# careylab/LocoMouse_cpp

Hardware: AMD Instinct MI355X
Metric: frames/sec whole-node + achieved HBM GB/s; 1024×256 gray, 6 templates (higher is better)
Workload: dtype f32

## Files before the change

### include/locomouse_hip.h

```cpp
#ifndef LOCOMOUSE_HIP_H
#define LOCOMOUSE_HIP_H

#include <stddef.h>
#include <stdint.h>

#ifdef __cplusplus
extern "C" {
#endif

#define LM_ABI_VERSION 6
#define LM_N_PAWS 4
#define LM_N_TAIL_POINTS 15
#define LM_N_LISTS 4
#define LM_N_FEATURES 2

typedef enum {
  LM_OK = 0,
  LM_ERR_INVALID_ARGUMENT = 1,
  LM_ERR_RUNTIME = 2,
  LM_ERR_HIP = 3
} lm_status;

typedef struct {
  int32_t x, y, width, height;
// ... 109 lines not shown
  const int64_t* pw_nz_offset;
  const int32_t* pw_ir;
  const double* pw_pr;
  const int32_t* tail;
} lm_batch_result;

typedef struct lm_ctx lm_ctx;

int32_t lm_abi_version(void);

const char* lm_last_error(void);

lm_status lm_ctx_create(int32_t device, const lm_setup* setup, const lm_params* params,
                        const lm_model* model, int32_t max_batch, lm_ctx** out);
void lm_ctx_destroy(lm_ctx* ctx);

lm_status lm_get_geometry(const lm_ctx* ctx, lm_geometry* out);

void* lm_ctx_stream(lm_ctx* ctx);

lm_status lm_detect_batch(lm_ctx* ctx, const uint8_t* frames, int64_t frame_pitch,
                          int32_t n, int32_t first_frame, const uint8_t* prev_frame,
                          const int32_t* bb, lm_batch_result* out);

lm_status lm_detect_batch_device(lm_ctx* ctx, const uint8_t* d_frames, int64_t frame_pitch,
                                 int32_t n, int32_t first_frame, const uint8_t* d_prev_frame,
                                 const int32_t* bb, lm_batch_result* out);

lm_status lm_detect_submit(lm_ctx* ctx, const uint8_t* frames, int64_t frame_pitch, int32_t n, int32_t first_frame,
                           const uint8_t* prev_frame, const int32_t* bb);
lm_status lm_detect_submit_device(lm_ctx* ctx, const uint8_t* d_frames, int64_t frame_pitch, int32_t n,
                                  int32_t first_frame, const uint8_t* d_prev_frame, const int32_t* bb);
lm_status lm_detect_collect(lm_ctx* ctx, lm_batch_result* out);
int32_t lm_ctx_lanes(const lm_ctx* ctx);
int32_t lm_ctx_pending(const lm_ctx* ctx);


lm_status lm_ctx_set_debug(lm_ctx* ctx, int32_t flags);

lm_status lm_debug_scores(lm_ctx* ctx, int32_t f, int32_t det, float* out, int32_t rows, int32_t cols);

lm_status lm_debug_tail_mask(lm_ctx* ctx, int32_t f, uint8_t* out, int32_t rows, int32_t cols);

int32_t lm_debug_kernel_times(lm_ctx* ctx, const char** names, double* ms, int32_t cap);

int32_t lm_debug_kernel_spans(lm_ctx* ctx, const char** names, double* t0, double* t1, int32_t cap);

lm_status lm_debug_corr_work(const lm_ctx* ctx, int32_t* out);

lm_status lm_debug_tail_work(lm_ctx* ctx, int32_t* out);

lm_status lm_debug_screen_fallback(lm_ctx* ctx, int64_t* out);

lm_status lm_debug_tail_tiles(lm_ctx* ctx, int32_t f, int32_t view, uint8_t* out, int32_t rows, int32_t cols);

lm_status lm_debug_point_work(lm_ctx* ctx, int32_t* out);

lm_status lm_debug_point_tiles(lm_ctx* ctx, int32_t f, int32_t det, uint8_t* out, int32_t rows, int32_t cols);

int32_t lm_debug_dark_tile_width(void);
int32_t lm_debug_dark_tile_height(void);

int32_t lm_debug_batch_slots(const lm_ctx* ctx);


#define LM_BB_FIRSTLAST_AS_EXECUTED 0
#define LM_BB_FIRSTLAST_INTEGER 1

typedef struct {
  int32_t median_filter_size;
  int32_t min_pixel_visible;
  int32_t moving_average_window;
  int32_t conn_comp_connectivity;
  int32_t firstlast_semantics;
  int32_t zero_col_pre, zero_col_post, zero_row_pre, zero_row_post;
  int32_t bb_width, bb_height_side;
  int32_t reserved0;
} lm_bb_params;

typedef struct {
  double x, y_bottom, y_side, width, height_bottom, height_side;
} lm_bb_frame;

typedef struct {
  int32_t n_frames;
  int32_t reserved0;
  lm_rect bb_side_mouse, bb_bottom_mouse;
  const uint32_t* x_pos;
  const uint32_t* y_bottom_pos;
  const uint32_t* y_side_pos;
  const lm_bb_frame* frames;
} lm_bb_result;

typedef struct lm_bb_ctx lm_bb_ctx;

lm_status lm_bb_create(int32_t device, const lm_setup* setup, const lm_bb_params* params, int32_t max_batch,
                       lm_bb_ctx** out);
void lm_bb_destroy(lm_bb_ctx* ctx);

lm_status lm_bb_push(lm_bb_ctx* ctx, const uint8_t* frames, int64_t frame_pitch, int32_t n, lm_bb_frame* out);
lm_status lm_bb_push_device(lm_bb_ctx* ctx, const uint8_t* d_frames, int64_t frame_pitch, int32_t n,
                            lm_bb_frame* out);

lm_status lm_bb_finish(lm_bb_ctx* ctx, lm_bb_result* out);

lm_status lm_bb_debug_binary(lm_bb_ctx* ctx, int32_t f, uint8_t* out, int32_t rows, int32_t cols);
// ... 15 lines not shown
```

### locomouse_cpp_amd/abi.py

```python
import ctypes as C

import numpy as np

LM_OK, LM_ERR_INVALID_ARGUMENT, LM_ERR_RUNTIME, LM_ERR_HIP = 0, 1, 2, 3
LM_N_TAIL_POINTS = 15
LM_FILTER_FUSED, LM_FILTER_UNFUSED = 0, 1
LM_DEBUG_SCORES, LM_DEBUG_TIMING = 1, 2
LM_DEBUG_PLAN_PER_WIDTH, LM_DEBUG_PLAN_MERGED = 16, 32
LM_CORR_FP32, LM_CORR_F16 = 0, 1
LM_DEPTH_8U, LM_DEPTH_32F, LM_DEPTH_64F = 0, 5, 6
DETECTORS = ("paw_bottom", "snout_bottom", "tail_bottom", "paw_side", "snout_side", "tail_side")


class lm_rect(C.Structure):
    _fields_ = [("x", C.c_int32), ("y", C.c_int32), ("width", C.c_int32), ("height", C.c_int32)]

    def tuple(self):
        return (self.x, self.y, self.width, self.height)


class lm_location_prior(C.Structure):
    _fields_ = [(n, C.c_double) for n in ("x", "y", "max_distance", "min_x", "max_x", "min_y", "max_y")]


class lm_params(C.Structure):
    _fields_ = [
        ("conn_comp_connectivity", C.c_int32),
        ("max_displacement_bottom", C.c_int32),
        ("max_displacement_side", C.c_int32),
        ("occlusion_grid_spacing_pixels_side", C.c_int32),
        ("occlusion_grid_spacing_pixels_bottom", C.c_int32),
        ("use_provided_bounding_box", C.c_int32),
        ("transform_gray_values", C.c_int32),
        ("use_reference_image_brightness", C.c_int32),
        ("side_bottom_min_overlap", C.c_double),
        ("occlusion_grid_max_width", C.c_double),
        ("tail_sub_bounding_box", C.c_double),
        ("alpha_vel_bottom", C.c_double),
        ("alpha_vel_side", C.c_double),
        ("pairwise_occluded_cost", C.c_double),
        ("location_prior", lm_location_prior * 5),
        ("bounding_box_side", lm_rect),
        ("bounding_box_bottom", lm_rect),
        ("gray_value_transformation", C.c_float * 256),
        ("gray_value_transformation_depth", C.c_int32),
    ]


class lm_detector(C.Structure):
    _fields_ = [("weights", C.POINTER(C.c_double)), ("rows", C.c_int32), ("cols", C.c_int32), ("bias", C.c_double)]


class lm_model(C.Structure):
    _fields_ = [(n, lm_detector) for n in ("paw_bottom", "paw_side", "snout_bottom", "snout_side", "tail_bottom", "tail_side")]


class lm_setup(C.Structure):
    _fields_ = [
        ("method", C.c_int32),
        ("flip", C.c_int32),
        ("video_rows", C.c_int32),
        ("video_cols", C.c_int32),
        ("background", C.POINTER(C.c_uint8)),
        ("calib_rows", C.c_int32),
# ... 333 lines not shown
```

### locomouse_cpp_amd/csrc/lm_corr.h

```cpp
#ifndef LM_CORR_H
#define LM_CORR_H

#include <hip/hip_runtime.h>
#include <stddef.h>
#include <stdint.h>

#include "lm_corr_dir.h"
#include "lm_device.h"

#define LM_CORR_THREADS 192
#define PK_C 5
#define PK_R 4

__host__ __device__ constexpr int pk_stride(int cols) { return cols + ((4 - (cols & 7)) + 8) % 8; }

struct LmDetGroup {
  int32_t n;
  int32_t ids[LM_NDET];
  int32_t tile_end[LM_NDET];
  int32_t ring_floats;
};

#ifdef LM_KW_ONLY
#define LM_KW_LIST(X) X(LM_KW_ONLY)
#elif defined(LM_KW_C3)
#define LM_KW_LIST(X) X(22) X(24) X(26) X(30)
#else
#define LM_KW_LIST(X)                                                                                             \
  X(16) X(17) X(18) X(19) X(20) X(21) X(22) X(23) X(24) X(25) X(26) X(27) X(28) X(29) X(30) X(31) X(32) X(36) \
      X(40) X(44) X(48) X(52) X(56) X(60) X(64)
#endif
#if defined(LM_KW_ONLY) || defined(LM_KW_C3)
#define LM_KW_LIST_RW_ALL LM_KW_LIST
#else
#define LM_KW_LIST_RW_ALL(X) X(16) X(18) X(20) X(22) X(24) X(26) X(28) X(30) X(32) X(36) X(40)
#endif
__host__ __device__ constexpr bool rw_all_width(int kw) {
  return kw % 2 == 0 && kw >= 16 && (kw <= 32 || kw == 36 || kw == 40);
}

#ifndef LM_RW_WAVES
#define LM_RW_WAVES 4
#endif
#define LM_RW_THREADS (64 * LM_RW_WAVES)
#ifndef LM_RW_ALL_WPE
#define LM_RW_ALL_WPE 4
#endif
#define LM_RW_TH 16
#define LM_RW_HTH LM_FH
#ifndef LM_RW_HSLOTS
#define LM_RW_HSLOTS (LM_FH == 4 ? 3 : LM_RW_NQ == 4 ? 7 : 8)
#endif
static_assert(LM_RW_HSLOTS >= (LM_FH == 4 ? 3 : 7), "k_corr_rw ring: rows live during a step");

__host__ __device__ constexpr int rw_stride(int kw) { return (LM_FW + kw - 1 + 3 + 3) / 4 * 4; }
__host__ __device__ constexpr int rw_qpitch(int kw) {
  return (LM_RW_HSLOTS + 1) * rw_stride(kw) +
         ((LM_FW / 5 - ((LM_RW_HSLOTS + 1) * rw_stride(kw)) % 32) + 32) % 32;
}
__host__ __device__ constexpr int rw_ring_floats(int kw) { return LM_RW_NQ * rw_qpitch(kw); }
size_t corr_rw_lds(int kw);

#define LM_F16_WAVES 4
#define LM_F16_TW 128
#define LM_F16_TH 64
#define LM_F16_THREADS (64 * LM_F16_WAVES)
#define LM_F16_MAX_NCH 10

__host__ __device__ constexpr int f16_nch(int kw) { return (kw + 31 + 15) / 16; }
__host__ __device__ constexpr int f16_cols(int nch) { return LM_F16_TW - 32 + 16 * nch; }
__host__ __device__ constexpr int f16_stride(int cols) { return (cols + 7) / 16 * 16 + 8; }
__host__ __device__ constexpr size_t f16_lds_bytes(int nch, int kh) {
  (void)nch;
  return (size_t)(LM_F16_TH + kh - 1) * f16_stride(f16_cols(nch)) * 2;
}
static inline float f16_bfrag_weight(const double* w, int kw, int i, int c, int l, int j) {
  const int r = l & 31, h = l >> 5, jj = 16 * c + 8 * h + j - r;
  return (jj >= 0 && jj < kw) ? (float)w[(size_t)i * kw + jj] : 0.0f;
}

bool corr_ring(int kw);
const void* corr_kernel(int kw, bool unf);
const void* corr_kernel_gen(bool unf);
const void* corr_kernel_rw_all(bool unf);
const void* corr_kernel_f16(int kw);
struct CorrDark {
  uint8_t* flags = nullptr;
  int32_t* cnt = nullptr;
  uint32_t* list = nullptr;
  uint8_t* tail_flags = nullptr;
  int32_t* tail_cnt = nullptr;
  uint32_t* tail_list = nullptr;
  uint8_t* pt_flags = nullptr;
  int32_t* pt_cnt = nullptr;
  uint32_t* pt_list = nullptr;
};
hipError_t launch_corr(const void* fn, bool ring, dim3 grid, int threads, size_t lds, hipStream_t st, const LmConst* K,
                       const LmDetGroup& G, const uint8_t* ext, int64_t ext_slot_bytes, const void* weights, int s0,
                       unsigned long long* keys, int32_t* n_pos, uint8_t* tailbin, int64_t tailbin_slot_bytes,
                       const CorrDark& dark, const LmCorrDirRec* dir);
#define LM_DEVERR_CORR_DIR 64
hipError_t launch_corr_dir(hipStream_t st, const LmConst* K, const LmDetGroup* groups, const char* ring, int ngroups,
                           int nslots, const CorrDark& dark, LmCorrDirRec* out, int32_t* err);
hipError_t launch_corr_dbg(bool unf, dim3 grid, hipStream_t st, const LmConst* K, const uint8_t* ext,
                           int64_t ext_slot_bytes, const float* weights, int s0, float* dbg, const int64_t* dbg_off,
                           int64_t dbg_slot_floats);

#endif
```

### locomouse_cpp_amd/csrc/lm_corr.hip

```cpp

#include <hip/hip_runtime.h>
#include <stdint.h>

#include <algorithm>
#include <cstdio>
#include <map>
#include <type_traits>
#include <vector>

#include "lm_corr.h"

#define DEV __device__ __forceinline__

typedef float lm_f2 __attribute__((ext_vector_type(2)));

template <bool UNF>
DEV lm_f2 corr_tap(lm_f2 acc, lm_f2 w2, lm_f2 p) {
  if constexpr (UNF) {
    const lm_f2 prod = w2 * p;
    return acc + prod;
  } else {
    return __builtin_elementwise_fma(w2, p, acc);
  }
}
// ... 92 lines not shown
#pragma unroll
          for (int k = 0; k < 16; ++k) o[k] = (float)((w[k >> 2] >> (8 * (k & 3))) & 0xFFu);
        } else {
#pragma unroll
          for (int k = 0; k < 16; ++k)
            if (c0 + k >= 0 && c0 + k < cols) o[k] = (float)((w[k >> 2] >> (8 * (k & 3))) & 0xFFu);
        }
      }
    }
  }
}

struct CorrTile {
  int d, oy0, ox0;
};
DEV CorrTile corr_tile(const LmConst& K, const LmDetGroup& G) {
  int gi = 0, tb = 0;
#pragma unroll
  for (int k = 0; k < LM_NDET - 1; ++k)
    if (k + 1 < G.n && (int)blockIdx.x >= G.tile_end[k]) {
      gi = k + 1;
      tb = G.tile_end[k];
    }
  const int d = G.ids[gi];
  const int lt = blockIdx.x - tb;
  const int tx = K.det[d].tiles_x;
  return CorrTile{d, (lt / tx) * K.det[d].tile_h, (lt % tx) * K.det[d].tile_w};
}

DEV const uint8_t* corr_src(const LmConst& K, const LmDet& D, const uint8_t* ext, int64_t ext_slot_bytes, int slot,
                            int oy0, int ox0) {
  return ext + (int64_t)slot * ext_slot_bytes + (D.view ? (int64_t)K.ext_h[0] * K.ext_w[0] : 0) +
         (int64_t)(D.in_y + oy0) * K.ext_w[D.view] + (D.in_x + ox0);
}


struct RwRun {
  const uint32_t* l;
  int nvalid;
  int ftx;
  int slot, oy, ox;
  DEV uint32_t entry(int i) const { return l ? l[min(i, nvalid - 1)] : 0u; }
  DEV void tile(int i, uint32_t e, int& s, int& y, int& x) const {
    if (l) {
      const int lt = (int)(e & 0xFFFFu);
      s = (int)(e >> 16);
      y = (lt / ftx) * LM_FH;
      x = (lt % ftx) * LM_FW;
    } else {
      s = slot;
      y = oy + (i / LM_RW_NQX) * LM_FH;
      x = ox + (i % LM_RW_NQX) * LM_FW;
    }
  }
};

static_assert(LM_TL_NC == 64, "one list counter per lane");

struct CorrList {
  const int32_t* cnt;
  const uint32_t* lst;
  int ftx, ntile;
};
DEV CorrList corr_det_list(const LmConst& K, const LmDet& D, const int32_t* tl_cnt, const uint32_t* tl_list, int tl_per_det,
                           const int32_t* tt_cnt, const uint32_t* tt_list) {
  const bool pt = tl_cnt != nullptr && D.kind == 0;
  if (!pt && !(tt_cnt != nullptr && D.kind != 0))
    return CorrList{nullptr, nullptr, 0, 0};
  const int v = pt ? D.view : D.list;
  const int li = pt && !tl_per_det ? v : D.list;
  const int ftx = pt ? K.fl_tx[v] : K.tt_tx[v], ntile = ftx * (pt ? K.fl_ty[v] : K.tt_ty[v]);
  const uint32_t* lst = pt ? tl_list + (int64_t)li * K.tl_stride : tt_list + (int64_t)li * K.tt_stride;
  return CorrList{(pt ? tl_cnt : tt_cnt) + li * LM_TL_NC, lst, ftx, ntile};
}

DEV int corr_scan_waves(int wv) {
  const int lane = threadIdx.x & 63;
  int P = wv;
#pragma unroll
  for (int o = 1; o < 64; o <<= 1) {
    const int u = __shfl_up(P, o);
    if (lane >= o) P += u;
  }
  return P;
}

DEV RwRun corr_listed_run(const CorrList& Ls, int cn, int wv, int P, int local, int nslots) {
  constexpr int NQ = LM_RW_NQ;
  const int c = __builtin_amdgcn_readfirstlane(__ffsll((long long)__ballot(P > local)) - 1);
  const int w = local - (__builtin_amdgcn_readlane(P, c) - __builtin_amdgcn_readlane(wv, c));
  const int ng = (nslots + LM_INGEST_FB - 1) / LM_INGEST_FB;
  return RwRun{Ls.lst + (int64_t)lm_tl_y0(c, ng) * LM_INGEST_FB * Ls.ntile + NQ * w,
               min(NQ, __builtin_amdgcn_readlane(cn, c) - NQ * w), Ls.ftx, 0, 0, 0};
}

DEV RwRun corr_unlisted_run(const LmDet& D, int nt, int s0, int local) {
  const int tx = D.tiles_x;
  const int lt = local - (local / nt) * nt;
  return RwRun{nullptr, LM_RW_NQ, 0, s0 + local / nt, (lt / tx) * LM_RW_TH, (lt % tx) * LM_TW};
}

DEV bool corr_locate_walk(const LmConst& K, const LmDetGroup& G, int nslots, int s0, int g, const int32_t* tl_cnt,
                          const uint32_t* tl_list, int tl_per_det, const int32_t* tt_cnt, const uint32_t* tt_list, int& d,
                          RwRun& R) {
  const int lane = threadIdx.x & 63;
  int base = 0;
// ... 133 lines not shown
DEV void lds_pair_nw(lm_f2& dst, unsigned base) {
  static_assert(Q + STRIDE <= 255, "ds_read2_b32 offset range");
  asm volatile("ds_read2_b32 %0, %1 offset0:%2 offset1:%3" : "=v"(dst) : "v"(base), "i"(Q), "i"(Q + STRIDE) : "memory");
}

template <bool UNF, int H>
DEV lm_f2 corr_tap_h(lm_f2 acc, lm_f2 w2, lm_f2 p) {
  if constexpr (UNF) {
    lm_f2 prod;
    if constexpr (H == 0)
      asm volatile("v_pk_mul_f32 %0, %1, %2 op_sel_hi:[0,1]" : "=v"(prod) : "s"(w2), "v"(p));
    else
      asm volatile("v_pk_mul_f32 %0, %1, %2 op_sel:[1,0] op_sel_hi:[1,1]" : "=v"(prod) : "s"(w2), "v"(p));
    asm volatile("v_pk_add_f32 %0, %0, %1" : "+v"(acc) : "v"(prod));
    return acc;
  } else if constexpr (H == 0) {
    asm volatile("v_pk_fma_f32 %0, %1, %2, %0 op_sel_hi:[0,1,1]" : "+v"(acc) : "s"(w2), "v"(p));
    return acc;
  } else {
    asm volatile("v_pk_fma_f32 %0, %1, %2, %0 op_sel:[1,0,0] op_sel_hi:[1,1,1]" : "+v"(acc) : "s"(w2), "v"(p));
    return acc;
  }
}

#define LM_RWF(a, w, p, sel) "v_pk_fma_f32 %" #a ", %" #w ", %" #p ", %" #a " " sel "\n"
#define LM_RW_S0 "op_sel_hi:[0,1,1]"
#define LM_RW_S1 "op_sel:[1,0,0] op_sel_hi:[1,1,1]"
DEV void rw_pair_ab(lm_f2 (&a)[PK_C], lm_f2 (&b)[PK_C], lm_f2 wa, lm_f2 wb, const lm_f2* px) {
  static_assert(PK_C == 5, "the asm block is written for 5 columns");
  asm volatile(LM_RWF(0, 10, 12, LM_RW_S0) LM_RWF(1, 10, 13, LM_RW_S0) LM_RWF(2, 10, 14, LM_RW_S0)
                   LM_RWF(3, 10, 15, LM_RW_S0) LM_RWF(4, 10, 16, LM_RW_S0)
               LM_RWF(5, 11, 12, LM_RW_S0) LM_RWF(6, 11, 13, LM_RW_S0) LM_RWF(7, 11, 14, LM_RW_S0)
                   LM_RWF(8, 11, 15, LM_RW_S0) LM_RWF(9, 11, 16, LM_RW_S0)
               LM_RWF(0, 10, 13, LM_RW_S1) LM_RWF(1, 10, 14, LM_RW_S1) LM_RWF(2, 10, 15, LM_RW_S1)
                   LM_RWF(3, 10, 16, LM_RW_S1) LM_RWF(4, 10, 17, LM_RW_S1)
               LM_RWF(5, 11, 13, LM_RW_S1) LM_RWF(6, 11, 14, LM_RW_S1) LM_RWF(7, 11, 15, LM_RW_S1)
                   LM_RWF(8, 11, 16, LM_RW_S1) LM_RWF(9, 11, 17, LM_RW_S1)
               : "+v"(a[0]), "+v"(a[1]), "+v"(a[2]), "+v"(a[3]), "+v"(a[4]), "+v"(b[0]), "+v"(b[1]), "+v"(b[2]),
                 "+v"(b[3]), "+v"(b[4])
               : "s"(wa), "s"(wb), "v"(px[0]), "v"(px[1]), "v"(px[2]), "v"(px[3]), "v"(px[4]), "v"(px[5]));
}
DEV void rw_pair_1(lm_f2 (&a)[PK_C], lm_f2 w, const lm_f2* px) {
  asm volatile(LM_RWF(0, 5, 6, LM_RW_S0) LM_RWF(1, 5, 7, LM_RW_S0) LM_RWF(2, 5, 8, LM_RW_S0)
                   LM_RWF(3, 5, 9, LM_RW_S0) LM_RWF(4, 5, 10, LM_RW_S0)
               LM_RWF(0, 5, 7, LM_RW_S1) LM_RWF(1, 5, 8, LM_RW_S1) LM_RWF(2, 5, 9, LM_RW_S1)
                   LM_RWF(3, 5, 10, LM_RW_S1) LM_RWF(4, 5, 11, LM_RW_S1)
               : "+v"(a[0]), "+v"(a[1]), "+v"(a[2]), "+v"(a[3]), "+v"(a[4])
               : "s"(w), "v"(px[0]), "v"(px[1]), "v"(px[2]), "v"(px[3]), "v"(px[4]), "v"(px[5]));
}
#undef LM_RWF
#undef LM_RW_S0
#undef LM_RW_S1

template <int KW, bool UNF>
struct RwPipe {
  using P = RwPlan<KW>;
  static constexpr int STR = rw_stride(KW);
  lm_f2 px[PK_C + KW - 1];
  lm_f2 acc[2][PK_C];
  lm_f2 wa[P::PMAX], wb[P::PMAX];
  template <int Q0, int Q1>
  DEV void issue(unsigned base) {
    if constexpr (Q0 < Q1) {
      lds_pair_nw<STR, Q0>(px[Q0], base);
      issue<Q0 + 1, Q1>(base);
    }
  }
  template <int C>
  DEV void load_w(lm_f2 (&na)[P::PMAX], lm_f2 (&nb)[P::PMAX], const lm_f2* __restrict__ ra,
                  const lm_f2* __restrict__ rb) {
#pragma unroll
    for (int q = 0; q < P::qe(C) - P::qb(C); ++q) {
      na[q] = ra[P::qb(C) + q];
      nb[q] = rb[P::qb(C) + q];
    }
  }
  template <int J, int C, bool A, bool B>
  DEV void compute_from() {
    if constexpr (J < P::end(C) && !UNF && (J & 1) == 0 && J + 1 < P::end(C) &&
                  (A || B)) {
      constexpr int q = J / 2 - P::qb(C);
      if constexpr (A && B) rw_pair_ab(acc[0], acc[1], wa[q], wb[q], &px[J]);
      else if constexpr (A) rw_pair_1(acc[0], wa[q], &px[J]);
      else rw_pair_1(acc[1], wb[q], &px[J]);
      compute_from<J + 2, C, A, B>();
    } else if constexpr (J < P::end(C)) {
      constexpr int q = J / 2 - P::qb(C), h = J & 1;
      if constexpr (A) {
#pragma unroll
        for (int c = 0; c < PK_C; ++c) acc[0][c] = corr_tap_h<UNF, h>(acc[0][c], wa[q], px[c + J]);
      }
      if constexpr (B) {
#pragma unroll
        for (int c = 0; c < PK_C; ++c) acc[1][c] = corr_tap_h<UNF, h>(acc[1][c], wb[q], px[c + J]);
      }
      compute_from<J + 1, C, A, B>();
    }
  }
  template <int C, bool A, bool B, bool NEXT = true, typename F>
  DEV void chunks(unsigned base, unsigned base_n, const lm_f2* __restrict__ ra, const lm_f2* __restrict__ rb,
                  const lm_f2* __restrict__ ra_n, const lm_f2* __restrict__ rb_n, F&& at_start) {
    __builtin_amdgcn_s_waitcnt(0xC07F);
    __builtin_amdgcn_sched_barrier(0);
    if constexpr (C == 0) at_start();
    lm_f2 na[P::PMAX], nb[P::PMAX];
    if constexpr (C + 1 < P::N) {
      load_w<C + 1>(na, nb, ra, rb);
      issue<P::pbeg(C + 1), P::pend(C + 1)>(base);
    } else if constexpr (NEXT) {
      load_w<0>(na, nb, ra_n, rb_n);
      issue<P::pbeg(0), P::pend(0)>(base_n);
    }
    __builtin_amdgcn_sched_barrier(0);
    compute_from<P::beg(C), C, A, B>();
    __builtin_amdgcn_sched_barrier(0);
    if constexpr (C + 1 < P::N || NEXT) {
#pragma unroll
      for (int q = 0; q < P::PMAX; ++q) {
        wa[q] = na[q];
        wb[q] = nb[q];
      }
    }
    if constexpr (C + 1 < P::N) chunks<C + 1, A, B, NEXT>(base, base_n, ra, rb, ra_n, rb_n, at_start);
  }
};

struct RwArgs {
  const LmConst* K;
  LmDetGroup G;
  const uint8_t* ext;
  int64_t ext_slot_bytes;
  const float* weights;
  int32_t s0, nslots;
  unsigned long long* keys;
  int32_t* n_pos;
  uint8_t* tailbin;
  int64_t tailbin_slot_bytes;
  const int32_t* tl_cnt;
  const uint32_t* tl_list;
  int32_t tl_per_det;
  const int32_t* tt_cnt;
  const uint32_t* tt_list;
};

template <int KW, bool UNF>
DEV __attribute__((always_inline)) void rw_tile(const RwArgs& A, int dix, const RwRun& R, float* ring) {
  constexpr int NQ = LM_RW_NQ;
  constexpr int QX = LM_FW / PK_C;
  static_assert(LM_FH == PK_R && QX * NQ == 64, "one row of 8 lanes per 40 x 4 sub-tile");
  constexpr int STR = rw_stride(KW);
  constexpr int QP = rw_qpitch(KW);
  constexpr int NL = (3 + LM_FW + KW - 1 + 3) / 4;
  constexpr int NLD = (NQ * NL + 63) / 64;
  static_assert(NLD <= 4, "window rows wider than four loads per lane");
  constexpr int HS = LM_RW_HSLOTS;
  const LmConst& K = *A.K;
  const LmDet& D = K.det[dix];
  const int lane = threadIdx.x & 63;
  const int q = lane / QX, lx = lane % QX;
  const int kh = D.kh, kwp = D.kwp;
  __builtin_assume(kh >= 2);
  const int nrows = LM_RW_HTH + kh - 1;
  const int ew = K.ext_w[D.view];
  const int ew4 = ew >> 2;
  const uint8_t* __restrict__ vext = A.ext + (D.view ? (int64_t)K.ext_h[0] * K.ext_w[0] : 0);
  const int mis = D.in_x & 3;
  int slot, oy0, ox0;
  R.tile(q, R.entry(q), slot, oy0, ox0);
  const bool valid = q < R.nvalid;
  int smin = slot;
#pragma unroll
  for (int o = 1; o < 64; o <<= 1) smin = min(smin, __shfl_xor(smin, o));
  smin = __builtin_amdgcn_readfirstlane(smin);
  const __amdgpu_buffer_rsrc_t wrsrc = __builtin_amdgcn_make_buffer_rsrc(
      const_cast<uint8_t*>(vext + (int64_t)smin * A.ext_slot_bytes), 0, (int)0xFFFFFFFF, 0x00020000);
  unsigned la[NLD];
  int lo[NLD];
  bool lk[NLD];
#pragma unroll
  for (int k = 0; k < NLD; ++k) {
    const int e = lane + 64 * k, qk = e / NL, dk = e - qk * NL;
    lk[k] = qk < R.nvalid;
    int sk, yk, xk;
    const int ik = min(qk, NQ - 1);
    R.tile(ik, R.entry(ik), sk, yk, xk);
    la[k] = (unsigned)((int64_t)(sk - smin) * A.ext_slot_bytes + (int64_t)(D.in_y + yk) * ew + (D.in_x + xk - mis)) +
            4u * (unsigned)dk;
    lo[k] = (int)(unsigned)(uintptr_t)(__attribute__((address_space(3))) float*)(ring + qk * QP + 4 * dk);
  }

  unsigned mbits = 0;
  if (D.kind == 0 && valid) {
    const uint8_t* __restrict__ m =
        vext + (int64_t)slot * A.ext_slot_bytes + (int64_t)(D.m_y + oy0) * ew + (D.m_x + ox0 + lx * PK_C);
    const int mo = (int)((uintptr_t)m & 3);
    const unsigned* __restrict__ m4 = reinterpret_cast<const unsigned*>(m - mo);
    unsigned mw[PK_R][2];
#pragma unroll
    for (int r = 0; r < PK_R; ++r) {
      mw[r][0] = m4[(int64_t)r * ew4];
      mw[r][1] = m4[(int64_t)r * ew4 + 1];
    }
#pragma unroll
    for (int r = 0; r < PK_R; ++r) {
      const unsigned long long row = ((unsigned long long)mw[r][1] << 32 | mw[r][0]) >> (8 * mo);
#pragma unroll
      for (int c = 0; c < PK_C; ++c) mbits |= (((unsigned)(row >> (8 * c)) & 0xFFu) > 25u ? 1u : 0u) << (r * PK_C + c);
    }
  }

  struct Row {
    unsigned v[NLD];
  };
  auto load_row = [&](int r) -> Row {
    Row w;
    const int ro = __builtin_amdgcn_readfirstlane(min(r, nrows - 1) * ew);
#pragma unroll
    for (int k = 0; k < NLD; ++k) w.v[k] = __builtin_amdgcn_raw_buffer_load_b32(wrsrc, (int)la[k], ro, 0);
    return w;
  };
  auto store_row = [&](int r, Row w) {
    if (r >= nrows) return;
    const int s = r % HS;
    const int so = __builtin_amdgcn_readfirstlane(s * STR * (int)sizeof(float));
#pragma unroll
    for (int k = 0; k < NLD; ++k)
      if (lk[k]) {
        const unsigned v = w.v[k];
        typedef float f4v __attribute__((ext_vector_type(4)));
        const f4v f = {(float)(v & 0xFFu), (float)((v >> 8) & 0xFFu), (float)((v >> 16) & 0xFFu), (float)(v >> 24)};
        typedef __attribute__((address_space(3))) f4v lds_f4;
        *reinterpret_cast<lds_f4*>((uintptr_t)(unsigned)(lo[k] + so)) = f;
        if (s == 0) *reinterpret_cast<lds_f4*>((uintptr_t)(unsigned)(lo[k] + HS * STR * (int)sizeof(float))) = f;
      }
  };
  {
    Row v0[HS];
#pragma unroll
    for (int r = 0; r < HS; ++r) v0[r] = load_row(r);
#pragma unroll
    for (int r = 0; r < HS; ++r) store_row(r, v0[r]);
  }

  const lm_f2* __restrict__ W = reinterpret_cast<const lm_f2*>(A.weights + D.w_off);
  const int kwp2 = kwp >> 1;
  const unsigned ring_base = (unsigned)(uintptr_t)(const __attribute__((address_space(3))) float*)ring +
                             (unsigned)(q * QP * (int)sizeof(float));
  const unsigned lane_off = (unsigned)((lx * PK_C + mis) * (int)sizeof(float));
  const unsigned ring_lane = ring_base + lane_off;
  auto row_base = [&](int t) -> unsigned {
    return ring_lane + (unsigned)__builtin_amdgcn_readfirstlane((t % HS) * STR * (int)sizeof(float));
  };
  RwPipe<KW, UNF> S;
#pragma unroll
  for (int p = 0; p < 2; ++p)
#pragma unroll
    for (int c = 0; c < PK_C; ++c) S.acc[p][c] = (lm_f2){D.delta, D.delta};
  auto wrow = [&](int i) { return W + min(max(i, 0), kh - 1) * kwp2; };
  S.template load_w<0>(S.wa, S.wb, wrow(0), wrow(-2));
  S.template issue<RwPlan<KW>::pbeg(0), RwPlan<KW>::pend(0)>(row_base(0));
  using T1 = std::true_type;
  using F0 = std::false_type;
  auto stepx = [&](int t, auto B0, auto B1, Row& st, Row& ld, auto N) {
    S.template chunks<0, decltype(B0)::value, decltype(B1)::value, decltype(N)::value>(
        row_base(t), row_base(t + 1), wrow(t), wrow(t - 2), wrow(t + 1), wrow(t - 1),
        [&]() { if constexpr (decltype(N)::value) ld = load_row(t + HS + 1); });
    if constexpr (decltype(N)::value) store_row(t + HS, st);
  };
  Row r0 = load_row(HS), r1;
  {
    stepx(0, T1{}, F0{}, r0, r1, T1{});
    stepx(1, T1{}, F0{}, r1, r0, T1{});
    int t = 2;
    for (; t + 1 < kh; t += 2) {
      stepx(t, T1{}, T1{}, r0, r1, T1{});
      stepx(t + 1, T1{}, T1{}, r1, r0, T1{});
    }
    if (t < kh) {
      stepx(t, T1{}, T1{}, r0, r1, T1{});
      stepx(kh, F0{}, T1{}, r1, r0, T1{});
      stepx(kh + 1, F0{}, T1{}, r0, r1, F0{});
    } else {
      stepx(kh, F0{}, T1{}, r0, r1, T1{});
      stepx(kh + 1, F0{}, T1{}, r1, r0, F0{});
    }
  }
  __builtin_amdgcn_s_waitcnt(0xC07F);

  unsigned bits = 0;
  if (valid) {
#pragma unroll
    for (int p = 0; p < PK_R / 2; ++p)
#pragma unroll
      for (int c = 0; c < PK_C; ++c) {
        const int x = ox0 + lx * PK_C + c;
        const int y0 = oy0 + 2 * p;
        if (x < D.ow && y0 < D.oh && S.acc[p][c].x > 0.0f) bits |= 1u << ((2 * p) * PK_C + c);
        if (x < D.ow && y0 + 1 < D.oh && S.acc[p][c].y > 0.0f) bits |= 1u << ((2 * p + 1) * PK_C + c);
      }
  }
  if (D.kind != 0) {
    constexpr int WPS = QX / LM_FH;
    static_assert(WPS * LM_FH == QX && (LM_FW == 40 ? WPS == 2 : WPS == 4), "a sub-tile's bitmap words, one per lane");
    unsigned* s_tb = reinterpret_cast<unsigned*>(ring);
    const int w0 = ox0 >> 5;
    s_tb[lane] = 0u;
    __builtin_amdgcn_wave_barrier();
#pragma unroll
    for (int r = 0; r < PK_R; ++r)
#pragma unroll
      for (int c = 0; c < PK_C; ++c)
        if (bits & (1u << (r * PK_C + c))) {
          const int x = ox0 + lx * PK_C + c;
          atomicOr(&s_tb[q * QX + r * WPS + (x >> 5) - w0], 1u << (x & 31));
        }
    __builtin_amdgcn_wave_barrier();
    const unsigned v = s_tb[lane];
    unsigned* __restrict__ tb = reinterpret_cast<unsigned*>(A.tailbin + (int64_t)slot * A.tailbin_slot_bytes) +
                                (D.list ? (int64_t)K.tail_hb * K.tail_nw : 0);
    const int y = oy0 + lx / WPS, gw = w0 + lx % WPS;
    if (v && y < D.oh && gw < K.tail_nw) atomicOr(&tb[(int64_t)y * K.tail_nw + gw], v);
    return;
  }
  bits &= mbits;
  const int cnt = __popc(bits);
  int incl = cnt;
#pragma unroll
  for (int o = 1; o < QX; o <<= 1) {
    const int u = __shfl_up(incl, o, QX);
    if (lx >= o) incl += u;
  }
  const int tot = __shfl(incl, QX - 1, QX);
  const int before = incl - cnt, lastl = (lane & ~(QX - 1)) + QX - 1;
  if (__ballot(tot != 0) == 0) return;
  int base_k = 0;
  if (lane == lastl && tot) base_k = atomicAdd(&A.n_pos[slot * LM_NLIST + D.list], tot);
  base_k = __shfl(base_k, lastl);
  unsigned long long* __restrict__ kl = A.keys + (int64_t)slot * K.keys_per_slot + K.list_off[D.list] + base_k + before;
  int pos = 0;
#pragma unroll
  for (int p = 0; p < PK_R / 2; ++p)
#pragma unroll
    for (int c = 0; c < PK_C; ++c)
#pragma unroll
      for (int hh = 0; hh < 2; ++hh) {
        const int r = 2 * p + hh, k = r * PK_C + c;
        if (bits & (1u << k)) {
          const int y = oy0 + r, x = ox0 + lx * PK_C + c;
          const float sc = hh ? S.acc[p][c].y : S.acc[p][c].x;
          kl[pos++] = ((unsigned long long)(~__float_as_uint(sc)) << 32) | (unsigned)(y * D.ow + x);
        }
      }
}

#ifndef LM_RW_XCD
#define LM_RW_XCD 16
#endif
DEV int xcd_block(int b, int nb) {
#if LM_RW_XCD
  constexpr int C = LM_RW_XCD;
  const int full = nb / (8 * C) * (8 * C);
  if (b >= full) return b;
  const int k = b >> 3, x = b & 7;
  return (k / C) * (8 * C) + x * C + (k % C);
#else
  (void)nb;
  return b;
#endif
}

#ifndef LM_RW_WPE
#define LM_RW_WPE (LM_FW == 40 ? 4 : 5)
#endif
template <int KW, bool UNF>
__global__ __launch_bounds__(LM_RW_THREADS) __attribute__((amdgpu_waves_per_eu(KW <= 32 ? LM_RW_WPE : 1, 8))) void k_corr_rw(
    const LmConst* __restrict__ Kp, const LmDetGroup G, const uint8_t* __restrict__ ext, int64_t ext_slot_bytes,
    const float* __restrict__ weights, int s0, int nslots, unsigned long long* __restrict__ keys,
    int32_t* __restrict__ n_pos, uint8_t* __restrict__ tailbin, int64_t tailbin_slot_bytes,
    const int32_t* __restrict__ tl_cnt, const uint32_t* __restrict__ tl_list, int tl_per_det,
    const int32_t* __restrict__ tt_cnt, const uint32_t* __restrict__ tt_list, const LmCorrDirRec* __restrict__ dir) {
  extern __shared__ uint4 lds_rw[];
  const int wave = __builtin_amdgcn_readfirstlane(threadIdx.x >> 6);
  float* ring = reinterpret_cast<float*>(lds_rw) + wave * rw_ring_floats(KW);
  const RwArgs a{Kp,    G,       ext,    ext_slot_bytes, weights, s0, nslots, keys, n_pos, tailbin, tailbin_slot_bytes,
                 tl_cnt, tl_list, tl_per_det, tt_cnt, tt_list};
  int d;
  RwRun R;
  if (!corr_locate_rw(*a.K, G, a.nslots, a.s0, xcd_block(blockIdx.x, gridDim.x) * LM_RW_WAVES + wave, a.tl_cnt,
                      a.tl_list, a.tl_per_det, a.tt_cnt, a.tt_list, dir, d, R))
    return;
  rw_tile<KW, UNF>(a, d, R, ring);
}

template <bool UNF>
__global__ __launch_bounds__(LM_RW_THREADS) __attribute__((amdgpu_waves_per_eu(LM_RW_ALL_WPE, 8))) void k_corr_rw_all(
    const LmConst* __restrict__ Kp, const LmDetGroup G, const uint8_t* __restrict__ ext, int64_t ext_slot_bytes,
    const float* __restrict__ weights, int s0, int nslots, unsigned long long* __restrict__ keys,
    int32_t* __restrict__ n_pos, uint8_t* __restrict__ tailbin, int64_t tailbin_slot_bytes,
    const int32_t* __restrict__ tl_cnt, const uint32_t* __restrict__ tl_list, int tl_per_det,
    const int32_t* __restrict__ tt_cnt, const uint32_t* __restrict__ tt_list, const LmCorrDirRec* __restrict__ dir) {
  extern __shared__ uint4 lds_rw[];
  const int wave = __builtin_amdgcn_readfirstlane(threadIdx.x >> 6);
  float* ring = reinterpret_cast<float*>(lds_rw) + wave * G.ring_floats;
  const RwArgs a{Kp,    G,       ext,    ext_slot_bytes, weights, s0, nslots, keys, n_pos, tailbin, tailbin_slot_bytes,
                 tl_cnt, tl_list, tl_per_det, tt_cnt, tt_list};
  int d;
  RwRun R;
  if (!corr_locate_rw(*a.K, G, a.nslots, a.s0, xcd_block(blockIdx.x, gridDim.x) * LM_RW_WAVES + wave, a.tl_cnt,
                      a.tl_list, a.tl_per_det, a.tt_cnt, a.tt_list, dir, d, R))
    return;
  switch (a.K->det[d].kw_ring) {
#define LM_KW_CASE(n)           \
  case n:                       \
    rw_tile<n, UNF>(a, d, R, ring); \
    break;
    LM_KW_LIST_RW_ALL(LM_KW_CASE)
#undef LM_KW_CASE
    default:
      break;
  }
}

template <bool UNF>
__global__ __launch_bounds__(LM_CORR_THREADS) void k_corr_gen(const LmConst* __restrict__ Kp, const LmDetGroup G,
                                                              const uint8_t* __restrict__ ext, int64_t ext_slot_bytes,
                                                              const float* __restrict__ weights, int s0,
                                                              unsigned long long* __restrict__ keys,
                                                              int32_t* __restrict__ n_pos, uint8_t* __restrict__ tailbin,
                                                              int64_t tailbin_slot_bytes,
                                                              const uint8_t* __restrict__ dark,
                                                              const uint8_t* __restrict__ tail_flags,
                                                              const uint8_t* __restrict__ pt_flags) {
  const LmConst& K = *Kp;
  extern __shared__ float lds[];
  __shared__ int s_cnt, s_base;
  const int slot = s0 + blockIdx.y;
  const CorrTile T = corr_tile(K, G);
  const LmDet D = K.det[T.d];
  const int oy0 = T.oy0, ox0 = T.ox0;
  if (corr_tile_dark(K, D, pt_flags ? pt_flags + (int64_t)(D.list & 1) * K.pt_plane : dark, tail_flags, slot, oy0, ox0))
    return;
  const int kh = D.kh, kwp = D.kwp, ch = D.chunk_rows;
  const int cols = LM_TW + kwp - 1, stride = pk_stride(cols);
  const int ew = K.ext_w[D.view];
  const uint8_t* __restrict__ src = corr_src(K, D, ext, ext_slot_bytes, slot, oy0, ox0);
  const float* __restrict__ W = weights + D.w_off;
  if (threadIdx.x == 0) s_cnt = 0;
  const int ly = threadIdx.x >> 4, lx = threadIdx.x & 15;
  lm_f2 acc[PK_R / 2][PK_C];
#pragma unroll
  for (int p = 0; p < PK_R / 2; ++p)
#pragma unroll
    for (int c = 0; c < PK_C; ++c) acc[p][c] = (lm_f2){D.delta, D.delta};
  for (int i0 = 0; i0 < kh; i0 += ch) {
    const int cn = min(ch, kh - i0);
    __syncthreads();
    tile_fill_f32(lds, stride, src + (int64_t)i0 * ew, ew, LM_TH + cn - 1, cols);
    __syncthreads();
    for (int t = 0; t < cn + PK_R - 2; ++t) {
      const float* p0 = lds + (ly * PK_R + t) * stride + lx * PK_C;
      for (int jc = 0; jc < kwp; jc += LM_JC) {
        lm_f2 px[PK_C + LM_JC - 1];
#pragma unroll
        for (int q = 0; q < PK_C + LM_JC - 1; ++q) px[q] = (lm_f2){p0[jc + q], p0[jc + q + stride]};
#pragma unroll
        for (int p = 0; p < PK_R / 2; ++p) {
          const int i = t - 2 * p;
// ... 226 lines not shown
  const int ew = K.ext_w[D.view];
  const uint8_t* __restrict__ base =
      ext + (int64_t)slot * ext_slot_bytes + (D.view ? (int64_t)K.ext_h[0] * K.ext_w[0] : 0);
  const float* __restrict__ W = weights + D.w_off;
  for (int64_t e = (int64_t)blockIdx.x * blockDim.x + threadIdx.x; e < n; e += (int64_t)gridDim.x * blockDim.x) {
    const int y = (int)(e / D.ow), x = (int)(e % D.ow);
    const uint8_t* src = base + (int64_t)(D.in_y + y) * ew + (D.in_x + x);
    float a = D.delta;
    for (int i = 0; i < D.kh; ++i)
      for (int j = 0; j < D.kw; ++j) a = corr_tap1<UNF>(a, W[i * D.kwp + j], (float)src[(int64_t)i * ew + j]);
    dbg[(int64_t)slot * dbg_slot_floats + dbg_off[d] + e] = a;
  }
}

const void* corr_kernel_f16(int kw) {
  switch (f16_nch(kw)) {
    case 2: return (const void*)&k_corr_f16<2>;
    case 3: return (const void*)&k_corr_f16<3>;
    case 4: return (const void*)&k_corr_f16<4>;
    case 5: return (const void*)&k_corr_f16<5>;
    case 6: return (const void*)&k_corr_f16<6>;
    case 7: return (const void*)&k_corr_f16<7>;
    case 8: return (const void*)&k_corr_f16<8>;
    case 9: return (const void*)&k_corr_f16<9>;
    case 10: return (const void*)&k_corr_f16<10>;
    default: return nullptr;
  }
}

bool corr_ring(int kw) {
  switch (kw) {
#define LM_KW_CASE(n) case n:
    LM_KW_LIST(LM_KW_CASE)
#undef LM_KW_CASE
    return true;
    default:
      return false;
  }
}

const void* corr_kernel(int kw, bool unf) {
  switch (kw) {
#define LM_KW_CASE(n) \
  case n:             \
    return unf ? (const void*)&k_corr_rw<n, true> : (const void*)&k_corr_rw<n, false>;
    LM_KW_LIST(LM_KW_CASE)
#undef LM_KW_CASE
    default:
      return unf ? (const void*)&k_corr_gen<true> : (const void*)&k_corr_gen<false>;
  }
}

size_t corr_rw_lds(int kw) { return (size_t)LM_RW_WAVES * rw_ring_floats(kw) * sizeof(float); }

const void* corr_kernel_gen(bool unf) { return unf ? (const void*)&k_corr_gen<true> : (const void*)&k_corr_gen<false>; }

const void* corr_kernel_rw_all(bool unf) {
  return unf ? (const void*)&k_corr_rw_all<true> : (const void*)&k_corr_rw_all<false>;
}

hipError_t launch_corr(const void* fn, bool ring, dim3 grid, int threads, size_t lds, hipStream_t st, const LmConst* K,
                       const LmDetGroup& G, const uint8_t* ext, int64_t ext_slot_bytes, const void* weights, int s0,
                       unsigned long long* keys, int32_t* n_pos, uint8_t* tailbin, int64_t tailbin_slot_bytes,
                       const CorrDark& dk, const LmCorrDirRec* dir) {
  if (ring) {
    int nslots = (int)grid.y;
    const unsigned waves = (unsigned)(G.tile_end[G.n - 1] * nslots);
    int per_det = dk.pt_cnt != nullptr ? 1 : 0;
    const int32_t* tl_cnt = per_det ? dk.pt_cnt : dk.cnt;
    const uint32_t* tl_list = per_det ? dk.pt_list : dk.list;
    void* args[] = {(void*)&K,       (void*)&G,    (void*)&ext,     (void*)&ext_slot_bytes,
                    (void*)&weights, (void*)&s0,   (void*)&nslots,  (void*)&keys,
                    (void*)&n_pos,   (void*)&tailbin, (void*)&tailbin_slot_bytes, (void*)&tl_cnt,
                    (void*)&tl_list, (void*)&per_det, (void*)&dk.tail_cnt, (void*)&dk.tail_list, (void*)&dir};
    return hipLaunchKernel(fn, dim3((waves + LM_RW_WAVES - 1) / LM_RW_WAVES), dim3(LM_RW_THREADS), args, lds, st);
  }
  void* args[] = {(void*)&K,     (void*)&G,       (void*)&ext,     (void*)&ext_slot_bytes,           (void*)&weights,
                  (void*)&s0,    (void*)&keys,    (void*)&n_pos,   (void*)&tailbin, (void*)&tailbin_slot_bytes,
                  (void*)&dk.flags, (void*)&dk.tail_flags, (void*)&dk.pt_flags};
  return hipLaunchKernel(fn, grid, dim3(threads), args, lds, st);
}

hipError_t launch_corr_dir(hipStream_t st, const LmConst* K, const LmDetGroup* groups, const char* ring, int ngroups,
                           int nslots, const CorrDark& dk, LmCorrDirRec* out, int32_t* err) {
  if (ngroups < 1 || ngroups > LM_NDET) return hipErrorInvalidValue;
  LmCorrDirGroups A{};
  A.n = ngroups;
  for (int b = 0; b < ngroups; ++b) {
    A.ring[b] = ring[b] ? 1 : 0;
    A.g[b] = groups[b];
  }
  const int per_det = dk.pt_cnt != nullptr ? 1 : 0;
  k_corr_dir<<<ngroups, 64, 0, st>>>(K, A, nslots, per_det ? dk.pt_cnt : dk.cnt, per_det ? dk.pt_list : dk.list, per_det,
                                     dk.tail_cnt, dk.tail_list, out, err);
  return hipGetLastError();
}

hipError_t launch_corr_dbg(bool unf, dim3 grid, hipStream_t st, const LmConst* K, const uint8_t* ext,
                           int64_t ext_slot_bytes, const float* weights, int s0, float* dbg, const int64_t* dbg_off,
                           int64_t dbg_slot_floats) {
  if (unf)
    k_corr_dbg<true><<<grid, 256, 0, st>>>(K, ext, ext_slot_bytes, weights, s0, dbg, dbg_off, dbg_slot_floats);
  else
    k_corr_dbg<false><<<grid, 256, 0, st>>>(K, ext, ext_slot_bytes, weights, s0, dbg, dbg_off, dbg_slot_floats);
  return hipGetLastError();
}
// ... 2 lines not shown
```

### locomouse_cpp_amd/csrc/lm_device.h

```cpp
#ifndef LM_DEVICE_H
#define LM_DEVICE_H

#include <stdint.h>

#if defined(__HIPCC__)
#define LM_HD __host__ __device__
#else
#define LM_HD
#endif

#define LM_C 5
#define LM_R 3
#define LM_TW (16 * LM_C)
#define LM_TH (16 * LM_R)
#define LM_JC 4
#ifndef LM_FW
#define LM_FW 40
#endif
#ifndef LM_FH
#define LM_FH 4
#endif
static_assert((LM_FW == 40 || LM_FW == 80) && (LM_FH == 4 || LM_FH == 8), "dark-tile grid");
#define LM_RW_NQX (LM_TW / LM_FW)
#define LM_RW_NQY (16 / LM_FH)
// ... 11 lines not shown
#define LM_NLIST 4
#define LM_NFEAT 2

enum { DET_PAW_B = 0, DET_SNOUT_B = 1, DET_TAIL_B = 2, DET_PAW_S = 3, DET_SNOUT_S = 4, DET_TAIL_S = 5 };
enum { LIST_PAW_B = 0, LIST_SNOUT_B = 1, LIST_PAW_S = 2, LIST_SNOUT_S = 3 };

struct LmDet {
  int32_t view;
  int32_t kind;
  int32_t list;
  int32_t kh, kw, kwp;
  int32_t kw_ring;
  int32_t w_off;
  float delta;
  int32_t oh, ow;
  int32_t in_y, in_x;
  int32_t m_y, m_x;
  int32_t tiles_x, tiles_y, tile_base;
  int32_t tile_w, tile_h;
  int32_t box_w, box_h;
  int32_t chunk_rows;
  int32_t w16_off;
  float wscale, inv_wscale;
};

struct LmConst {
  LmDet det[LM_NDET];
  int32_t n_tiles;
  int32_t ext_h[2], ext_w[2];
  int32_t ext_oy[2], ext_ox[2];
  int32_t crop_h[2], crop_w[2];
  int32_t unpad_y[2], unpad_x[2];
  int32_t video_rows, video_cols;
  int32_t n_rows, n_cols;
  int32_t pad_pre_rows, pad_pre_cols, ipad_rows, ipad_cols;
  int32_t flip;
  int32_t tail_w, tail_hb, tail_hs;
  int32_t tail_cap, tail_ntc;
  int32_t tail_nw, tail_bm_words;
  int32_t connectivity;
  int32_t fl_tx[2], fl_ty[2], fl_off[2], fl_slot;
  int32_t tl_stride;
  int32_t tt_tx[2], tt_ty[2], tt_off[2], tt_slot;
  int32_t tt_stride;
  int64_t pt_plane;
  int32_t tb_skip[LM_NDET], tb_off[LM_NDET], tb_rng[LM_NDET], tb_lds[2];
  double tb_bias[LM_NDET];
  int32_t tbw_br[2], tbw_nband[2], tbw_blo[2], tbw_nbk[2], tbw_rows[2], tbw_v[2], tbw_al[2], tbw_work[2], tbw_lds[2];
  int32_t tbw_use[LM_NDET], tbw_pn[LM_NDET], tbw_win[LM_NDET], tbw_wsz[LM_NDET], tbw_ent[LM_NDET];
  uint32_t tbw_inv[LM_NDET];
  int32_t tbr_on[LM_NDET], tbr_ng[LM_NDET], tbr_off[LM_NDET];
  int32_t tbs_on[LM_NDET], tbs_off[LM_NDET];
  float tbs_bf[LM_NDET], tbs_e[LM_NDET];
  int32_t fl_my[2], fl_mx[2], fl_oh[2], fl_ow[2];
  int32_t ing_b0[2], ing_nb[2], ing_threads;
  int32_t list_cap[LM_NLIST];
  int64_t list_off[LM_NLIST];
  int64_t keys_per_slot;
  double side_bottom_min_overlap;
  double alpha_vel_bottom, pairwise_occluded_cost;
  int32_t max_displacement_bottom, ong_spacing_bottom;
  int32_t ong_nx, ong_ny;
  double ong_br_x, ong_br_y;
  int32_t bb_bottom_w, bb_bottom_h;
  int32_t spre_b_w, spre_b_h, spre_t_w, spre_t_h;
  int32_t match_b[LM_NFEAT][4];
  int32_t match_s[LM_NFEAT][4];
  int32_t size_b[LM_NFEAT][2];
  int32_t size_s[LM_NFEAT][2];
  double prior[5][7];
  int32_t gray_lut_on;
  uint8_t gray_lut[256];
};

LM_HD inline uint32_t lm_rcp(int d) { return (uint32_t)(0x80000000u / (uint32_t)d + 1u); }
LM_HD inline int lm_div(int x, uint32_t rcp) { return (int)(((uint64_t)(uint32_t)x * rcp) >> 31); }

LM_HD inline int lm_tbw_band(const LmDet& D, int ty, int br, int j, int* t0, int* nty) {
  *t0 = j * br;
  const int t1 = ty < *t0 + br ? ty : *t0 + br;
  *nty = t1 > *t0 ? t1 - *t0 : 0;
  if (*nty == 0) return 0;
  return (D.oh < LM_FH * t1 ? D.oh : LM_FH * t1) - LM_FH * *t0;
}

struct LmSlot {
  int32_t crop_x[2], crop_y[2];
  int32_t frame;
  int32_t active;
};

struct LmSlotOut {
  int32_t n_pos[LM_NLIST];
  int32_t cand_off[LM_NLIST];
  int32_t cand_cnt[LM_NLIST];
  int32_t p22d_off[LM_NFEAT], p22d_cnt[LM_NFEAT];
  int32_t side_off[LM_NFEAT], side_cnt[LM_NFEAT];
  int32_t unary_off[LM_NFEAT], unary_cnt[LM_NFEAT];
  int32_t pw_rows[LM_NFEAT], pw_cols[LM_NFEAT], pw_nnz[LM_NFEAT];
  int32_t pw_jc_off[LM_NFEAT], pw_nz_off[LM_NFEAT];
  int32_t tail[45];
  int32_t ties[LM_NLIST];
  int32_t bottom_kept[LM_NFEAT];
  int32_t pad_[1];
};

// ... 70 lines not shown
```

### locomouse_cpp_amd/csrc/lm_kernels.hip

```cpp
#include <hip/hip_runtime.h>
#include <stdint.h>

#include <type_traits>
#include <utility>

#include "lm_device.h"
#include "lm_introsort.h"

#include "lm_dev_common.h"
#include "lm_tail_bound.h"
#include "lm_tile_plan.h"



__global__ __launch_bounds__(LM_MM_THREADS) void k_minmax(const uint8_t* const* __restrict__ frame_ptr,
                                                          const uint8_t* __restrict__ bkg, int npix, int s0,
                                                          unsigned* __restrict__ mm) {
  const int slot = s0 + blockIdx.y;
  const lm_gu8* __restrict__ F = as_global(frame_ptr[slot]);
  const int nvec = npix >> 4;
  const int per = (nvec + LM_MM_SPLIT - 1) / LM_MM_SPLIT;
  const int v0 = blockIdx.x * per, v1 = min(nvec, v0 + per);
  const lm_gu4* F4 = reinterpret_cast<const lm_gu4*>(F);
  const uint4* B4 = reinterpret_cast<const uint4*>(bkg);
  unsigned mn = 255, mx = 0;
  auto fold = [&](unsigned fw, unsigned bw) {
#pragma unroll
    for (int k = 0; k < 4; ++k) {
      const unsigned fv = (fw >> (8 * k)) & 255u, bv = (bw >> (8 * k)) & 255u;
      const unsigned d = fv > bv ? fv - bv : 0u;
      mn = min(mn, d);
      mx = max(mx, d);
    }
  };
  int i = v0 + threadIdx.x;
  for (; i + 3 * LM_MM_THREADS < v1; i += 4 * LM_MM_THREADS) {
    lm_u32x4 f[4];
    uint4 b[4];
#pragma unroll
    for (int u = 0; u < 4; ++u) {
      f[u] = F4[i + u * LM_MM_THREADS];
      b[u] = B4[i + u * LM_MM_THREADS];
    }
#pragma unroll
    for (int u = 0; u < 4; ++u) {
      fold(f[u].x, b[u].x);
      fold(f[u].y, b[u].y);
      fold(f[u].z, b[u].z);
      fold(f[u].w, b[u].w);
    }
  }
  for (; i < v1; i += LM_MM_THREADS) {
    const lm_u32x4 f = F4[i];
    const uint4 b = B4[i];
    fold(f.x, b.x);
    fold(f.y, b.y);
    fold(f.z, b.z);
    fold(f.w, b.w);
  }
  if (blockIdx.x == LM_MM_SPLIT - 1)
    for (int q = (nvec << 4) + threadIdx.x; q < npix; q += LM_MM_THREADS) {
      const unsigned fv = F[q], bv = bkg[q];
// ... 545 lines not shown
    for (int i = tid; i < ntile; i += T) {
      bool keep = br ? br[i] != 0 : true;
      mbr += br && keep ? 1 : 0;
      if (keep && use[k])
        keep = !lm_tb_tile_skip(rmax, rmin, ftx, D.oh, D.kh, i / ftx, i % ftx, P, P + D.kh, K.tb_bias[d]);
      if (keep && use[k] && K.tbr_on[d] != 0)
        keep = !lm_tbr_tile_skip(bmax, bmin, nbw, D.in_y, D.in_x, D.oh, D.ow, D.kh, D.kw, i / ftx, i % ftx,
                                 tbc + K.tbr_off[d], K.tb_bias[d], LM_TB_RH, false);
      fl[i] = keep ? 1 : 0;
      mine += keep ? 1 : 0;
    }
    if (mine) atomicAdd(&s_n[k], mine);
    if (mbr) atomicAdd(&s_b[k], mbr);
  }
  __syncthreads();
  const int G = ((int)gridDim.x + LM_INGEST_FB - 1) / LM_INGEST_FB;
  const int c = ((int)blockIdx.x / LM_INGEST_FB) * LM_TL_NC / G;
  if (tid < 3 && (K.det[3 * v + tid].kind != 0 ? tt_cnt != nullptr : pt_cnt != nullptr)) {
    const LmDet& D = K.det[3 * v + tid];
    int32_t* __restrict__ cnt = D.kind != 0 ? tt_cnt + v * LM_TL_NC : pt_cnt + D.list * LM_TL_NC;
    s_base[tid] = s_n[tid] ? atomicAdd(&cnt[c], s_n[tid]) : 0;
    if (D.kind == 0 && s_b[tid]) atomicAdd(&pt_cnt[(LM_NLIST + D.list) * LM_TL_NC + c], s_b[tid]);
  }
  __syncthreads();
#pragma unroll
  for (int k = 0; k < 3; ++k) {
    if (!on[k]) continue;
    const LmDet& D = K.det[3 * v + k];
    const bool tail = D.kind != 0;
    const int ntile = tail ? K.tt_tx[v] * K.tt_ty[v] : K.fl_tx[v] * K.fl_ty[v];
    const uint8_t* __restrict__ fl = tail ? tail_flags + (int64_t)slot * K.tt_slot + K.tt_off[v]
                                          : pt_flags + (D.list & 1) * K.pt_plane + (int64_t)slot * K.fl_slot + K.fl_off[v];
    uint32_t* __restrict__ out =
        (tail ? tt_list + (int64_t)v * K.tt_stride : pt_list + (int64_t)D.list * K.tl_stride) +
        (int64_t)lm_tl_y0(c, G) * LM_INGEST_FB * ntile + s_base[k];
    for (int i = tid; i < ntile; i += T)
      if (fl[i]) out[atomicAdd(&s_k[k], 1)] = ((uint32_t)slot << 16) | (uint32_t)i;
  }
}

DEV uint32_t range_merge(uint32_t a, uint32_t b) { return lm_tb_range_merge(a, b); }
DEV int wave_append(bool p, int* ctr) {
  const unsigned long long m = __ballot(p);
  if (m == 0ull) return 0;
  const int rank = (int)__builtin_amdgcn_mbcnt_hi((unsigned)(m >> 32), __builtin_amdgcn_mbcnt_lo((unsigned)m, 0u));
  int base = 0;
  if (p && rank == 0) base = atomicAdd(ctr, (int)__popcll(m));
  return __shfl(base, __ffsll((long long)m) - 1) + rank;
}
#ifndef LM_TBW_WPE
#define LM_TBW_WPE 8
#endif
#define TBW_SEL(a) (k == 0 ? a[0] : k == 1 ? a[1] : a[2])
template <bool ROWS>
__global__ __launch_bounds__(LM_TB_THREADS) __attribute__((amdgpu_waves_per_eu(LM_TBW_WPE, 8))) void k_tile_bound(
    const LmConst* __restrict__ Kp, const uint32_t* __restrict__ rng, int64_t rng_slot, int s0, int nslot,
    const double* __restrict__ tbc, const uint8_t* __restrict__ bright, uint8_t* __restrict__ tail_flags,
    int32_t* __restrict__ tt_cnt, uint32_t* __restrict__ tt_list, uint8_t* __restrict__ pt_flags,
    int32_t* __restrict__ pt_cnt, uint32_t* __restrict__ pt_list, unsigned long long* __restrict__ tbs_fallback) {
  const LmConst& K = *Kp;
  extern __shared__ __attribute__((aligned(16))) uint8_t tbw_lds[];
  __shared__ int s_n[3], s_b[3], s_m[3], s_base[3], s_nw;
  const int v = (int)blockIdx.y < K.tbw_nband[0] ? 0 : 1;
  const int band = (int)blockIdx.y - (v ? K.tbw_nband[0] : 0);
  const int slot = s0 + (int)blockIdx.x;
  const int T = (int)blockDim.x, tid = (int)threadIdx.x;
  if (tid < 3) {
    s_n[tid] = 0;
    s_b[tid] = 0;
    s_m[tid] = 0;
  }
  if (tid == 0) s_nw = 0;
  bool on[3], use[3], refine[3], tail[3];
  int t0[3], nt[3], ohb[3], ftx[3], tbase[3];
  uint8_t* fl[3];
  int y_lo = K.ext_h[v], y_hi = 0;
#pragma unroll
  for (int k = 0; k < 3; ++k) {
    const int d = 3 * v + k;
    const LmDet& D = K.det[d];
    tail[k] = D.kind != 0;
    on[k] = tail[k] ? tt_cnt != nullptr : pt_cnt != nullptr;
    use[k] = on[k] && K.tbw_use[d] != 0;
    ftx[k] = tail[k] ? K.tt_tx[v] : K.fl_tx[v];
    int nty;
    ohb[k] = lm_tbw_band(D, tail[k] ? K.tt_ty[v] : K.fl_ty[v], K.tbw_br[v], band, &t0[k], &nty);
    nt[k] = on[k] ? nty * ftx[k] : 0;
    tbase[k] = t0[k] * ftx[k];
    fl[k] = tail[k] ? tail_flags + (int64_t)slot * K.tt_slot + K.tt_off[v]
                    : pt_flags + (D.list & 1) * K.pt_plane + (int64_t)slot * K.fl_slot + K.fl_off[v];
    use[k] = use[k] && nt[k] > 0;
    refine[k] = use[k] && K.tbr_on[d] != 0;
    if (use[k]) {
      y_lo = min(y_lo, D.in_y + LM_FH * t0[k]);
      y_hi = max(y_hi, D.in_y + LM_FH * t0[k] + ohb[k] + D.kh - 1);
    }
  }
  y_hi = min(y_hi, K.ext_h[v]);
  const int nrow = max(0, min(y_hi - y_lo, K.tbw_rows[v]));
  const int nbk = K.tbw_nbk[v], nw = nbk / 2;
  uint32_t* B = reinterpret_cast<uint32_t*>(tbw_lds);
  uint32_t* V = reinterpret_cast<uint32_t*>(tbw_lds + K.tbw_v[v]);
  uint32_t* work = reinterpret_cast<uint32_t*>(tbw_lds + K.tbw_work[v]);
  __syncthreads();
  constexpr int LD = LM_TBW_LD;
  const int ne = nrow * nw, ewq = K.ext_w[v] / LM_INGEST_VEC;
  const uint32_t rc = lm_rcp(max(nw, 1));
  const uint32_t* __restrict__ src = rng + (int64_t)slot * rng_slot +
                                     (v ? (int64_t)K.ext_h[0] * K.ext_w[0] / LM_INGEST_VEC : 0) +
                                     (int64_t)min(y_lo, y_hi) * ewq + K.tbw_blo[v] / 2;
  uint32_t w[LD];
  auto rng_load = [&](int e0) {
#pragma unroll
    for (int u = 0; u < LD; ++u) {
      const int e = e0 + u * T + tid;
// ... 238 lines not shown
        }) ? -1 : 1;
      };
      auto level_b = [&](int rs, int nn) {
        return lm_tbr_sum_negative(kh, ng, C, bias, [&](int i, int g, unsigned& M, unsigned& m) {
          const uint16_t* row = B16 + (row0 + rs + i) * nbk;
          M = 0u;
          m = 255u;
          for (int r = 0; r < nn; ++r, row += nbk) {
            unsigned a, b;
            lm_tbr_pair_range(nullptr, row, ba0 + g, bendl, a, b);
            M = max(M, a);
            m = min(m, b);
          }
        });
      };
      using std::integral_constant;
      using std::false_type;
      using std::true_type;
      bool proven;
      if constexpr (!ROWS) {
        proven = nr == LM_TB_H && level_v(integral_constant<int, 0>{}, false_type{}) < 0;
      } else {
        proven = false;
        if (nr != LM_TB_H) {
        } else if (nc != 1) proven = level_v(integral_constant<int, 0>{}, false_type{}) < 0;
        else {
          int dec = 0;
          if (K.tbs_on[d] != 0) {
            if (ng == 4) dec = level_v(integral_constant<int, 4>{}, true_type{});
            else if (ng == 3) dec = level_v(integral_constant<int, 3>{}, true_type{});
            else if (ng == 2) dec = level_v(integral_constant<int, 2>{}, true_type{});
            else dec = level_v(integral_constant<int, 1>{}, true_type{});
            const unsigned long long und = __ballot(dec == 0);
            if (und != 0ull && (tid & (WV - 1)) == __ffsll((long long)und) - 1)
              atomicAdd(tbs_fallback, (unsigned long long)__popcll(und));
          }
          if (dec == 0) {
            if (ng == 4) dec = level_v(integral_constant<int, 4>{}, false_type{});
            else if (ng == 3) dec = level_v(integral_constant<int, 3>{}, false_type{});
            else if (ng == 2) dec = level_v(integral_constant<int, 2>{}, false_type{});
            else dec = level_v(integral_constant<int, 1>{}, false_type{});
          }
          proven = dec < 0;
        }
      }
      if (!proven && !(LM_TB_RH == LM_TB_H && nr == LM_TB_H)) {
        if (LM_TB_RH == LM_TB_H) {
          proven = level_b(0, nr);
        } else {
          proven = true;
          for (int r = 0; r < nr && proven; ++r) proven = level_b(r, 1);
        }
      }
      if (!proven) mark[mb + t] = 1u;
    }
    __syncthreads();
    constexpr int CR = LM_TBW_CR;
    for (int g0 = 0; g0 < nref; g0 += CR * T) {
      uint32_t en[CR];
      int kk[CR];
#pragma unroll
      for (int u = 0; u < CR; ++u) {
        const int i = g0 + u * T + tid;
        const bool act = i < nref;
        const int k = i < nr3[0] ? 0 : i < nr3[0] + nr3[1] ? 1 : 2;
        const int t = i - (k == 0 ? 0 : k == 1 ? nr3[0] : nr3[0] + nr3[1]);
        en[u] = act ? reinterpret_cast<const uint32_t*>(tbw_lds + TBW_SEL(ent3))[t] : 0u;
        const bool kp = act && mark[i] != 0u;
        kk[u] = kp ? k : -1;
        if (act) TBW_SEL(fl)[en[u] & 0xFFFFu] = kp ? 1 : 0;
      }
      __syncthreads();
#pragma unroll
      for (int u = 0; u < CR; ++u)
#pragma unroll
        for (int k = 0; k < 3; ++k) {
          const bool mine = kk[u] == k;
          const int pos = wave_append(mine, &s_m[k]);
          if (mine) reinterpret_cast<uint32_t*>(tbw_lds + ent3[k])[pos] = en[u];
        }
    }
    __syncthreads();
    if (tid < 3) {
      const int k = tid;
      if (TBW_SEL(nr3) > 0) s_n[k] = s_m[k];
    }
  }
  __syncthreads();
  const int G = (nslot + LM_INGEST_FB - 1) / LM_INGEST_FB;
  const int c = ((int)blockIdx.x / LM_INGEST_FB) * LM_TL_NC / G;
  if (tid < 3 && (K.det[3 * v + tid].kind != 0 ? tt_cnt != nullptr : pt_cnt != nullptr)) {
    const LmDet& D = K.det[3 * v + tid];
    int32_t* __restrict__ cnt = D.kind != 0 ? tt_cnt + v * LM_TL_NC : pt_cnt + D.list * LM_TL_NC;
    s_base[tid] = s_n[tid] ? atomicAdd(&cnt[c], s_n[tid]) : 0;
    if (D.kind == 0 && s_b[tid]) atomicAdd(&pt_cnt[(LM_NLIST + D.list) * LM_TL_NC + c], s_b[tid]);
  }
  __syncthreads();
#pragma unroll
  for (int k = 0; k < 3; ++k) {
    if (!on[k] || s_n[k] == 0) continue;
    const LmDet& D = K.det[3 * v + k];
    const int ntile = tail[k] ? K.tt_tx[v] * K.tt_ty[v] : K.fl_tx[v] * K.fl_ty[v];
    const uint32_t* ent = reinterpret_cast<const uint32_t*>(tbw_lds + K.tbw_ent[3 * v + k]);
    uint32_t* __restrict__ out =
        (tail[k] ? tt_list + (int64_t)v * K.tt_stride : pt_list + (int64_t)D.list * K.tl_stride) +
        (int64_t)lm_tl_y0(c, G) * LM_INGEST_FB * ntile + s_base[k];
    for (int p = tid; p < s_n[k]; p += T) out[p] = ent[p];
  }
}
#undef TBW_SEL

#include "lm_corr.h"

#include "lm_cc.h"

DEV float key_score(unsigned long long k) { return __uint_as_float(~(unsigned)(k >> 32)); }
DEV unsigned key_lo(unsigned long long k) { return (unsigned)(k & 0xFFFFFFFFu); }
#ifndef LM_TAIL_THREADS
#define LM_TAIL_THREADS 256
#endif
#define LM_TAIL_SEGS 15

struct TailLayout {
  int rowoff, colc, colm, mask, bm, par, area, key, rs, re, mb, ms, bytes;
};
__host__ __device__ inline TailLayout tail_layout(int TW, int HB, int HS, int cap, int ntc) {
  const int Hm = HB > HS ? HB : HS, nb64 = (TW + 63) / 64;
  const int ntrb = (HB + 31) / 32, ntrs = (HS + 31) / 32;
  TailLayout L;
  int o = 0;
  L.rowoff = o;
  o += 4 * (Hm + 1);
  L.colc = o;
  o += 4 * (TW + 2);
  o = (o + 15) & ~15;
  L.colm = o;
  o += 8 * nb64;
  L.mask = o;
  o += 8 * HB * nb64;
  L.bm = o;
  L.par = o;
  L.area = o + 4 * cap;
  L.key = o + 8 * cap;
  const int bmb = 8 * Hm * (nb64 + 1), ufb = 12 * cap;
  o += bmb > ufb ? bmb : ufb;
  L.rs = o;
  o += 2 * cap;
  L.re = o;
  o += 2 * cap;
  o = (o + 15) & ~15;
  L.mb = o;
  o += 4 * LM_TAIL_SEGS * ntrb * ntc * 3;
  L.ms = o;
  o += 4 * LM_TAIL_SEGS * ntrs * 2;
  L.bytes = o;
  return L;
}

DEV void tail_segment(int rx, int rem, int reg, int* seg, int* sx) {
  if (rx < rem * (reg + 1)) {
// ... 1475 lines not shown
    int* g = reinterpret_cast<int*>(gscratch + (int64_t)blockIdx.x * gscratch_slot);
    int* g_off = g;
    int* g_mb = g_off + max(Ni + Nong, Nb) + 1;
    int* g_mt = g_mb + big;
    float* g_bps = reinterpret_cast<float*>(g_mt + big);
    float* g_tpb = g_bps + big;
    if ((int64_t)(reinterpret_cast<int*>(g_tpb + big) - g) > 2 * gscratch_slot) {
      if (threadIdx.x == 0) atomicOr(err, 8);
      return;
    }
    post_run<true>(K, slots, frame_ptr, bkg, cal, luts, H, slot, feat, frame, Nb, Ns, Ni, cb, ct, cp, g_off, g_mb, g_mt,
                   g_bps, g_tpb, big, s_base, s_any1, s_any0, arena_p22d, arena_side_y, arena_side_s, arena_unary,
                   arena_jc, arena_ir, arena_pr, ctl, err, (2 * bx + feat) % ctl->nparts, prof);
  }
}

template <bool GLOB>
__global__ __launch_bounds__(LM_POST_THREADS) void k_post(LM_POST_ARGS, int npairs) {
  if constexpr (!GLOB)
    post_block<false>(blockIdx.x, blockIdx.y, LM_POST_PASS);
  else
    for_overflow_pairs(
        npairs,
        [&](int p) {
          const int slot = 1 + (p >> 1), feat = p & 1;
          const LmSlotOut* H = hdr + slot;
          const int Nb = H->cand_cnt[feat], Ns = H->cand_cnt[2 + feat];
          const int Ni = slots[slot].frame > 0 ? hdr[slot - 1].cand_cnt[feat] : 0;
          return !(Nb <= LM_POST_MAXC && Ns <= LM_POST_MAXC && Ni <= LM_POST_MAXC &&
                   Ni + Kp->ong_nx * Kp->ong_ny + 1 <= LM_POST_MAXOFF);
        },
        [&](int p) { post_block<true>(p >> 1, p & 1, LM_POST_PASS); });
}

DEV void carry_block(const LmConst& K, unsigned long long* __restrict__ keys, const LmSlotOut* __restrict__ prev_hdr,
                     int prev_slot, LmSlotOut* __restrict__ hdr) {
  for (int l = 0; l < LM_NFEAT; ++l) {
    const int cnt = prev_hdr[prev_slot].cand_cnt[l];
    const LmCand* src = LM_CAND_STAGE(K, keys, prev_slot, l);
    LmCand* dst = LM_CAND_STAGE(K, keys, 0, l);
    for (int k = threadIdx.x; k < cnt; k += blockDim.x) dst[k] = src[k];
    if (threadIdx.x == 0) hdr[0].cand_cnt[l] = cnt;
  }
}

static_assert(4 * LM_TL_NC == 256 && 2 * LM_NLIST * LM_TL_NC == 512, "k_prep zeroes the tile-list counters with its 256 threads");
__global__ __launch_bounds__(256) void k_prep(const LmSlot* __restrict__ h_slots, const uint8_t* const* __restrict__ h_fptr,
                                              const LmArenaCtl* __restrict__ h_ctl, int ns, LmSlot* __restrict__ slots,
                                              const uint8_t** __restrict__ fptr, LmArenaCtl* __restrict__ ctl,
                                              int32_t* __restrict__ npos, int32_t* __restrict__ err,
                                              const LmConst* __restrict__ Kp, unsigned long long* __restrict__ keys,
                                              const LmSlotOut* __restrict__ prev_hdr, int prev_slot,
                                              LmSlotOut* __restrict__ hdr, int32_t* __restrict__ dark_cnt,
                                              int32_t* __restrict__ tail_cnt, int32_t* __restrict__ pt_cnt) {
  if (blockIdx.x == 1) {
    carry_block(*Kp, keys, prev_hdr, prev_slot, hdr);
    return;
  }
  if (dark_cnt) dark_cnt[threadIdx.x] = 0;
  if (tail_cnt && threadIdx.x < 2 * LM_TL_NC) tail_cnt[threadIdx.x] = 0;
  if (pt_cnt) {
    pt_cnt[threadIdx.x] = 0;
    pt_cnt[256 + threadIdx.x] = 0;
  }
  for (int i = threadIdx.x; i < ns; i += blockDim.x) {
    slots[i] = h_slots[i];
    fptr[i] = h_fptr[i];
  }
  for (int i = threadIdx.x; i < ns * LM_NLIST; i += blockDim.x) npos[i] = 0;
  if (threadIdx.x < 16) err[threadIdx.x] = 0;
  if (threadIdx.x < AR_COUNT) {
    ctl->used[threadIdx.x] = h_ctl->used[threadIdx.x];
    ctl->cap[threadIdx.x] = h_ctl->cap[threadIdx.x];
  }
  if (threadIdx.x == 0) {
    ctl->overflow = h_ctl->overflow;
    ctl->nparts = h_ctl->nparts;
    ctl->pack_dst = h_ctl->pack_dst;
    ctl->pack_cap = h_ctl->pack_cap;
  }
  for (int i = threadIdx.x; i < LM_SUBARENA * 32; i += blockDim.x) (&ctl->sub[0][0])[i] = 0;
}

__global__ __launch_bounds__(256) void k_out(const LmPackHdr* __restrict__ ph, LmPackHdr* __restrict__ h_ph,
                                             const uint8_t* __restrict__ pack, uint8_t* __restrict__ h_pack, int64_t h_cap,
                                             const LmArenaCtl* __restrict__ ctl,
                                             const uint8_t* __restrict__ halo_arg, const uint8_t* const* __restrict__ fptr,
                                             int fidx, uint8_t* __restrict__ halo_dst, int64_t halo_bytes) {
  if (!h_pack && ctl) {
    h_pack = ctl->pack_dst;
    h_cap = ctl->pack_cap;
  }
  const uint8_t* __restrict__ halo_src = halo_arg ? halo_arg : (fptr ? fptr[fidx] : nullptr);
  const int64_t tid = (int64_t)blockIdx.x * blockDim.x + threadIdx.x, nth = (int64_t)gridDim.x * blockDim.x;
  if (tid == 0) *h_ph = *ph;
  const int64_t bytes = ph->bytes;
  if (ph->overflow || ph->err || bytes > h_cap) return;
  for (int64_t i = tid; i < bytes / 16; i += nth)
    reinterpret_cast<uint4*>(h_pack)[i] = reinterpret_cast<const uint4*>(pack)[i];
  if (halo_src) {
    for (int64_t i = tid; i < halo_bytes / 16; i += nth)
      reinterpret_cast<uint4*>(halo_dst)[i] = reinterpret_cast<const uint4*>(halo_src)[i];
    for (int64_t i = halo_bytes / 16 * 16 + tid; i < halo_bytes; i += nth) halo_dst[i] = halo_src[i];
  }
}

__global__ __launch_bounds__(1024) void k_pack_scan(const LmSlotOut* __restrict__ hdr, int n,
                                                    const LmArenaCtl* __restrict__ ctl, const int32_t* __restrict__ err,
                                                    LmPackHdr* __restrict__ ph, uint8_t* __restrict__ pack, int64_t pack_cap,
                                                    int64_t* __restrict__ side_base) {
  constexpr int NA = 6;
  __shared__ int64_t s_w[1024 / 64 + 1][NA];
  const int64_t zero[PK_COUNT] = {0, 0, 0, 0, 0, 0};
  const LmPackLayout L0 = lm_pack_layout(n, zero);
  const LmSlotOut* H = hdr + 1;
  int64_t* outs[NA] = {reinterpret_cast<int64_t*>(pack + L0.cand_off), reinterpret_cast<int64_t*>(pack + L0.p22d_off),
// ... 156 lines not shown
```

### locomouse_cpp_amd/csrc/lm_runtime.hip

```cpp
#include <hip/hip_runtime.h>

#include <algorithm>
#include <array>
#include <cmath>
#include <cstdio>
#include <cstring>
#include <map>
#include <numeric>
#include <atomic>
#include <deque>
#include <memory>
#include <mutex>
#include <stdexcept>
#include <string>
#include <thread>
#include <vector>

#include "locomouse_hip.h"
#include "lm_host.h"
#include "lm_batch_plan.h"
#include "lm_kernels.hip"

namespace {

// ... 23 lines not shown
  void alloc(const int* c, int nslots) {
    for (int k = 0; k < AR_COUNT; ++k) cap[k] = c[k];
    p22d.alloc(cap[AR_P22D]);
    side_y.alloc(cap[AR_SIDE]);
    side_s.alloc(cap[AR_SIDE]);
    unary.alloc(cap[AR_UNARY]);
    jc.alloc(cap[AR_PWJC]);
    ir.alloc(cap[AR_PWNZ]);
    pr.alloc(cap[AR_PWNZ]);
    if (!hdr.p) hdr.alloc(nslots);
    if (!ctl.p) ctl.alloc(1);
    if (!ph.p) ph.alloc(1);
    if (!side_base.p) side_base.alloc(2 * (size_t)nslots + 1);
    const int64_t tot[PK_COUNT] = {cap[AR_CAND], cap[AR_P22D], cap[AR_SIDE], cap[AR_UNARY], cap[AR_PWJC], cap[AR_PWNZ]};
    alloc_pack(lm_pack_layout(nslots, tot).bytes);
  }
  void alloc_pack(int64_t bytes) {
    if (bytes <= pack_cap) return;
    pack.alloc((size_t)bytes);
    pack_cap = bytes;
  }
};

struct Lane {
  int index = 0;
  int device = 0;
  hipStream_t stream = nullptr;
  DevBuf<uint8_t> frames, halo, luts, ext, tailbin;
  DevBuf<unsigned long long> tailmask;
  DevBuf<int32_t> npos, err;
  DevBuf<unsigned> mm;
  DevBuf<unsigned> tscratch;
  DevBuf<uint8_t> tail_ws;
  DevBuf<float> dbg;
  DevBuf<int64_t> dbg_offd;
  DevBuf<const uint8_t*> frame_ptr;
  DevBuf<LmSlot> slots;
  DevBuf<unsigned long long> keys, gscratch;
  DevBuf<int2> smap;
  DevBuf<uint4> sbkg;
  DevBuf<int32_t> skey;
  int skey_h[4] = {-1, -1, -1, -1};
  DevBuf<uint8_t> dark_flags;
  DevBuf<uint32_t> dark_list;
  DevBuf<int32_t> dark_cnt;
  DevBuf<uint8_t> tail_flags;
  DevBuf<uint32_t> tail_list;
  DevBuf<int32_t> tail_cnt;
  DevBuf<uint8_t> pt_flags;
  DevBuf<uint32_t> pt_list;
  DevBuf<int32_t> pt_cnt;
  DevBuf<uint32_t> rng;
  DevBuf<LmCorrDirRec> corr_dir;
  HostBuf<int32_t> h_cnt;
  bool h_cnt_valid = false;
  DevBuf<long long> kprof;
  DevBuf<long long> kprof_ing;
  Arena arena[2];
  int parity = 0;
  HostBuf<LmSlot> h_slots;
  HostBuf<const uint8_t*> h_frame_ptr;
  HostBuf<LmArenaCtl> h_ctl;
  HostBuf<int32_t> h_err;
  HostBuf<LmPackHdr> h_ph;
  DevBuf<LmPackHdr> zero_ph;
  bool have_state = false;
  int last_frame = -1, last_n = 0, last_parity = 0;
  struct Pending {
    bool on = false;
    int n = 0, first = 0, s_lut0 = 1, s_proc0 = 1, plan = 0, cur = 0, prv = 0, last_n = 0;
    int pack = -1;
    bool carry = false;
  } pend;
  int64_t seq = -1;
  int64_t done_seq = -1;
  int batch_n = 0, batch_s0 = 1;
  hipEvent_t ev_snap = nullptr, ev_consumed = nullptr;
  hipEvent_t ev_done = nullptr;
  std::vector<std::pair<const char*, int>> t_ev;
  std::vector<const char*> t_names;
  std::vector<double> t_ms, t_t0, t_t1;
  int32_t t_work[4] = {-1, -1, -1, -1};
  std::vector<hipEvent_t> ev_pool;
  struct GraphEntry {
    hipGraphExec_t exec[3];
  };
  std::map<std::array<int, 7>, GraphEntry> graphs;
  bool use_graphs = true;
  void drop_graphs() {
    for (auto& g : graphs)
      for (hipGraphExec_t x : g.second.exec)
        if (x) (void)hipGraphExecDestroy(x);
    graphs.clear();
  }
  ~Lane() {
    drop_graphs();
    if (stream) {
      (void)hipSetDevice(device);
      (void)hipStreamSynchronize(stream);
      for (hipEvent_t e : ev_pool) (void)hipEventDestroy(e);
      if (ev_snap) (void)hipEventDestroy(ev_snap);
      if (ev_consumed) (void)hipEventDestroy(ev_consumed);
      if (ev_done) (void)hipEventDestroy(ev_done);
      (void)hipStreamDestroy(stream);
    }
  }
};

}

struct lm_ctx {
  int device = 0;
  int max_batch = 0, nslots = 0;
  int debug = 0;
  lm_setup setup{};
  lm_params params{};
  lm_geometry geo{};
  LmConst K{};
  int npix = 0;
  int64_t fstride = 0;
  int bb_x = 0, bb_yb = 0, bb_ys = 0;
  int64_t ext_slot_bytes = 0, tailbin_slot_bytes = 0, dbg_slot_floats = 0;
  int64_t dbg_off[LM_NDET] = {0};
  int64_t gscratch_slot = 0;
  bool unfused = false;
  struct CorrPlan {
    std::vector<std::pair<const void*, LmDetGroup>> groups;
    std::vector<size_t> lds;
    std::vector<int> threads;
    std::vector<char> ring;
  } corr_plan[2];
  DevBuf<uint8_t> bkg, adj;
  DevBuf<int32_t> cal;
  DevBuf<float> weights;
  DevBuf<_Float16> weights16;
  DevBuf<LmConst> dK;
  size_t tail_lds = 0;
  bool tail_big = false;
  int64_t tail_ws_slot = 0;
  bool kprof_on = false;
  bool dark_on = true;
  bool tailskip_on = true;
  bool pointskip_on = true;
  bool tb_ref = false;
  bool tb_refine = true;
  bool tb_screen = true;
  bool corr_dir_on = true;
  size_t tb_lds = 0;
  size_t tbw_lds = 0;
  bool tbw_row_loop = false;
  DevBuf<double> tb_const;
  DevBuf<unsigned long long> tbs_fallback;
  std::vector<std::unique_ptr<Lane>> lanes;
  DevBuf<uint8_t> handoff;
  std::vector<std::unique_ptr<HostBuf<uint8_t>>> packs;
  std::vector<char> pack_busy;
  int take_pack(size_t cap) {
    size_t i = 0;
    while (i < packs.size() && pack_busy[i]) ++i;
    if (i == packs.size()) {
      packs.emplace_back(new HostBuf<uint8_t>());
      pack_busy.push_back(0);
    }
    if (packs[i]->n < cap) packs[i]->alloc(cap);
    pack_busy[i] = 1;
    return (int)i;
  }
  void drop_pack(int i) {
    if (i >= 0 && i < (int)pack_busy.size()) pack_busy[i] = 0;
  }
  struct BatchRec {
    int64_t seq = 0;
    int lane = -1;
    int ran_lane = -1;
    int first = 0, n = 0;
    int slots = 0;
    lm_status status = LM_OK;
    std::string err;
    int pack = -1;
    LmPackHdr ph{};
    std::vector<const char*> t_names;
    std::vector<double> t_ms, t_t0, t_t1;
    int32_t work[4] = {-1, -1, -1, -1};
  };
  std::deque<BatchRec> queue;
  BatchRec delivered;
  int last_lane = -1;
  int64_t nsub = 0;
  bool have_state = false;
  int last_frame = -1;
  int last_bb[3] = {0, 0, 0};
};

namespace {


struct ModelDets {
  const lm_detector* p[LM_NDET];
  const lm_detector* operator[](int d) const { return p[d]; }
};
// ... 33 lines not shown
    for (int i = 0; i < 256; ++i) {
      const float v = P->gray_value_transformation[i];
      if (!(v >= 0.f && v <= 255.f && v == std::floor(v)))
        throw std::invalid_argument("gray_value_transformation: a CV_8U table holds integers 0..255.");
    }
  }
  if (P->occlusion_grid_spacing_pixels_bottom <= 0) throw std::invalid_argument("occlusion_grid_spacing_pixels_bottom must be > 0.");
  if (!su->background || !su->ind_warp_mapping) throw std::invalid_argument("background / calibration missing.");
  if (su->video_rows <= 0 || su->video_cols <= 0 || su->calib_rows <= 0 || su->calib_cols <= 0)
    throw std::invalid_argument("empty video or calibration.");
  if (su->method < 0 || su->method > 2) throw std::invalid_argument("method must be 0, 1 or 2.");
  const int64_t nv = (int64_t)su->video_rows * su->video_cols;
  const int64_t nc = (int64_t)su->calib_rows * su->calib_cols;
  int32_t mn = INT32_MAX, mx = INT32_MIN;
  for (int64_t i = 0; i < nc; ++i) {
    mn = std::min(mn, su->ind_warp_mapping[i]);
    mx = std::max(mx, su->ind_warp_mapping[i]);
  }
  if (mn < 0 || mx >= nv) throw std::runtime_error("Calibration mapping indices out of range.");
  const int NR = su->calib_rows, NC = su->calib_cols;
  const lm_rect ub = P->bounding_box_bottom, us = P->bounding_box_side;
  if (ub.x < 0 || ub.y < 0 || ub.x + ub.width >= NC || ub.y + ub.height >= NR)
    throw std::runtime_error("Provided bounding box for the bottom view exceeds the image dimensions.");
  if (us.x < 0 || us.y < 0 || us.x + us.width >= NC || us.y + us.height >= NR)
    throw std::runtime_error("Provided bounding box for the side view exceeds the image dimensions.");
  if (ub.width <= 0 || ub.height <= 0 || us.width <= 0 || us.height <= 0)
    throw std::runtime_error("Empty mouse bounding box: cropBoundingBox / filter2D would work on an empty image.");
  const ModelDets dets = model_dets(M);
  const char* names[6] = {"modelPaw_bottom", "modelSnout_bottom", "modelTail_bottom", "modelPaw_side", "modelSnout_side", "modelTail_side"};
  for (int d = 0; d < 6; ++d) {
    if (!dets[d]->weights || dets[d]->rows <= 0 || dets[d]->cols <= 0)
      throw std::invalid_argument(std::string("Error: ") + names[d] + " cannot be empty.");
    if ((size_t)(LM_TH + 1) * pk_stride(LM_TW + dets[d]->cols + LM_JC) * sizeof(float) > kCorrLdsBudget)
      throw std::invalid_argument(std::string(names[d]) + ": detector too wide for the correlation window.");
    if (su->corr_precision == LM_CORR_F16 &&
        (f16_nch(dets[d]->cols) > LM_F16_MAX_NCH || f16_lds_bytes(f16_nch(dets[d]->cols), dets[d]->rows) > kF16LdsMax))
      throw std::invalid_argument(std::string(names[d]) + ": detector too large for the f16 correlation (LM_CORR_F16).");
  }
  if (su->corr_precision != LM_CORR_FP32 && su->corr_precision != LM_CORR_F16)
    throw std::invalid_argument("corr_precision must be LM_CORR_FP32 or LM_CORR_F16.");
}

LmTileSwitches read_switches(lm_ctx* c, const lm_setup* su) {
  auto flag = [](const char* name, bool dflt) {
    const char* v = getenv(name);
    return v ? atoi(v) != 0 : dflt;
  };
  c->kprof_on = flag("LM_KPROF", false);
  c->dark_on = flag("LM_CORR_DARK", true);
  c->tb_refine = flag("LM_TILE_REFINE", true);
  c->tb_screen = flag("LM_TILE_SCREEN", true);
  c->tb_ref = flag("LM_TILE_BOUND_REF", false);
  c->corr_dir_on = flag("LM_CORR_DIR", true);
  LmTileSwitches sw;
  sw.tailskip = flag("LM_CORR_TAILSKIP", true);
  sw.pointskip = flag("LM_CORR_POINTSKIP", true);
  sw.refine = c->tb_refine;
  sw.screen = c->tb_screen;
  sw.f16 = su->corr_precision == LM_CORR_F16;
  sw.dark = c->dark_on;
  return sw;
}

lm_geometry make_geometry(const lm_setup* su, const lm_params* P, const lm_model* M) {
  const int NR = su->calib_rows, NC = su->calib_cols;
  const lm_rect ub = P->bounding_box_bottom, us = P->bounding_box_side;
  lm_geometry g;
  std::memset(&g, 0, sizeof(g));
  g.n_rows = NR;
  g.n_cols = NC;
  const int mts_c = std::max(M->paw_side.cols, M->snout_side.cols), mts_r = std::max(M->paw_side.rows, M->snout_side.rows);
  const int mtb_c = std::max(M->paw_bottom.cols, M->snout_bottom.cols), mtb_r = std::max(M->paw_bottom.rows, M->snout_bottom.rows);
  g.spre_t_w = ceil_half(mts_c - 1);
  g.spre_t_h = ceil_half(mts_r - 1);
  g.spre_b_w = ceil_half(mtb_c - 1);
  g.spre_b_h = ceil_half(mtb_r - 1);
  g.spost_t_w = (mts_c - 1) / 2;
  g.spost_t_h = (mts_r - 1) / 2;
  g.spost_b_w = g.spre_b_w;
  g.spost_b_h = g.spre_b_h;
  g.bb_bottom_mouse = lm_rect{0, 0, ub.width, ub.height};
  g.bb_side_mouse = lm_rect{0, 0, us.width, us.height};
  g.pad_pre_rows = std::max({us.height, g.spre_t_h, g.spre_b_h});
  g.pad_post_rows = g.spost_b_h > g.spost_t_h ? g.spost_b_h : g.spost_t_h;
  g.pad_pre_cols = std::max({ub.width, g.spre_t_w, g.spre_b_w});
  g.pad_post_cols = g.spost_b_w > g.spost_t_w ? g.spost_b_w : g.spost_t_w;
  g.ipad_rows = g.pad_pre_rows + NR + g.pad_post_rows;
  g.ipad_cols = g.pad_pre_cols + NC + g.pad_post_cols;
  g.bb_bottom_mouse_pad = lm_rect{0, 0, g.spre_b_w + ub.width + g.spost_b_w, g.spre_b_h + ub.height + g.spost_b_h};
  g.bb_side_mouse_pad = lm_rect{0, 0, g.spre_t_w + us.width + g.spost_t_w, g.spre_t_h + us.height + g.spost_t_h};
  g.bb_unpad_mouse_bottom = lm_rect{g.spre_b_w, g.spre_b_h, ub.width, ub.height};
  g.bb_unpad_mouse_side = lm_rect{g.spre_t_w, g.spre_t_h, us.width, us.height};
  const int tw = (int)(unsigned)((int)(double)(ub.width) * P->tail_sub_bounding_box);
  g.tail_box_width = tw;
  g.bb_bottom_tail_pad = lm_rect{0, 0, tw + g.spre_b_w + g.spost_b_w, ub.height + g.spre_b_h + g.spost_b_h};
  g.bb_unpad_tail_bottom = lm_rect{g.spre_b_w, g.spre_b_h, tw, ub.height};
  g.bb_bottom_tail = lm_rect{0, 0, tw, ub.height};
  g.bb_side_tail_pad = lm_rect{0, 0, tw + g.spre_t_w + g.spost_t_w, us.height + g.spre_t_h + g.spost_t_h};
  g.bb_unpad_tail_side = lm_rect{g.spre_t_w, g.spre_t_h, tw, us.height};
  const int sp = P->occlusion_grid_spacing_pixels_bottom;
  g.ong_ny = (int)(unsigned)(((ub.height - sp) / sp) + 1);
  g.ong_nx = (int)(unsigned)(((P->occlusion_grid_max_width * ub.width) - sp) / sp + 1);
  g.ong_br_x = (double)(ub.width - 1 - sp / 2);
  g.ong_br_y = (double)(ub.height - 1 - sp / 2);
  const int sps = P->occlusion_grid_spacing_pixels_side;
  g.n_ong_side = sps > 0 ? (int)(unsigned)(((us.height - sps) / sps) + 1) : 0;
// ... 182 lines not shown
  K.ong_ny = g.ong_ny;
  K.ong_br_x = g.ong_br_x;
  K.ong_br_y = g.ong_br_y;
  K.bb_bottom_w = g.bb_bottom_mouse.width;
  K.bb_bottom_h = g.bb_bottom_mouse.height;
  K.spre_b_w = g.spre_b_w;
  K.spre_b_h = g.spre_b_h;
  K.spre_t_w = g.spre_t_w;
  K.spre_t_h = g.spre_t_h;
  const lm_rect mb[2] = {g.match_box_paw_bottom, g.match_box_snout_bottom};
  const lm_rect ms[2] = {g.match_box_paw_side, g.match_box_snout_side};
  for (int f = 0; f < 2; ++f) {
    K.match_b[f][0] = mb[f].x;
    K.match_b[f][1] = mb[f].y;
    K.match_b[f][2] = mb[f].width;
    K.match_b[f][3] = mb[f].height;
    K.match_s[f][0] = ms[f].x;
    K.match_s[f][1] = ms[f].y;
    K.match_s[f][2] = ms[f].width;
    K.match_s[f][3] = ms[f].height;
    const lm_detector& db = f == 0 ? M->paw_bottom : M->snout_bottom;
    const lm_detector& ds = f == 0 ? M->paw_side : M->snout_side;
    K.size_b[f][0] = db.cols;
    K.size_b[f][1] = db.rows;
    K.size_s[f][0] = ds.cols;
    K.size_s[f][1] = ds.rows;
  }
  for (int k = 0; k < 5; ++k) {
    const lm_location_prior& q = P->location_prior[k];
    const double row[7] = {q.x, q.y, q.max_distance, q.min_x, q.max_x, q.min_y, q.max_y};
    for (int j = 0; j < 7; ++j) K.prior[k][j] = row[j];
  }
  K.gray_lut_on = P->transform_gray_values && !P->use_reference_image_brightness ? 1 : 0;
  for (int i = 0; i < 256; ++i) K.gray_lut[i] = K.gray_lut_on ? (uint8_t)P->gray_value_transformation[i] : (uint8_t)i;
}

void slot_sizes(lm_ctx* c) {
  LmConst& K = c->K;
  c->ext_slot_bytes = ((int64_t)K.ext_h[0] * K.ext_w[0] + (int64_t)K.ext_h[1] * K.ext_w[1] + 255) / 256 * 256;
  K.tail_nw = 2 * ((K.tail_w + 63) / 64);
  K.tail_bm_words = (K.tail_hb + K.tail_hs) * K.tail_nw;
  c->tailbin_slot_bytes = (int64_t)K.tail_bm_words * 4;
  int64_t doff = 0;
  for (int d = 0; d < 6; ++d) {
    c->dbg_off[d] = doff;
    doff += (int64_t)K.det[d].oh * K.det[d].ow;
  }
  c->dbg_slot_floats = doff;
  int np = 1;
  while (np < std::max(K.list_cap[0], K.list_cap[2])) np <<= 1;
  c->gscratch_slot = std::max(3 * (int64_t)np, (5 * (int64_t)np + K.ong_nx * K.ong_ny + 2) / 2 + 1);
}

void build_corr_plans(lm_ctx* c, const lm_setup* su) {
  LmConst& K = c->K;
  c->unfused = su->filter_arith == LM_FILTER_UNFUSED;
  int order[6] = {0, 1, 2, 3, 4, 5};
  std::stable_sort(order, order + 6, [&](int x, int y) {
    return (int64_t)(K.det[x].kh + 2) * K.det[x].kw > (int64_t)(K.det[y].kh + 2) * K.det[y].kw;
  });
  for (int m = 0; m < 2; ++m) {
    lm_ctx::CorrPlan& P = c->corr_plan[m];
    P = lm_ctx::CorrPlan{};
    for (int oi = 0; oi < 6; ++oi) {
      const int d = order[oi];
      LmDet& D = K.det[d];
      const bool f16 = su->corr_precision == LM_CORR_F16;
      const bool ring = !f16 && corr_ring(D.kw_ring) && D.kh >= 2;
      const void* fn = f16     ? corr_kernel_f16(D.kw)
                       : !ring ? corr_kernel_gen(c->unfused)
                       : m == 1 && rw_all_width(D.kw_ring) ? corr_kernel_rw_all(c->unfused)
                                                           : corr_kernel(D.kw_ring, c->unfused);
      size_t need;
      if (f16) {
        D.chunk_rows = D.kh;
        need = f16_lds_bytes(f16_nch(D.kw), D.kh);
      } else if (ring) {
        D.chunk_rows = D.kh;
        need = corr_rw_lds(D.kw_ring);
      } else {
        const size_t row = (size_t)pk_stride(LM_TW + D.kwp - 1) * sizeof(float);
        D.chunk_rows = std::max(1, std::min(D.kh, (int)(kCorrLdsBudget / row) - (LM_TH - 1)));
        need = (size_t)(LM_TH + D.chunk_rows - 1) * row;
      }
      size_t gi = 0;
      while (gi < P.groups.size() && P.groups[gi].first != fn) ++gi;
      if (gi == P.groups.size()) {
        LmDetGroup G;
        std::memset(&G, 0, sizeof(G));
        P.groups.push_back({fn, G});
        P.lds.push_back(0);
        P.threads.push_back(f16 ? LM_F16_THREADS : ring ? LM_RW_THREADS : LM_CORR_THREADS);
        P.ring.push_back(ring);
      }
      LmDetGroup& G = P.groups[gi].second;
      const int prev = G.n ? G.tile_end[G.n - 1] : 0;
      G.ids[G.n] = d;
      G.tile_end[G.n] = prev + D.tiles_x * D.tiles_y;
      ++G.n;
      if (ring) G.ring_floats = std::max(G.ring_floats, rw_ring_floats(D.kw_ring));
      P.lds[gi] = std::max(P.lds[gi], need);
    }
  }
}

std::vector<float> pad_weights(const LmConst& K, const lm_model* M, int w_off) {
// ... 25 lines not shown
      for (int i = 0; i < D.kh; ++i)
        for (int c = 0; c < nch; ++c)
          for (int l = 0; l < 64; ++l)
            for (int j = 0; j < 8; ++j)
              w16.push_back((_Float16)std::ldexp(f16_bfrag_weight(dets[d]->weights, D.kw, i, c, l, j), sc));
    }
  }
  return w16;
}

void imadjust_table(uint8_t (&adj)[256]) {
  double low_in = 0 * 255, high_in = 0.6 * 255, low_out = 0 * 255, high_out = 1 * 255.0;
  double range_in = high_in - low_in, range_out = high_out - low_out, range_div = range_out / range_in;
  for (int i = 0; i < 256; ++i) {
    double temp;
    if (i <= low_in) temp = 0;
    else if (i >= high_in) temp = range_out;
    else temp = (i - low_in) * (range_div);
    adj[i] = (uint8_t)std::round((temp + low_out));
  }
}

void upload_constants(lm_ctx* c, const lm_setup* su, const std::vector<float>& wts, const std::vector<double>& tbc,
                      const std::vector<_Float16>& w16, const uint8_t (&adj)[256]) {
  const int64_t nv = (int64_t)su->video_rows * su->video_cols;
  const int64_t nc = (int64_t)su->calib_rows * su->calib_cols;
  hipStream_t cs = nullptr;
  HIPCHK(hipStreamCreateWithFlags(&cs, hipStreamNonBlocking));
  struct StreamGuard {
    hipStream_t s;
    ~StreamGuard() { (void)hipStreamDestroy(s); }
  } cs_guard{cs};
  c->bkg.alloc(nv);
  COPY_SYNC(c->bkg.p, su->background, nv, hipMemcpyHostToDevice, cs);
  c->cal.alloc(nc);
  COPY_SYNC(c->cal.p, su->ind_warp_mapping, nc * sizeof(int32_t), hipMemcpyHostToDevice, cs);
  c->weights.alloc(wts.size());
  COPY_SYNC(c->weights.p, wts.data(), wts.size() * sizeof(float), hipMemcpyHostToDevice, cs);
  c->tb_const.alloc(tbc.size());
  COPY_SYNC(c->tb_const.p, tbc.data(), tbc.size() * sizeof(double), hipMemcpyHostToDevice, cs);
  c->tbs_fallback.alloc(1);
  SET_SYNC(c->tbs_fallback.p, 0, sizeof(unsigned long long), cs);
  if (!w16.empty()) {
    c->weights16.alloc(w16.size());
    COPY_SYNC(c->weights16.p, w16.data(), w16.size() * sizeof(_Float16), hipMemcpyHostToDevice, cs);
  }
  c->adj.alloc(256);
  COPY_SYNC(c->adj.p, adj, 256, hipMemcpyHostToDevice, cs);
  c->dK.alloc(1);
  COPY_SYNC(c->dK.p, &c->K, sizeof(LmConst), hipMemcpyHostToDevice, cs);
  c->fstride = (nv + 255) / 256 * 256;
  HIPCHK(hipFuncSetAttribute((const void*)k_tail<false>, hipFuncAttributeMaxDynamicSharedMemorySize, (int)c->tail_lds));
  HIPCHK(hipFuncSetAttribute((const void*)k_tile_bound_ref, hipFuncAttributeMaxDynamicSharedMemorySize, (int)c->tb_lds));
  HIPCHK(hipFuncSetAttribute((const void*)k_tile_bound<false>, hipFuncAttributeMaxDynamicSharedMemorySize, (int)c->tbw_lds));
  HIPCHK(hipFuncSetAttribute((const void*)k_tile_bound<true>, hipFuncAttributeMaxDynamicSharedMemorySize, (int)c->tbw_lds));
  for (const auto& P : c->corr_plan)
    for (size_t g = 0; g < P.groups.size(); ++g)
      HIPCHK(hipFuncSetAttribute(P.groups[g].first, hipFuncAttributeMaxDynamicSharedMemorySize, (int)P.lds[g]));
}

void validate_and_build(lm_ctx* c, const lm_setup* su, const lm_params* P, const lm_model* M) {
  check_inputs(su, P, M);
  const LmTileSwitches sw = read_switches(c, su);
  c->setup = *su;
  c->params = *P;
  c->geo = make_geometry(su, P, M);
  const lm_geometry& g = c->geo;
  const lm_rect ub = P->bounding_box_bottom, us = P->bounding_box_side;
  c->bb_x = ub.x + ub.width;
  c->bb_ys = us.y + us.height;
  c->bb_yb = ub.y + ub.height;
  c->npix = (int)((int64_t)su->video_rows * su->video_cols);

  LmConst& K = c->K;
  std::memset(&K, 0, sizeof(K));
  const int w_off = fill_detectors(K, g, su, M);
  fill_image_constants(K, g, su, P);
  fill_flag_grid(K, c->nslots);
  plan_tail_lds(c, g);
  fill_list_and_cost_constants(K, g, P, M);
  slot_sizes(c);
  build_corr_plans(c, su);
  const std::vector<float> wts = pad_weights(K, M, w_off);
  const LmTilePlan plan = lm_tile_plan(K, c->nslots, wts.data(), sw);
  c->tailskip_on = plan.tailskip;
  c->pointskip_on = plan.pointskip;
  c->tb_lds = plan.tb_lds;
  c->tbw_lds = plan.tbw_lds;
  c->tbw_row_loop = plan.row_loop;
  const std::vector<_Float16> w16 = f16_fragments(K, su, M);
  uint8_t adj[256];
  imadjust_table(adj);
  upload_constants(c, su, wts, plan.tbc, w16, adj);
}


void lane_alloc(lm_ctx* c, Lane& L) {
  const LmConst& K = c->K;
  const lm_geometry& g = c->geo;
  const int ns = c->nslots;
  const int64_t fstride = c->fstride;
  hipStream_t st = L.stream;
  L.frames.alloc((size_t)fstride * ns);
  L.halo.alloc(fstride);
  SET_SYNC(L.halo.p, 0, fstride, st);
  L.luts.alloc((size_t)256 * ns);
  L.mm.alloc((size_t)2 * LM_MM_SPLIT * ns);
  L.ext.alloc((size_t)c->ext_slot_bytes * ns + (size_t)(LM_F16_TH + 16) * std::max(K.ext_w[0], K.ext_w[1]) + 64);
  L.tailbin.alloc((size_t)c->tailbin_slot_bytes * ns);
  SET_SYNC(L.tailbin.p, 0, (size_t)c->tailbin_slot_bytes * ns, st);
  L.tailmask.alloc((size_t)K.tail_hb * ((K.tail_w + 63) / 64) * ns);
  L.tscratch.alloc((size_t)5 * std::max(K.tail_hb, K.tail_hs) * ((K.tail_w + 1) / 2) * ns);
  if (c->tail_big) L.tail_ws.alloc((size_t)c->tail_ws_slot * ns);
  L.keys.alloc((size_t)K.keys_per_slot * ns);
  L.npos.alloc((size_t)LM_NLIST * ns);
  {
    const int64_t nchunks = ((int64_t)K.ext_h[0] * K.ext_w[0] + (int64_t)K.ext_h[1] * K.ext_w[1]) / LM_INGEST_VEC;
    L.smap.alloc((size_t)nchunks);
    L.sbkg.alloc((size_t)nchunks);
    L.skey.alloc(4);
    SET_SYNC(L.skey.p, 0x80, 4 * sizeof(int32_t), st);
  }
  if (c->dark_on) {
    L.dark_flags.alloc((size_t)K.fl_slot * ns);
    SET_SYNC(L.dark_flags.p, 0, (size_t)K.fl_slot * ns, st);
    L.dark_list.alloc((size_t)2 * K.tl_stride);
    L.dark_cnt.alloc(4 * LM_TL_NC);
    L.h_cnt.alloc(4 * LM_TL_NC);
  }
  if (c->tailskip_on) {
    L.tail_flags.alloc((size_t)K.tt_slot * ns);
    SET_SYNC(L.tail_flags.p, 0, (size_t)K.tt_slot * ns, st);
    L.tail_list.alloc((size_t)2 * K.tt_stride);
    L.tail_cnt.alloc(2 * LM_TL_NC);
    SET_SYNC(L.tail_cnt.p, 0, 2 * LM_TL_NC * sizeof(int32_t), st);
  }
  if (c->pointskip_on) {
    L.pt_flags.alloc((size_t)2 * K.pt_plane);
    SET_SYNC(L.pt_flags.p, 0, (size_t)2 * K.pt_plane, st);
    L.pt_list.alloc((size_t)LM_NLIST * K.tl_stride);
    L.pt_cnt.alloc(2 * LM_NLIST * LM_TL_NC);
    SET_SYNC(L.pt_cnt.p, 0, 2 * LM_NLIST * LM_TL_NC * sizeof(int32_t), st);
  }
  if ((c->tailskip_on || c->pointskip_on) && !c->tb_ref) {
    L.rng.alloc((size_t)(c->ext_slot_bytes / LM_INGEST_VEC) * ns);
    SET_SYNC(L.rng.p, 0, (size_t)(c->ext_slot_bytes / LM_INGEST_VEC) * ns * sizeof(uint32_t), st);
  }
  L.err.alloc(16);
  if (c->corr_dir_on) {
    L.corr_dir.alloc(LM_NDET);
    SET_SYNC(L.corr_dir.p, 0, LM_NDET * sizeof(LmCorrDirRec), st);
  }
  L.frame_ptr.alloc(ns);
  L.slots.alloc(ns);
  L.h_slots.alloc(ns);
  L.h_frame_ptr.alloc(ns);
  L.h_ctl.alloc(1);
  L.h_ph.alloc(1);
  L.zero_ph.alloc(1);
  SET_SYNC(L.zero_ph.p, 0, sizeof(LmPackHdr), st);
  L.h_err.alloc(16);
  int cap[AR_COUNT];
  cap[AR_CAND] = ns * LM_NLIST * 64;
  cap[AR_P22D] = ns * LM_NFEAT * 64;
  cap[AR_SIDE] = ns * LM_NFEAT * 256;
  cap[AR_UNARY] = ns * LM_NFEAT * 64 * 4;
  cap[AR_PWJC] = ns * LM_NFEAT * (64 + g.ong_nx * g.ong_ny + 1);
  cap[AR_PWNZ] = ns * LM_NFEAT * (1024 + g.ong_nx * g.ong_ny);
  for (int a = 0; a < 2; ++a) L.arena[a].alloc(cap, ns);
  HIPCHK(hipEventCreateWithFlags(&L.ev_snap, hipEventDisableTiming));
  HIPCHK(hipEventCreateWithFlags(&L.ev_consumed, hipEventDisableTiming));
  HIPCHK(hipEventCreateWithFlags(&L.ev_done, hipEventDisableTiming | hipEventBlockingSync));
}

std::mutex g_epoch_mu;
std::map<int, hipEvent_t> g_epoch;

hipEvent_t epoch_event(const lm_ctx* c) {
  std::lock_guard<std::mutex> lk(g_epoch_mu);
  auto it = g_epoch.find(c->device);
  return it == g_epoch.end() ? nullptr : it->second;
}


struct Timer {
  Lane& L;
  bool on;
  Timer(lm_ctx* c, Lane& l) : L(l), on(c->debug & 2) {}
  hipEvent_t pool(size_t i) {
    while (L.ev_pool.size() <= i) {
      hipEvent_t e;
      HIPCHK(hipEventCreate(&e));
      L.ev_pool.push_back(e);
    }
    return L.ev_pool[i];
  }
  bool capturing = false;
  void record(hipEvent_t e) {
    const hipError_t r = hipEventRecord(e, L.stream);
    if (r != hipSuccess && !capturing) hip_check(r, "hipEventRecord");
// ... 189 lines not shown
            nb, nb ? life / nb : 0.0, nb ? wlife / nb : 0.0, (t_max - t_min) * 0.01, s_max * 0.01);
    for (int k = 1; k < 13; ++k)
      if (cnt[k]) fprintf(stderr, " p%d=%.0f", k, acc[k] / cnt[k]);
    fprintf(stderr, "\n");
  }
}

void dump_slot(lm_ctx* c, Lane& L, const char* dir, int frame, int slot, int feat) {
  const LmConst& K = c->K;
  std::vector<int32_t> np(LM_NLIST);
  COPY_SYNC(np.data(), L.npos.p + (int64_t)slot * LM_NLIST, LM_NLIST * sizeof(int32_t), hipMemcpyDeviceToHost, L.stream);
  LmSlotOut h;
  COPY_SYNC(&h, L.arena[L.parity].hdr.p + slot, sizeof(h), hipMemcpyDeviceToHost, L.stream);
  std::string path = std::string(dir) + "/dump_" + std::to_string(frame) + ".bin";
  FILE* f = fopen(path.c_str(), "wb");
  if (!f) return;
  int32_t hd[5 + 12] = {frame, slot, feat, np[0], np[1]};
  for (int l = 0; l < 4; ++l) {
    hd[5 + l] = h.n_pos[l];
    hd[9 + l] = h.cand_cnt[l];
    hd[13 + l] = h.ties[l];
  }
  fwrite(hd, sizeof(hd), 1, f);
  fwrite(np.data(), sizeof(int32_t), LM_NLIST, f);
  for (int l = 0; l < LM_NLIST; ++l) {
    std::vector<unsigned long long> kv((size_t)K.list_cap[l]);
    HIPCHK(hipMemcpy(kv.data(), L.keys.p + (int64_t)slot * K.keys_per_slot + K.list_off[l],
                     kv.size() * sizeof(unsigned long long), hipMemcpyDeviceToHost));
    fwrite(kv.data(), sizeof(unsigned long long), kv.size(), f);
  }
  fclose(f);
}

CorrDark lane_dark(const lm_ctx* c, Lane& L) {
  CorrDark d;
  if (c->dark_on) {
    d.flags = L.dark_flags.p;
    d.cnt = L.dark_cnt.p;
    d.list = L.dark_list.p;
  }
  if (c->tailskip_on) {
    d.tail_flags = L.tail_flags.p;
    d.tail_cnt = L.tail_cnt.p;
    d.tail_list = L.tail_list.p;
  }
  if (c->pointskip_on) {
    d.pt_flags = L.pt_flags.p;
    d.pt_cnt = L.pt_cnt.p;
    d.pt_list = L.pt_list.p;
  }
  return d;
}

void enqueue_chain(lm_ctx* c, Lane& L, Arena& A, const Lane::Pending& P, Timer& T, bool do_carry, int part) {
  const LmConst& K = c->K;
  const LmConst* dK = c->dK.p;
  hipStream_t st = L.stream;
  const int n = P.n, s_lut0 = P.s_lut0, s_proc0 = P.s_proc0;
  const int nproc = n + 1 - s_proc0;
  if (part <= 0) {
    k_prep<<<do_carry ? 2 : 1, 256, 0, st>>>(L.h_slots.d, L.h_frame_ptr.d, L.h_ctl.d, n + 1, L.slots.p, L.frame_ptr.p,
                                             A.ctl.p, L.npos.p, L.err.p, dK, L.keys.p, L.arena[P.prv].hdr.p, P.last_n,
                                             A.hdr.p, L.dark_cnt.p, L.tail_cnt.p, L.pt_cnt.p);
    T.begin("k_minmax");
    k_minmax<<<dim3(LM_MM_SPLIT, n + 1 - s_lut0), LM_MM_THREADS, 0, st>>>(L.frame_ptr.p, c->bkg.p, c->npix, s_lut0,
                                                                        L.mm.p);
    k_lut<<<(n + 1 - s_lut0 + 3) / 4, 256, 0, st>>>(L.mm.p, s_lut0, n + 1, c->adj.p, c->setup.method != 0, L.luts.p);
    T.end();
    T.begin("k_ingest");
    const CorrDark dk = lane_dark(c, L);
    long long* kpi = nullptr;
    const size_t ing_blocks = (size_t)(K.ing_nb[0] + K.ing_nb[1]) * ((c->nslots + LM_INGEST_FB - 1) / LM_INGEST_FB);
    if (c->kprof_on) {
      if (!L.kprof_ing.p) L.kprof_ing.alloc(16 * ing_blocks);
      HIPCHK(hipMemsetAsync(L.kprof_ing.p, 0, sizeof(long long) * 16 * ing_blocks, st));
      kpi = L.kprof_ing.p;
    }
    k_ingest<<<dim3((unsigned)(K.ing_nb[0] + K.ing_nb[1]), (unsigned)((nproc + LM_INGEST_FB - 1) / LM_INGEST_FB)),
               K.ing_threads, 0, st>>>(dK, L.frame_ptr.p, c->bkg.p, c->cal.p, L.luts.p, L.slots.p, s_proc0, n + 1, L.ext.p,
                                        c->ext_slot_bytes, reinterpret_cast<unsigned*>(L.tailbin.p), L.smap.p, L.sbkg.p,
                                        L.skey.p, dk.flags, dk.cnt, dk.list, L.rng.p, kpi);
    T.end();
    if (dk.tail_cnt || dk.pt_cnt) {
      T.begin("k_tile_bound");
      if (c->tb_ref)
        k_tile_bound_ref<<<dim3((unsigned)nproc, 2), LM_TB_THREADS, c->tb_lds, st>>>(
            dK, L.ext.p, c->ext_slot_bytes, s_proc0, c->tb_const.p, dk.flags, dk.tail_flags, dk.tail_cnt, dk.tail_list,
            dk.pt_flags, dk.pt_cnt, dk.pt_list);
      else
        (c->tbw_row_loop ? k_tile_bound<true> : k_tile_bound<false>)
            <<<dim3((unsigned)nproc, (unsigned)(K.tbw_nband[0] + K.tbw_nband[1])), LM_TB_THREADS, c->tbw_lds, st>>>(
                dK, L.rng.p, c->ext_slot_bytes / LM_INGEST_VEC, s_proc0, nproc, c->tb_const.p, dk.flags, dk.tail_flags,
                dk.tail_cnt, dk.tail_list, dk.pt_flags, dk.pt_cnt, dk.pt_list, c->tbs_fallback.p);
      T.end();
    }
    const lm_ctx::CorrPlan& CP = c->corr_plan[P.plan];
    if (c->corr_dir_on && std::find(CP.ring.begin(), CP.ring.end(), (char)1) != CP.ring.end()) {
      std::vector<LmDetGroup> groups;
      for (const auto& grp : CP.groups) groups.push_back(grp.second);
      HIPCHK(launch_corr_dir(st, dK, groups.data(), CP.ring.data(), (int)groups.size(), nproc, dk, L.corr_dir.p,
                             L.err.p));
    }
  }
  if (part == 1 || part < 0) {
    T.begin("k_corr");
    const lm_ctx::CorrPlan& CP = c->corr_plan[P.plan];
    for (size_t gi = 0; gi < CP.groups.size(); ++gi) {
      const auto& grp = CP.groups[gi];
      const LmDetGroup& G = grp.second;
      const void* w = c->setup.corr_precision == LM_CORR_F16 ? (const void*)c->weights16.p : (const void*)c->weights.p;
      HIPCHK(launch_corr(grp.first, CP.ring[gi], dim3(G.tile_end[G.n - 1], nproc), CP.threads[gi], CP.lds[gi], st, dK,
                         G, L.ext.p, c->ext_slot_bytes, w, s_proc0, L.keys.p, L.npos.p, L.tailbin.p,
                         c->tailbin_slot_bytes, lane_dark(c, L),
                         c->corr_dir_on && CP.ring[gi] ? L.corr_dir.p + gi : nullptr));
    }
    T.end();
  }
  if (part == 2 || part < 0) {
    if (c->debug & 1) {
      if (!L.dbg.p) {
        L.dbg.alloc((size_t)c->dbg_slot_floats * c->nslots);
        L.dbg_offd.alloc(LM_NDET);
        COPY_SYNC(L.dbg_offd.p, c->dbg_off, sizeof(c->dbg_off), hipMemcpyHostToDevice, st);
      }
      HIPCHK(launch_corr_dbg(c->unfused, dim3(64, nproc, LM_NDET), st, dK, L.ext.p, c->ext_slot_bytes, c->weights.p,
                             s_proc0, L.dbg.p, L.dbg_offd.p, c->dbg_slot_floats));
    }
    long long *kp0 = nullptr, *kp1 = nullptr, *kp2 = nullptr, *kp3 = nullptr;
    if (c->kprof_on) {
      if (!L.kprof.p) L.kprof.alloc((size_t)4 * 16 * 2 * c->nslots);
      HIPCHK(hipMemsetAsync(L.kprof.p, 0, sizeof(long long) * 4 * 16 * 2 * c->nslots, st));
      kp0 = L.kprof.p;
      kp1 = L.kprof.p + 16 * 2 * c->nslots;
      kp2 = L.kprof.p + 2 * 16 * 2 * c->nslots;
      kp3 = L.kprof.p + 3 * 16 * 2 * c->nslots;
    }
    T.begin("k_tail");
    if (c->tail_big)
      k_tail<true><<<nproc, LM_TAIL_THREADS, 0, st>>>(dK, s_proc0, L.tailbin.p, c->tailbin_slot_bytes, L.tailmask.p,
                                                      L.tscratch.p, A.hdr.p, kp2, L.tail_ws.p, c->tail_ws_slot,
                                                      L.keys.p, L.npos.p);
    else
      k_tail<false><<<nproc, LM_TAIL_THREADS, c->tail_lds, st>>>(dK, s_proc0, L.tailbin.p, c->tailbin_slot_bytes,
                                                                 L.tailmask.p, L.tscratch.p, A.hdr.p, kp2, nullptr, 0,
                                                                 L.keys.p, L.npos.p);
    T.end();
    T.begin("k_nms");
    k_nms<false><<<dim3(nproc, 4), LM_NMS_THREADS, 0, st>>>(dK, s_proc0, L.keys.p, L.npos.p, L.tailmask.p, L.gscratch.p,
                                                           c->gscratch_slot, A.hdr.p, L.err.p, kp0, kp1, 0);
    k_nms<true><<<LM_GLOB_BLOCKS, LM_NMS_THREADS, 0, st>>>(dK, s_proc0, L.keys.p, L.npos.p, L.tailmask.p, L.gscratch.p,
                                              c->gscratch_slot, A.hdr.p, L.err.p, nullptr, nullptr, 4 * nproc);
    T.end();
    T.begin("k_post");
    k_post<false><<<dim3(n, 2), LM_POST_THREADS, 0, st>>>(dK, L.slots.p, L.frame_ptr.p, c->bkg.p, c->cal.p, L.luts.p,
                                                         A.hdr.p, L.keys.p, A.p22d.p, A.side_y.p, A.side_s.p, A.unary.p,
                                                         A.jc.p, A.ir.p, A.pr.p, A.ctl.p, L.err.p, L.gscratch.p,
                                                         c->gscratch_slot, kp3, 0);
    k_post<true><<<LM_GLOB_BLOCKS, LM_POST_THREADS, 0, st>>>(dK, L.slots.p, L.frame_ptr.p, c->bkg.p, c->cal.p, L.luts.p, A.hdr.p,
                                                L.keys.p, A.p22d.p, A.side_y.p, A.side_s.p, A.unary.p, A.jc.p, A.ir.p,
                                                A.pr.p, A.ctl.p, L.err.p, L.gscratch.p, c->gscratch_slot, nullptr,
                                                2 * n);
    T.end();
    T.begin("k_pack");
    k_pack_scan<<<1, 1024, 0, st>>>(A.hdr.p, n, A.ctl.p, L.err.p, A.ph.p, A.pack.p, A.pack_cap, A.side_base.p);
    k_pack_copy<<<dim3(n, 2), 256, 0, st>>>(dK, A.hdr.p, n, L.keys.p, A.p22d.p, A.side_y.p, A.side_s.p, A.unary.p,
                                            A.jc.p, A.ir.p, A.pr.p, A.ph.p, A.pack.p, A.side_base.p);
    T.end();
    k_out<<<128, 256, 0, st>>>(A.ph.p, L.h_ph.d, A.pack.p, nullptr, 0, A.ctl.p, nullptr, L.frame_ptr.p, n, L.halo.p,
// ... 572 lines not shown
  const Lane* L = delivered_lane(ctx);
  if (!L) return fail(LM_ERR_INVALID_ARGUMENT, kLaneReused);
  if (const char* what = bad(*L)) return fail(LM_ERR_INVALID_ARGUMENT, what);
  return guarded([&] {
    HIPCHK(hipSetDevice(ctx->device));
    read(*L, [&](void* dst, const void* src, size_t bytes) {
      COPY_SYNC(dst, src, bytes, hipMemcpyDeviceToHost, L->stream);
    });
  });
}
const char* no_check(const Lane&) { return nullptr; }
}

LM_API lm_status lm_debug_scores(lm_ctx* ctx, int32_t f, int32_t det, float* out, int32_t rows, int32_t cols) {
  if (!ctx || !out) return fail(LM_ERR_INVALID_ARGUMENT, "null argument");
  const auto bad = [&](const Lane& L) -> const char* {
    if (!(ctx->debug & 1) || !L.dbg.p) return "debug scores not enabled";
    if (f < 0 || f >= L.batch_n || det < 0 || det >= LM_NDET) return "index out of range";
    if (rows != ctx->K.det[det].oh || cols != ctx->K.det[det].ow) return "shape mismatch";
    return nullptr;
  };
  return read_delivered(ctx, bad, [&](const Lane& L, auto fetch) {
    fetch(out, L.dbg.p + (int64_t)(f + 1) * ctx->dbg_slot_floats + ctx->dbg_off[det], sizeof(float) * rows * cols);
  });
}

LM_API lm_status lm_debug_tail_work(lm_ctx* ctx, int32_t* out) {
  if (!ctx || !out) return fail(LM_ERR_INVALID_ARGUMENT, "null argument");
  for (int k = 0; k < 4; ++k) out[k] = -1;
  if (!ctx->tailskip_on) return LM_OK;
  return read_delivered(ctx, no_check, [&](const Lane& L, auto fetch) {
    int32_t h[2 * LM_TL_NC];
    fetch(h, L.tail_cnt.p, sizeof(h));
    for (int t = 0; t < 2; ++t) {
      out[2 * t] = std::accumulate(h + t * LM_TL_NC, h + (t + 1) * LM_TL_NC, 0);
      out[2 * t + 1] = ctx->delivered.slots * ctx->K.tt_tx[t] * ctx->K.tt_ty[t];
    }
  });
}

LM_API lm_status lm_debug_screen_fallback(lm_ctx* ctx, int64_t* out) {
  if (!ctx || !out) return fail(LM_ERR_INVALID_ARGUMENT, "null argument");
  *out = 0;
  if (ctx->lanes.empty() || !ctx->tbs_fallback.p) return LM_OK;
  return guarded([&] {
    HIPCHK(hipSetDevice(ctx->device));
    for (const auto& L : ctx->lanes) HIPCHK(hipStreamSynchronize(L->stream));
    unsigned long long h = 0;
    COPY_SYNC(&h, ctx->tbs_fallback.p, sizeof(h), hipMemcpyDeviceToHost, ctx->lanes[0]->stream);
    *out = (int64_t)h;
  });
}

LM_API lm_status lm_debug_tail_tiles(lm_ctx* ctx, int32_t f, int32_t view, uint8_t* out, int32_t rows, int32_t cols) {
  if (!ctx || !out) return fail(LM_ERR_INVALID_ARGUMENT, "null argument");
  if (!ctx->tailskip_on) return fail(LM_ERR_INVALID_ARGUMENT, "tail-tile skipping is off");
  const auto bad = [&](const Lane& L) -> const char* {
    if (f < 0 || f >= L.batch_n || view < 0 || view > 1) return "index out of range";
    if (rows != ctx->K.tt_ty[view] || cols != ctx->K.tt_tx[view]) return "shape mismatch";
    return nullptr;
  };
  return read_delivered(ctx, bad, [&](const Lane& L, auto fetch) {
    fetch(out, L.tail_flags.p + (int64_t)(f + 1) * ctx->K.tt_slot + ctx->K.tt_off[view], (size_t)rows * cols);
  });
}

LM_API lm_status lm_debug_point_work(lm_ctx* ctx, int32_t* out) {
  if (!ctx || !out) return fail(LM_ERR_INVALID_ARGUMENT, "null argument");
  for (int k = 0; k < 2 * LM_NLIST; ++k) out[k] = -1;
  if (!ctx->pointskip_on) return LM_OK;
  return read_delivered(ctx, no_check, [&](const Lane& L, auto fetch) {
    int32_t h[2 * LM_NLIST * LM_TL_NC];
    fetch(h, L.pt_cnt.p, sizeof(h));
    for (int l = 0; l < LM_NLIST; ++l) {
      out[2 * l] = std::accumulate(h + l * LM_TL_NC, h + (l + 1) * LM_TL_NC, 0);
      out[2 * l + 1] = std::accumulate(h + (LM_NLIST + l) * LM_TL_NC, h + (LM_NLIST + l + 1) * LM_TL_NC, 0);
    }
  });
}

LM_API lm_status lm_debug_point_tiles(lm_ctx* ctx, int32_t f, int32_t det, uint8_t* out, int32_t rows, int32_t cols) {
  if (!ctx || !out) return fail(LM_ERR_INVALID_ARGUMENT, "null argument");
  if (!ctx->pointskip_on) return fail(LM_ERR_INVALID_ARGUMENT, "point-tile skipping is off");
  const auto bad = [&](const Lane& L) -> const char* {
    if (f < 0 || f >= L.batch_n || det < 0 || det >= LM_NDET || ctx->K.det[det].kind != 0) return "index out of range";
    const int view = ctx->K.det[det].view;
    if (rows != ctx->K.fl_ty[view] || cols != ctx->K.fl_tx[view]) return "shape mismatch";
    return nullptr;
  };
  return read_delivered(ctx, bad, [&](const Lane& L, auto fetch) {
    const int view = ctx->K.det[det].view, list = ctx->K.det[det].list;
    fetch(out, L.pt_flags.p + (list & 1) * ctx->K.pt_plane + (int64_t)(f + 1) * ctx->K.fl_slot + ctx->K.fl_off[view],
          (size_t)rows * cols);
  });
}

LM_API lm_status lm_debug_tail_mask(lm_ctx* ctx, int32_t f, uint8_t* out, int32_t rows, int32_t cols) {
  if (!ctx || !out) return fail(LM_ERR_INVALID_ARGUMENT, "null argument");
  const auto bad = [&](const Lane& L) -> const char* {
    if (f < 0 || f >= L.batch_n) return "index out of range";
    if (rows != ctx->K.tail_hb || cols != ctx->K.tail_w) return "shape mismatch";
    return nullptr;
  };
  return read_delivered(ctx, bad, [&](const Lane& L, auto fetch) {
    const int nb = (cols + 63) / 64;
    std::vector<unsigned long long> bits((size_t)rows * nb);
// ... 72 lines not shown
```

### locomouse_cpp_amd/runtime.py

```python
import ctypes as C
import os
import subprocess

import numpy as np

from .abi import (BB_FRAME_DTYPE, CALIB_RECORD_DTYPE, LM_ENC_GRAY8, LM_ENC_RGB24, LM_OK, lm_batch_result, lm_bb_result,
                  lm_calib_fit_result, lm_calib_opts, lm_calib_record, lm_enc_mark, lm_enc_overlay, lm_enc_result,
                  lm_enc_stats, lm_geometry, lm_jpeg_info, lm_jpeg_interval_stats, lm_jpeg_stats, lm_train_heldout,
                  lm_train_point, lm_train_problem, lm_train_stats, result_to_numpy)

PKG = os.path.dirname(os.path.abspath(__file__))
ROOT = os.path.dirname(PKG)
LIB_PATH = os.path.join(PKG, "liblocomouse_hip.so")
CSRC = os.path.join(PKG, "csrc")

EXPORTED = (
    "lm_abi_version", "lm_last_error", "lm_ctx_create", "lm_ctx_destroy", "lm_get_geometry", "lm_ctx_stream",
    "lm_detect_batch", "lm_detect_batch_device", "lm_ctx_set_debug", "lm_debug_scores", "lm_debug_tail_mask",
    "lm_debug_kernel_times", "lm_debug_kernel_spans", "lm_synth_frames_device",
    "lm_bb_create", "lm_bb_destroy", "lm_bb_push", "lm_bb_push_device", "lm_bb_finish", "lm_bb_debug_binary",
    "lm_bb_stream", "lm_host_alloc", "lm_host_free",
    "lm_detect_submit", "lm_detect_submit_device", "lm_detect_collect", "lm_ctx_lanes", "lm_ctx_pending",
    "lm_debug_corr_work", "lm_debug_batch_slots", "lm_debug_dark_tile_width",
    "lm_debug_dark_tile_height", "lm_debug_tail_work", "lm_debug_tail_tiles", "lm_debug_point_work",
    "lm_debug_point_tiles", "lm_debug_screen_fallback",
)

HIPCC_FLAGS = ["--offload-arch=gfx950", "-O3", "-std=c++17", "-fPIC", "-shared", "-ffp-contract=off", "-fno-slp-vectorize",
               "-fvisibility=hidden", "-Wall", "-Wno-unused-function", "-Wno-unused-variable"]


HOST_DIR = os.path.join(PKG, "host")
HOST_LIB_PATH = os.path.join(PKG, "liblocomouse_host.so")
CLI_PATH = os.path.join(PKG, "bin", "LocoMouse")


HIP_UNITS = ("lm_runtime.hip", "lm_corr.hip", "lm_bbox.hip", "lm_jpeg.hip", "lm_bkg.hip", "lm_jpeg_enc.hip",
             "lm_train.hip", "lm_calib.hip")

JPEG_EXPORTED = ("lm_jpeg_create", "lm_jpeg_destroy", "lm_jpeg_decode_device", "lm_jpeg_probe", "lm_jpeg_stream",
                 "lm_jpeg_debug_stats", "lm_jpeg_device_alloc", "lm_jpeg_device_free", "lm_jpeg_upload",
                 "lm_jpeg_set_interval_path", "lm_jpeg_debug_interval_stats")

BKG_EXPORTED = ("lm_bkg_create", "lm_bkg_destroy", "lm_bkg_push", "lm_bkg_push_device", "lm_bkg_finish",
                "lm_bkg_reset", "lm_bkg_samples", "lm_bkg_stream")
BKG_CLI_PATH = os.path.join(PKG, "bin", "LocoMouseBackground")

ENC_EXPORTED = ("lm_enc_slot_bytes", "lm_enc_slot_bytes_restart", "lm_enc_create", "lm_enc_create_restart", "lm_enc_destroy",
                "lm_enc_encode_device", "lm_enc_encode", "lm_enc_set_overlay", "lm_enc_render_encode_device", "lm_enc_render_encode", "lm_enc_render_device", "lm_enc_stream",
                "lm_enc_last_stats")

TRAIN_EXPORTED = ("lm_train_create", "lm_train_destroy", "lm_train_add_patches", "lm_train_gather",
                  "lm_train_gather_device", "lm_train_samples", "lm_train_reset", "lm_train_patches", "lm_train_solve",
                  "lm_train_margins", "lm_train_stream", "lm_train_set_groups", "lm_train_solve_many",
                  "lm_train_problem_block")
TRAIN_CLI_PATH = os.path.join(PKG, "bin", "LocoMouseTrain")
TRANSCODE_CLI_PATH = os.path.join(PKG, "bin", "LocoMouseTranscode")

CALIB_EXPORTED = ("lm_calib_default_opts", "lm_calib_create", "lm_calib_destroy", "lm_calib_set_background", "lm_calib_push",
                  "lm_calib_push_device", "lm_calib_frames", "lm_calib_read", "lm_calib_reset", "lm_calib_stream",
                  "lm_calib_fit", "lm_calib_map")
CALIB_CLI_PATH = os.path.join(PKG, "bin", "LocoMouseCalibrate")


def _up_to_date(obj, cmd):
    try:
        with open(obj + ".cmd") as fh:
            if fh.read() != " ".join(cmd):
                return False
        with open(obj + ".d") as fh:
            deps = fh.read().replace("\\\n", " ").split(":", 1)[1].split()
        t = os.path.getmtime(obj)
        return all(os.path.getmtime(d) <= t for d in deps)
    except (OSError, IndexError):
        return False


def build(verbose=False, defines=(), out=None):
# ... 59 lines not shown
        print(" ".join(cmd))
    subprocess.check_call(cmd)
    cmd = [*flags, "-o", CALIB_CLI_PATH, os.path.join(HOST_DIR, "CalibrateCli.cpp"), "-L" + PKG, "-llocomouse_host",
           "-llocomouse_hip", "-Wl,-rpath,$ORIGIN/.."]
    if verbose:
        print(" ".join(cmd))
    subprocess.check_call(cmd)
    return HOST_LIB_PATH


_lib = None


def lib():
    global _lib
    if _lib is None:
        try:
            import torch
        except ImportError:
            pass
        if not os.path.exists(LIB_PATH):
            raise RuntimeError(f"{LIB_PATH} is missing: run locomouse_cpp_amd.runtime.build() (no CPU fallback)")
        L = C.CDLL(LIB_PATH)
        L.lm_abi_version.restype = C.c_int32
        L.lm_last_error.restype = C.c_char_p
        L.lm_ctx_create.argtypes = [C.c_int32, C.c_void_p, C.c_void_p, C.c_void_p, C.c_int32, C.POINTER(C.c_void_p)]
        L.lm_ctx_destroy.argtypes = [C.c_void_p]
        L.lm_get_geometry.argtypes = [C.c_void_p, C.POINTER(lm_geometry)]
        L.lm_ctx_stream.argtypes = [C.c_void_p]
        L.lm_ctx_stream.restype = C.c_void_p
        for fn in (L.lm_detect_batch, L.lm_detect_batch_device):
            fn.argtypes = [C.c_void_p, C.c_void_p, C.c_int64, C.c_int32, C.c_int32, C.c_void_p, C.c_void_p,
                           C.POINTER(lm_batch_result)]
        for fn in (L.lm_detect_submit, L.lm_detect_submit_device):
            fn.argtypes = [C.c_void_p, C.c_void_p, C.c_int64, C.c_int32, C.c_int32, C.c_void_p, C.c_void_p]
        L.lm_detect_collect.argtypes = [C.c_void_p, C.POINTER(lm_batch_result)]
        for fn in (L.lm_ctx_lanes, L.lm_ctx_pending):
            fn.argtypes = [C.c_void_p]
            fn.restype = C.c_int32
        L.lm_ctx_set_debug.argtypes = [C.c_void_p, C.c_int32]
        L.lm_debug_scores.argtypes = [C.c_void_p, C.c_int32, C.c_int32, C.c_void_p, C.c_int32, C.c_int32]
        L.lm_debug_tail_mask.argtypes = [C.c_void_p, C.c_int32, C.c_void_p, C.c_int32, C.c_int32]
        L.lm_debug_kernel_times.argtypes = [C.c_void_p, C.POINTER(C.c_char_p), C.POINTER(C.c_double), C.c_int32]
        L.lm_debug_kernel_times.restype = C.c_int32
        L.lm_debug_kernel_spans.argtypes = [C.c_void_p, C.POINTER(C.c_char_p), C.POINTER(C.c_double),
                                            C.POINTER(C.c_double), C.c_int32]
        L.lm_debug_kernel_spans.restype = C.c_int32
        L.lm_debug_corr_work.argtypes = [C.c_void_p, C.POINTER(C.c_int32)]
        L.lm_debug_tail_work.argtypes = [C.c_void_p, C.POINTER(C.c_int32)]
        L.lm_debug_tail_tiles.argtypes = [C.c_void_p, C.c_int32, C.c_int32, C.c_void_p, C.c_int32, C.c_int32]
        L.lm_debug_point_work.argtypes = [C.c_void_p, C.POINTER(C.c_int32)]
        L.lm_debug_point_tiles.argtypes = [C.c_void_p, C.c_int32, C.c_int32, C.c_void_p, C.c_int32, C.c_int32]
        L.lm_debug_screen_fallback.argtypes = [C.c_void_p, C.POINTER(C.c_int64)]
        L.lm_debug_batch_slots.argtypes = [C.c_void_p]
        L.lm_debug_batch_slots.restype = C.c_int32
        L.lm_synth_frames_device.argtypes = [C.c_int32, C.c_void_p, C.c_int32, C.c_int32, C.c_int64, C.c_int32,
                                             C.c_int64]
        L.lm_bb_create.argtypes = [C.c_int32, C.c_void_p, C.c_void_p, C.c_int32, C.POINTER(C.c_void_p)]
        L.lm_bb_destroy.argtypes = [C.c_void_p]
        for fn in (L.lm_bb_push, L.lm_bb_push_device):
            fn.argtypes = [C.c_void_p, C.c_void_p, C.c_int64, C.c_int32, C.c_void_p]
        L.lm_bb_finish.argtypes = [C.c_void_p, C.POINTER(lm_bb_result)]
        L.lm_bb_debug_binary.argtypes = [C.c_void_p, C.c_int32, C.c_void_p, C.c_int32, C.c_int32]
        L.lm_host_alloc.argtypes = [C.c_size_t, C.POINTER(C.c_void_p)]
        L.lm_host_free.argtypes = [C.c_void_p]
        L.lm_bb_stream.argtypes = [C.c_void_p]
        L.lm_bb_stream.restype = C.c_void_p
        L.lm_jpeg_create.argtypes = [C.c_int32, C.c_int32, C.c_int32, C.c_int32, C.c_int32, C.POINTER(C.c_void_p)]
        L.lm_jpeg_destroy.argtypes = [C.c_void_p]
        L.lm_jpeg_decode_device.argtypes = [C.c_void_p, C.POINTER(C.c_char_p), C.POINTER(C.c_size_t), C.c_int32,
                                            C.c_void_p, C.c_int64, C.POINTER(C.c_int32)]
        L.lm_jpeg_probe.argtypes = [C.c_char_p, C.c_size_t, C.POINTER(lm_jpeg_info)]
        L.lm_jpeg_stream.argtypes = [C.c_void_p]
        L.lm_jpeg_stream.restype = C.c_void_p
        L.lm_jpeg_debug_stats.argtypes = [C.c_void_p, C.POINTER(lm_jpeg_stats)]
        L.lm_jpeg_set_interval_path.argtypes = [C.c_void_p, C.c_int32]
        L.lm_jpeg_debug_interval_stats.argtypes = [C.c_void_p, C.POINTER(lm_jpeg_interval_stats)]
        L.lm_bkg_create.argtypes = [C.c_int32, C.c_int32, C.c_int32, C.c_int32, C.POINTER(C.c_void_p)]
        L.lm_bkg_destroy.argtypes = [C.c_void_p]
        for fn in (L.lm_bkg_push, L.lm_bkg_push_device):
            fn.argtypes = [C.c_void_p, C.c_void_p, C.c_int64, C.c_int32]
        L.lm_bkg_finish.argtypes = [C.c_void_p, C.c_int32, C.c_void_p]
        L.lm_bkg_reset.argtypes = [C.c_void_p]
        L.lm_bkg_samples.argtypes = [C.c_void_p]
        L.lm_bkg_samples.restype = C.c_int64
        L.lm_bkg_stream.argtypes = [C.c_void_p]
        L.lm_bkg_stream.restype = C.c_void_p
        L.lm_enc_slot_bytes.argtypes = [C.c_int32, C.c_int32, C.c_int32]
        L.lm_enc_slot_bytes.restype = C.c_int64
        L.lm_enc_create.argtypes = [C.c_int32, C.c_int32, C.c_int32, C.c_int32, C.c_int32, C.c_int32, C.POINTER(C.c_void_p)]
        L.lm_enc_slot_bytes_restart.argtypes = [C.c_int32, C.c_int32, C.c_int32, C.c_int32]
        L.lm_enc_slot_bytes_restart.restype = C.c_int64
        L.lm_enc_create_restart.argtypes = [C.c_int32, C.c_int32, C.c_int32, C.c_int32, C.c_int32, C.c_int32, C.c_int32,
                                            C.POINTER(C.c_void_p)]
        L.lm_enc_destroy.argtypes = [C.c_void_p]
        for fn in (L.lm_enc_encode_device, L.lm_enc_encode):
            fn.argtypes = [C.c_void_p, C.c_void_p, C.c_int64, C.c_int32, C.POINTER(lm_enc_result)]
        L.lm_enc_set_overlay.argtypes = [C.c_void_p, C.POINTER(lm_enc_overlay)]
        for fn in (L.lm_enc_render_encode_device, L.lm_enc_render_encode):
            fn.argtypes = [C.c_void_p, C.c_void_p, C.c_int64, C.c_int32, C.c_void_p, C.c_void_p, C.POINTER(lm_enc_result)]
        L.lm_enc_render_device.argtypes = [C.c_void_p, C.c_void_p, C.c_int64, C.c_int32, C.c_void_p, C.c_void_p, C.c_void_p]
        L.lm_enc_stream.argtypes = [C.c_void_p]
        L.lm_enc_stream.restype = C.c_void_p
        L.lm_enc_last_stats.argtypes = [C.c_void_p, C.POINTER(lm_enc_stats)]
        L.lm_train_create.argtypes = [C.c_int32, C.c_int32, C.c_int32, C.c_int32, C.POINTER(C.c_void_p)]
        L.lm_train_destroy.argtypes = [C.c_void_p]
# ... 128 lines not shown
    def detect_device(self, d_frames_ptr, pitch, n, first_frame, d_prev_ptr=None, bb=None, raw=True):
        res = lm_batch_result()
        bbp = None
        if bb is not None:
            self._bb = np.ascontiguousarray(bb, dtype=np.int32)
            bbp = self._bb.ctypes.data
        _check(lib().lm_detect_batch_device(self._h, C.c_void_p(d_frames_ptr), pitch, n, first_frame,
                                            C.c_void_p(d_prev_ptr) if d_prev_ptr else None, bbp, C.byref(res)))
        return res if raw else result_to_numpy(res)

    def debug_scores(self, f, det):
        g = self.geometry()
        shapes = {0: (g.bb_bottom_mouse.height, g.bb_bottom_mouse.width), 1: (g.bb_bottom_mouse.height, g.bb_bottom_mouse.width),
                  2: (g.bb_bottom_mouse.height, g.tail_box_width), 3: (g.bb_side_mouse.height, g.bb_side_mouse.width),
                  4: (g.bb_side_mouse.height, g.bb_side_mouse.width), 5: (g.bb_side_mouse.height, g.tail_box_width)}
        out = np.zeros(shapes[det], dtype=np.float32)
        _check(lib().lm_debug_scores(self._h, f, det, out.ctypes.data, out.shape[0], out.shape[1]))
        return out

    def debug_tail_mask(self, f):
        g = self.geometry()
        out = np.zeros((g.bb_bottom_mouse.height, g.tail_box_width), dtype=np.uint8)
        _check(lib().lm_debug_tail_mask(self._h, f, out.ctypes.data, out.shape[0], out.shape[1]))
        return out

    def kernel_times(self):
        names = (C.c_char_p * 64)()
        ms = (C.c_double * 64)()
        n = lib().lm_debug_kernel_times(self._h, names, ms, 64)
        return [(names[i].decode(), ms[i]) for i in range(min(n, 64))]

    def kernel_spans(self):
        names = (C.c_char_p * 64)()
        t0 = (C.c_double * 64)()
        t1 = (C.c_double * 64)()
        n = lib().lm_debug_kernel_spans(self._h, names, t0, t1, 64)
        return [(names[i].decode(), t0[i], t1[i]) for i in range(min(n, 64))]

    def corr_work(self):
        out = (C.c_int32 * 4)()
        _check(lib().lm_debug_corr_work(self._h, out))
        return None if out[0] < 0 else {"tiles": (out[0], out[1]), "outputs": (out[2], out[3])}

    def tail_work(self):
        out = (C.c_int32 * 4)()
        _check(lib().lm_debug_tail_work(self._h, out))
        return None if out[0] < 0 else {"listed": (out[0], out[2]), "total": (out[1], out[3])}

    def screen_fallback(self):
        out = C.c_int64(0)
        _check(lib().lm_debug_screen_fallback(self._h, C.byref(out)))
        return int(out.value)

    def tail_tiles(self, f, view):
        g = self.geometry()
        tw, th = self.dark_tile_shape()
        oh = (g.bb_side_mouse if view else g.bb_bottom_mouse).height
        out = np.zeros((-(-oh // th), -(-g.tail_box_width // tw)), dtype=np.uint8)
        _check(lib().lm_debug_tail_tiles(self._h, f, view, out.ctypes.data, out.shape[0], out.shape[1]))
        return out

    def point_work(self):
        out = (C.c_int32 * 8)()
        _check(lib().lm_debug_point_work(self._h, out))
        return None if out[0] < 0 else {"listed": tuple(out[0:8:2]), "bright": tuple(out[1:8:2])}

    def point_tiles(self, f, det):
        g = self.geometry()
        tw, th = self.dark_tile_shape()
        box = g.bb_side_mouse if det >= 3 else g.bb_bottom_mouse
        out = np.zeros((-(-box.height // th), -(-box.width // tw)), dtype=np.uint8)
        _check(lib().lm_debug_point_tiles(self._h, f, det, out.ctypes.data, out.shape[0], out.shape[1]))
        return out

    def batch_slots(self):
        return lib().lm_debug_batch_slots(self._h)

    @staticmethod
    def dark_tile_shape():
        L = lib()
        return int(L.lm_debug_dark_tile_width()), int(L.lm_debug_dark_tile_height())

    def close(self):
        if getattr(self, "_h", None) and self._h.value:
            lib().lm_ctx_destroy(self._h)
            self._h = C.c_void_p()

    def __del__(self):
        try:
            self.close()
        except Exception:
            pass


class BBContext:

    def __init__(self, setup, bb_params, max_batch=64, device=0):
        self._setup, self._params = setup, bb_params
        self._h = C.c_void_p()
        _check(lib().lm_bb_create(device, C.byref(setup), C.byref(bb_params), max_batch, C.byref(self._h)))
        self.max_batch = max_batch
        self.rows, self.cols = setup.calib_rows, setup.calib_cols

    def push(self, frames):
        frames = np.ascontiguousarray(frames, dtype=np.uint8)
        out = np.zeros(frames.shape[0], dtype=BB_FRAME_DTYPE)
# ... 428 lines not shown
```

Measured before the change: 957,900.

## Add narrow-width work items to the ring correlation path for partially active tiles

Adds a narrow work class: the tile-bound kernel emits lists of narrow (sub-tile width) entries covering only the active columns of tiles. New k_corr_rwn kernels then run the ring correlation at the narrower width with per-entry owned column ranges, plus a directory kernel to map waves to entries. The aim is to avoid computing full 40-wide sub-tiles when only part of each is bright or active. The cost is extra list-building work and atomics, more kernel launches, and a large set of new kernel instantiations.

```diff
diff --git a/include/locomouse_hip.h b/include/locomouse_hip.h
--- a/include/locomouse_hip.h
+++ b/include/locomouse_hip.h
@@ -185,6 +185,9 @@
 
 lm_status lm_debug_screen_fallback(lm_ctx* ctx, int64_t* out);
 
+lm_status lm_debug_narrow_work(lm_ctx* ctx, int32_t* out);
+lm_status lm_debug_narrow_entries(lm_ctx* ctx, int32_t det, int32_t narrow, uint64_t* out, int32_t cap, int32_t* n);
+
 lm_status lm_debug_tail_tiles(lm_ctx* ctx, int32_t f, int32_t view, uint8_t* out, int32_t rows, int32_t cols);
 
 lm_status lm_debug_point_work(lm_ctx* ctx, int32_t* out);
diff --git a/locomouse_cpp_amd/abi.py b/locomouse_cpp_amd/abi.py
--- a/locomouse_cpp_amd/abi.py
+++ b/locomouse_cpp_amd/abi.py
@@ -10,6 +10,12 @@
 LM_CORR_FP32, LM_CORR_F16 = 0, 1
 LM_DEPTH_8U, LM_DEPTH_32F, LM_DEPTH_64F = 0, 5, 6
 DETECTORS = ("paw_bottom", "snout_bottom", "tail_bottom", "paw_side", "snout_side", "tail_side")
+
+
+def narrow_entry_fields(entries):
+    e = np.asarray(entries, dtype=np.uint64)
+    lo, hi = (e & np.uint64(0xFFFFFFFF)).astype(np.int64), (e >> np.uint64(32)).astype(np.int64)
+    return np.stack([lo >> 16, lo & 0xFFFF, hi & 15, (hi >> 4) & 15], axis=1).reshape(-1, 4)
 
 
 class lm_rect(C.Structure):
diff --git a/locomouse_cpp_amd/csrc/lm_corr.h b/locomouse_cpp_amd/csrc/lm_corr.h
--- a/locomouse_cpp_amd/csrc/lm_corr.h
+++ b/locomouse_cpp_amd/csrc/lm_corr.h
@@ -6,6 +6,7 @@
 #include <stdint.h>
 
 #include "lm_corr_dir.h"
+#include "lm_corr_narrow.h"
 #include "lm_device.h"
 
 #define LM_CORR_THREADS 192
@@ -53,13 +54,22 @@
 #endif
 static_assert(LM_RW_HSLOTS >= (LM_FH == 4 ? 3 : 7), "k_corr_rw ring: rows live during a step");
 
-__host__ __device__ constexpr int rw_stride(int kw) { return (LM_FW + kw - 1 + 3 + 3) / 4 * 4; }
-__host__ __device__ constexpr int rw_qpitch(int kw) {
-  return (LM_RW_HSLOTS + 1) * rw_stride(kw) +
-         ((LM_FW / 5 - ((LM_RW_HSLOTS + 1) * rw_stride(kw)) % 32) + 32) % 32;
+__host__ __device__ constexpr int rw_stride(int kw, int fw = LM_FW) { return (fw + kw - 1 + 3 + 3) / 4 * 4; }
+__host__ __device__ constexpr int rw_qpitch(int kw, int fw = LM_FW) {
+  return fw == LM_FW ? (LM_RW_HSLOTS + 1) * rw_stride(kw) +
+                           ((LM_FW / 5 - ((LM_RW_HSLOTS + 1) * rw_stride(kw)) % 32) + 32) % 32
+                     : (LM_RW_HSLOTS + 1) * rw_stride(kw, fw) + ((4 - ((LM_RW_HSLOTS + 1) * rw_stride(kw, fw)) % 8) + 8) % 8;
 }
-__host__ __device__ constexpr int rw_ring_floats(int kw) { return LM_RW_NQ * rw_qpitch(kw); }
+__host__ __device__ constexpr int rw_nq(int fw = LM_FW) { return fw == LM_FW ? LM_RW_NQ : 64 / (fw / 5); }
+__host__ __device__ constexpr int rw_ring_floats(int kw, int fw = LM_FW) { return rw_nq(fw) * rw_qpitch(kw, fw); }
+#if defined(LM_KW_ONLY) || defined(LM_KW_C3)
+#define LM_KW_LIST_N LM_KW_LIST
+#else
+#define LM_KW_LIST_N(X) \
+  X(16) X(17) X(18) X(19) X(20) X(21) X(22) X(23) X(24) X(25) X(26) X(27) X(28) X(29) X(30) X(31) X(32) X(36) X(40)
+#endif
 size_t corr_rw_lds(int kw);
+size_t corr_rwn_lds(int kw);
 
 #define LM_F16_WAVES 4
 #define LM_F16_TW 128
@@ -83,6 +93,9 @@
 const void* corr_kernel(int kw, bool unf);
 const void* corr_kernel_gen(bool unf);
 const void* corr_kernel_rw_all(bool unf);
+bool corr_narrow_width(int kw);
+const void* corr_kernel_n(int kw, bool unf);
+const void* corr_kernel_n_all(bool unf);
 const void* corr_kernel_f16(int kw);
 struct CorrDark {
   uint8_t* flags = nullptr;
@@ -95,6 +108,12 @@
   int32_t* pt_cnt = nullptr;
   uint32_t* pt_list = nullptr;
 };
+hipError_t launch_corr_n(const void* fn, int nslots, size_t lds, hipStream_t st, const LmConst* K, const LmDetGroup& G,
+                         const uint8_t* ext, int64_t ext_slot_bytes, const void* weights, unsigned long long* keys,
+                         int32_t* n_pos, uint8_t* tailbin, int64_t tailbin_slot_bytes, const int32_t* nw_cnt,
+                         const unsigned long long* nw_list, const LmCorrDirRecN* dir);
+hipError_t launch_corr_dir_n(hipStream_t st, const LmDetGroup* groups, int ngroups, int nslots, const int32_t* nw_cnt,
+                             LmCorrDirRecN* out, int32_t* err);
 hipError_t launch_corr(const void* fn, bool ring, dim3 grid, int threads, size_t lds, hipStream_t st, const LmConst* K,
                        const LmDetGroup& G, const uint8_t* ext, int64_t ext_slot_bytes, const void* weights, int s0,
                        unsigned long long* keys, int32_t* n_pos, uint8_t* tailbin, int64_t tailbin_slot_bytes,
diff --git a/locomouse_cpp_amd/csrc/lm_corr.hip b/locomouse_cpp_amd/csrc/lm_corr.hip
--- a/locomouse_cpp_amd/csrc/lm_corr.hip
+++ b/locomouse_cpp_amd/csrc/lm_corr.hip
@@ -168,6 +168,23 @@
       y = oy + (i / LM_RW_NQX) * LM_FH;
       x = ox + (i % LM_RW_NQX) * LM_FW;
     }
+  }
+};
+struct RwRunN {
+  const unsigned long long* l;
+  int nvalid;
+  int ftx;
+  DEV unsigned long long entry(int i) const { return l[min(i, nvalid - 1)]; }
+  DEV void tile(int, unsigned long long e, int& s, int& y, int& x) const {
+    const uint32_t t = lm_nw_entry_tile(e);
+    const int lt = (int)(t & 0xFFFFu);
+    s = (int)(t >> 16);
+    y = (lt / ftx) * LM_FH;
+    x = (lt % ftx) * LM_FW + lm_nw_origin(lm_nw_entry_first(e));
+  }
+  DEV void owned(unsigned long long e, int ow, int& x0, int& x1) const {
+    const int lt = (int)(lm_nw_entry_tile(e) & 0xFFFFu);
+    lm_nw_owned((lt % ftx) * LM_FW, lm_nw_entry_first(e), lm_nw_entry_count(e), ow, &x0, &x1);
   }
 };
 
@@ -407,10 +424,10 @@
 #undef LM_RW_S0
 #undef LM_RW_S1
 
-template <int KW, bool UNF>
+template <int KW, bool UNF, int FW = LM_FW>
 struct RwPipe {
   using P = RwPlan<KW>;
-  static constexpr int STR = rw_stride(KW);
+  static constexpr int STR = rw_stride(KW, FW);
   lm_f2 px[PK_C + KW - 1];
   lm_f2 acc[2][PK_C];
   lm_f2 wa[P::PMAX], wb[P::PMAX];
@@ -498,14 +515,15 @@
   const uint32_t* tt_list;
 };
 
-template <int KW, bool UNF>
-DEV __attribute__((always_inline)) void rw_tile(const RwArgs& A, int dix, const RwRun& R, float* ring) {
-  constexpr int NQ = LM_RW_NQ;
-  constexpr int QX = LM_FW / PK_C;
-  static_assert(LM_FH == PK_R && QX * NQ == 64, "one row of 8 lanes per 40 x 4 sub-tile");
-  constexpr int STR = rw_stride(KW);
-  constexpr int QP = rw_qpitch(KW);
-  constexpr int NL = (3 + LM_FW + KW - 1 + 3) / 4;
+template <int KW, bool UNF, int FW = LM_FW, class RUN = RwRun>
+DEV __attribute__((always_inline)) void rw_tile(const RwArgs& A, int dix, const RUN& R, float* ring) {
+  constexpr bool NARROW = FW != LM_FW;
+  constexpr int NQ = rw_nq(FW);
+  constexpr int QX = FW / PK_C;
+  static_assert(LM_FH == PK_R && QX * NQ == 64, "one row of FW / 5 lanes per FW x 4 work item (8 per 40 x 4 sub-tile, 4 per narrow item)");
+  constexpr int STR = rw_stride(KW, FW);
+  constexpr int QP = rw_qpitch(KW, FW);
+  constexpr int NL = (3 + FW + KW - 1 + 3) / 4;
   constexpr int NLD = (NQ * NL + 63) / 64;
   static_assert(NLD <= 4, "window rows wider than four loads per lane");
   constexpr int HS = LM_RW_HSLOTS;
@@ -606,7 +624,7 @@
   auto row_base = [&](int t) -> unsigned {
     return ring_lane + (unsigned)__builtin_amdgcn_readfirstlane((t % HS) * STR * (int)sizeof(float));
   };
-  RwPipe<KW, UNF> S;
+  RwPipe<KW, UNF, FW> S;
 #pragma unroll
   for (int p = 0; p < 2; ++p)
 #pragma unroll
@@ -644,17 +662,36 @@
 
   unsigned bits = 0;
   if (valid) {
+    int own0 = 0, own1 = D.ow;
+    if constexpr (NARROW) R.owned(R.entry(q), D.ow, own0, own1);
 #pragma unroll
     for (int p = 0; p < PK_R / 2; ++p)
 #pragma unroll
       for (int c = 0; c < PK_C; ++c) {
         const int x = ox0 + lx * PK_C + c;
         const int y0 = oy0 + 2 * p;
-        if (x < D.ow && y0 < D.oh && S.acc[p][c].x > 0.0f) bits |= 1u << ((2 * p) * PK_C + c);
-        if (x < D.ow && y0 + 1 < D.oh && S.acc[p][c].y > 0.0f) bits |= 1u << ((2 * p + 1) * PK_C + c);
-      }
-  }
-  if (D.kind != 0) {
+        const bool in = NARROW ? x >= own0 && x < own1 : x < D.ow;
+        if (in && y0 < D.oh && S.acc[p][c].x > 0.0f) bits |= 1u << ((2 * p) * PK_C + c);
+        if (in && y0 + 1 < D.oh && S.acc[p][c].y > 0.0f) bits |= 1u << ((2 * p + 1) * PK_C + c);
+      }
+  }
+  if constexpr (NARROW) {
+    if (D.kind != 0) {
+      unsigned* __restrict__ tb = reinterpret_cast<unsigned*>(A.tailbin + (int64_t)slot * A.tailbin_slot_bytes) +
+                                  (D.list ? (int64_t)K.tail_hb * K.tail_nw : 0);
+#pragma unroll
+      for (int r = 0; r < PK_R; ++r)
+#pragma unroll
+        for (int c = 0; c < PK_C; ++c)
+          if (bits & (1u << (r * PK_C + c))) {
+            const int x = ox0 + lx * PK_C + c, y = oy0 + r;
+            if ((x >> 5) < K.tail_nw) atomicOr(&tb[(int64_t)y * K.tail_nw + (x >> 5)], 1u << (x & 31));
+          }
+      return;
+    }
+  }
+  if constexpr (!NARROW) {
+   if (D.kind != 0) {
     constexpr int WPS = QX / LM_FH;
     static_assert(WPS * LM_FH == QX && (LM_FW == 40 ? WPS == 2 : WPS == 4), "a sub-tile's bitmap words, one per lane");
     unsigned* s_tb = reinterpret_cast<unsigned*>(ring);
@@ -676,6 +713,7 @@
     const int y = oy0 + lx / WPS, gw = w0 + lx % WPS;
     if (v && y < D.oh && gw < K.tail_nw) atomicOr(&tb[(int64_t)y * K.tail_nw + gw], v);
     return;
+   }
   }
   bits &= mbits;
   const int cnt = __popc(bits);
@@ -768,6 +806,120 @@
 #define LM_KW_CASE(n)           \
   case n:                       \
     rw_tile<n, UNF>(a, d, R, ring); \
+    break;
+    LM_KW_LIST_RW_ALL(LM_KW_CASE)
+#undef LM_KW_CASE
+    default:
+      break;
+  }
+}
+
+DEV bool corr_locate_n(const LmConst& K, const LmDetGroup& G, int nslots, int g, const int32_t* __restrict__ ncnt,
+                       const unsigned long long* __restrict__ nlist, const LmCorrDirRecN* __restrict__ dir, int& d,
+                       RwRunN& R) {
+  const int lane = threadIdx.x & 63;
+  int k = 0, local = 0;
+  if (dir) {
+    typedef int32_t lm_i8 __attribute__((ext_vector_type(8)));
+    const lm_i8 rv = *reinterpret_cast<const lm_i8*>(dir);
+    const LmCorrDirRecN rec{{rv[0], rv[1], rv[2], rv[3], rv[4], rv[5]}, rv[6], rv[7]};
+    if (!lm_nw_lookup(rec, G.n, g, &k, &local)) return false;
+  } else {
+    int base = 0;
+    bool found = false;
+#pragma unroll
+    for (int kk = 0; kk < LM_NDET; ++kk) {
+      if (kk >= G.n || found) continue;
+      const int wv = lm_nw_seg_waves(ncnt[LM_NW_CNT_N + G.ids[kk] * LM_TL_NC + lane]);
+      const int tot = __builtin_amdgcn_readlane(corr_scan_waves(wv), 63);
+      if (g < base + tot) {
+        k = kk;
+        local = g - base;
+        found = true;
+      }
+      base += tot;
+    }
+    if (!found) return false;
+  }
+  const int dk = G.ids[k];
+  const LmDet& D = K.det[dk];
+  const int cn = ncnt[LM_NW_CNT_N + dk * LM_TL_NC + lane];
+  const int wv = lm_nw_seg_waves(cn);
+  const int P = corr_scan_waves(wv);
+  const int c = __builtin_amdgcn_readfirstlane(__ffsll((long long)__ballot(P > local)) - 1);
+  const int w = local - (__builtin_amdgcn_readlane(P, c) - __builtin_amdgcn_readlane(wv, c));
+  const bool pt = D.kind == 0;
+  const int v = pt ? D.view : D.list;
+  const int ftx = pt ? K.fl_tx[v] : K.tt_tx[v], ntile = ftx * (pt ? K.fl_ty[v] : K.tt_ty[v]);
+  const int ng = (nslots + LM_INGEST_FB - 1) / LM_INGEST_FB;
+  const unsigned long long* lst =
+      nlist + (pt ? (int64_t)D.list * K.tl_stride : (int64_t)LM_NLIST * K.tl_stride + (int64_t)v * K.tt_stride);
+  d = dk;
+  R = RwRunN{lst + (int64_t)lm_tl_y0(c, ng) * LM_INGEST_FB * ntile + LM_NW_NQ * w,
+             min(LM_NW_NQ, __builtin_amdgcn_readlane(cn, c) - LM_NW_NQ * w), ftx};
+  return true;
+}
+
+struct LmCorrDirGroupsN {
+  int32_t n;
+  int32_t grid[LM_NDET];
+  LmDetGroup g[LM_NDET];
+};
+__global__ __launch_bounds__(64) void k_corr_dirn(const LmCorrDirGroupsN A, const int32_t* __restrict__ ncnt,
+                                                   LmCorrDirRecN* __restrict__ out, int32_t* __restrict__ err) {
+  const int b = blockIdx.x;
+  const LmDetGroup& G = A.g[b];
+  const int lane = threadIdx.x;
+  int32_t waves[LM_NDET];
+#pragma unroll
+  for (int k = 0; k < LM_NDET; ++k) {
+    waves[k] = 0;
+    if (k < G.n)
+      waves[k] = __builtin_amdgcn_readlane(corr_scan_waves(lm_nw_seg_waves(ncnt[LM_NW_CNT_N + G.ids[k] * LM_TL_NC + lane])), 63);
+  }
+  if (lane == 0) {
+    const LmCorrDirRecN rec = lm_nw_record(waves, G.n);
+    out[b] = rec;
+    if (rec.total > A.grid[b]) atomicOr(err, LM_DEVERR_CORR_DIR);
+  }
+}
+
+#define LM_RWN_WPE 3
+template <int KW, bool UNF>
+__global__ __launch_bounds__(LM_RW_THREADS) __attribute__((amdgpu_waves_per_eu(KW <= 32 ? LM_RWN_WPE : 1, 8))) void k_corr_rwn(
+    const LmConst* __restrict__ Kp, const LmDetGroup G, const uint8_t* __restrict__ ext, int64_t ext_slot_bytes,
+    const float* __restrict__ weights, int nslots, unsigned long long* __restrict__ keys, int32_t* __restrict__ n_pos,
+    uint8_t* __restrict__ tailbin, int64_t tailbin_slot_bytes, const int32_t* __restrict__ ncnt,
+    const unsigned long long* __restrict__ nlist, const LmCorrDirRecN* __restrict__ dir) {
+  extern __shared__ uint4 lds_rw[];
+  const int wave = __builtin_amdgcn_readfirstlane(threadIdx.x >> 6);
+  float* ring = reinterpret_cast<float*>(lds_rw) + wave * rw_ring_floats(KW, LM_NW_FW);
+  const RwArgs a{Kp, G, ext, ext_slot_bytes, weights, 0, nslots, keys, n_pos, tailbin, tailbin_slot_bytes,
+                 nullptr, nullptr, 0, nullptr, nullptr};
+  int d;
+  RwRunN R;
+  if (!corr_locate_n(*a.K, G, nslots, xcd_block(blockIdx.x, gridDim.x) * LM_RW_WAVES + wave, ncnt, nlist, dir, d, R)) return;
+  rw_tile<KW, UNF, LM_NW_FW, RwRunN>(a, d, R, ring);
+}
+
+template <bool UNF>
+__global__ __launch_bounds__(LM_RW_THREADS) __attribute__((amdgpu_waves_per_eu(LM_RWN_WPE, 8))) void k_corr_rwn_all(
+    const LmConst* __restrict__ Kp, const LmDetGroup G, const uint8_t* __restrict__ ext, int64_t ext_slot_bytes,
+    const float* __restrict__ weights, int nslots, unsigned long long* __restrict__ keys, int32_t* __restrict__ n_pos,
+    uint8_t* __restrict__ tailbin, int64_t tailbin_slot_bytes, const int32_t* __restrict__ ncnt,
+    const unsigned long long* __restrict__ nlist, const LmCorrDirRecN* __restrict__ dir) {
+  extern __shared__ uint4 lds_rw[];
+  const int wave = __builtin_amdgcn_readfirstlane(threadIdx.x >> 6);
+  float* ring = reinterpret_cast<float*>(lds_rw) + wave * G.ring_floats;
+  const RwArgs a{Kp, G, ext, ext_slot_bytes, weights, 0, nslots, keys, n_pos, tailbin, tailbin_slot_bytes,
+                 nullptr, nullptr, 0, nullptr, nullptr};
+  int d;
+  RwRunN R;
+  if (!corr_locate_n(*a.K, G, nslots, xcd_block(blockIdx.x, gridDim.x) * LM_RW_WAVES + wave, ncnt, nlist, dir, d, R)) return;
+  switch (a.K->det[d].kw_ring) {
+#define LM_KW_CASE(n)                                   \
+  case n:                                               \
+    rw_tile<n, UNF, LM_NW_FW, RwRunN>(a, d, R, ring); \
     break;
     LM_KW_LIST_RW_ALL(LM_KW_CASE)
 #undef LM_KW_CASE
@@ -1100,6 +1252,58 @@
 }
 
 size_t corr_rw_lds(int kw) { return (size_t)LM_RW_WAVES * rw_ring_floats(kw) * sizeof(float); }
+size_t corr_rwn_lds(int kw) { return (size_t)LM_RW_WAVES * rw_ring_floats(kw, LM_NW_FW) * sizeof(float); }
+
+bool corr_narrow_width(int kw) {
+  switch (kw) {
+#define LM_KW_CASE(n) case n:
+    LM_KW_LIST_N(LM_KW_CASE)
+#undef LM_KW_CASE
+    return true;
+    default:
+      return false;
+  }
+}
+
+const void* corr_kernel_n(int kw, bool unf) {
+  switch (kw) {
+#define LM_KW_CASE(n) \
+  case n:             \
+    return unf ? (const void*)&k_corr_rwn<n, true> : (const void*)&k_corr_rwn<n, false>;
+    LM_KW_LIST_N(LM_KW_CASE)
+#undef LM_KW_CASE
+    default:
+      return nullptr;
+  }
+}
+
+const void* corr_kernel_n_all(bool unf) {
+  return unf ? (const void*)&k_corr_rwn_all<true> : (const void*)&k_corr_rwn_all<false>;
+}
+
+hipError_t launch_corr_n(const void* fn, int nslots, size_t lds, hipStream_t st, const LmConst* K, const LmDetGroup& G,
+                         const uint8_t* ext, int64_t ext_slot_bytes, const void* weights, unsigned long long* keys,
+                         int32_t* n_pos, uint8_t* tailbin, int64_t tailbin_slot_bytes, const int32_t* nw_cnt,
+                         const unsigned long long* nw_list, const LmCorrDirRecN* dir) {
+  const unsigned waves = (unsigned)lm_nw_grid_waves(G.tile_end[G.n - 1], nslots, G.n);
+  void* args[] = {(void*)&K,    (void*)&G,     (void*)&ext,     (void*)&ext_slot_bytes,     (void*)&weights,
+                  (void*)&nslots, (void*)&keys, (void*)&n_pos,   (void*)&tailbin, (void*)&tailbin_slot_bytes,
+                  (void*)&nw_cnt, (void*)&nw_list, (void*)&dir};
+  return hipLaunchKernel(fn, dim3((waves + LM_RW_WAVES - 1) / LM_RW_WAVES), dim3(LM_RW_THREADS), args, lds, st);
+}
+
+hipError_t launch_corr_dir_n(hipStream_t st, const LmDetGroup* groups, int ngroups, int nslots, const int32_t* nw_cnt,
+                             LmCorrDirRecN* out, int32_t* err) {
+  if (ngroups < 1 || ngroups > LM_NDET) return hipErrorInvalidValue;
+  LmCorrDirGroupsN A{};
+  A.n = ngroups;
+  for (int b = 0; b < ngroups; ++b) {
+    A.g[b] = groups[b];
+    A.grid[b] = lm_nw_grid_waves(groups[b].tile_end[groups[b].n - 1], nslots, groups[b].n);
+  }
+  k_corr_dirn<<<ngroups, 64, 0, st>>>(A, nw_cnt, out, err);
+  return hipGetLastError();
+}
 
 const void* corr_kernel_gen(bool unf) { return unf ? (const void*)&k_corr_gen<true> : (const void*)&k_corr_gen<false>; }
 
diff --git a/locomouse_cpp_amd/csrc/lm_corr_narrow.h b/locomouse_cpp_amd/csrc/lm_corr_narrow.h
--- /dev/null
+++ b/locomouse_cpp_amd/csrc/lm_corr_narrow.h
@@ -0,0 +1,129 @@
+#ifndef LM_CORR_NARROW_H
+#define LM_CORR_NARROW_H
+
+#include <stdint.h>
+
+#include "lm_device.h"
+
+#define LM_NW_FW 20
+#define LM_NW_NQ (64 / (LM_NW_FW / 5))
+#define LM_NW_BLK 8
+#define LM_NW_NBX (LM_FW / LM_NW_BLK)
+#define LM_NW_SPAN 2
+#define LM_NW_UNTRIED 0x20u
+static_assert(LM_NW_SPAN * LM_NW_BLK <= LM_NW_FW && LM_NW_FW % 5 == 0 && (LM_FW - LM_NW_FW) % 4 == 0, "narrow item geometry");
+
+#define LM_NW_FN LM_HD inline __attribute__((always_inline))
+
+struct LmNwClass {
+  int narrow;
+  int first;
+  int count;
+};
+
+LM_NW_FN LmNwClass lm_nw_classify(uint32_t mask) {
+  LmNwClass c{0, 0, 0};
+  const uint32_t m = mask & ((1u << LM_NW_NBX) - 1u);
+  if ((mask & LM_NW_UNTRIED) != 0u || m == 0u) return c;
+  int first = 0, last = LM_NW_NBX - 1;
+  while (!(m >> first & 1u)) ++first;
+  while (!(m >> last & 1u)) --last;
+  if (last - first + 1 > LM_NW_SPAN) return c;
+  c.narrow = 1;
+  c.first = first;
+  c.count = last - first + 1;
+  return c;
+}
+
+template <class F>
+LM_NW_FN uint32_t lm_nw_mask_of(int nblocks, bool tried, F unproven) {
+  uint32_t m = 0u;
+  for (int b = 0; b < nblocks && b < LM_NW_NBX; ++b)
+    if (unproven(b)) m |= (1u << b) | (tried ? 0u : LM_NW_UNTRIED);
+  return m;
+}
+
+LM_NW_FN int lm_nw_origin(int first) {
+  const int o = LM_NW_BLK * first;
+  return o < LM_FW - LM_NW_FW ? o : LM_FW - LM_NW_FW;
+}
+
+LM_NW_FN void lm_nw_owned(int tile_x, int first, int count, int ow, int* x0, int* x1) {
+  *x0 = tile_x + LM_NW_BLK * first;
+  const int e = tile_x + LM_NW_BLK * (first + count);
+  *x1 = e < ow ? e : ow;
+}
+
+LM_NW_FN uint64_t lm_nw_entry(uint32_t tile_entry, int first, int count) {
+  return (uint64_t)tile_entry | (uint64_t)(uint32_t)(first | count << 4) << 32;
+}
+LM_NW_FN uint32_t lm_nw_entry_tile(uint64_t e) { return (uint32_t)e; }
+LM_NW_FN int lm_nw_entry_first(uint64_t e) { return (int)(e >> 32) & 15; }
+LM_NW_FN int lm_nw_entry_count(uint64_t e) { return (int)(e >> 36) & 15; }
+
+#define LM_NW_CNT_PTW 0
+#define LM_NW_CNT_TTW (LM_NLIST * LM_TL_NC)
+#define LM_NW_CNT_N ((LM_NLIST + 2) * LM_TL_NC)
+#define LM_NW_CNT_WORDS ((LM_NLIST + 2 + LM_NDET) * LM_TL_NC)
+
+struct LmNarrowOut {
+  int32_t* cnt;
+  uint32_t* ptw_list;
+  uint32_t* ttw_list;
+  unsigned long long* n_list;
+};
+
+struct LmCorrDirRecN {
+  int32_t end[LM_NDET];
+  int32_t total;
+  int32_t pad;
+};
+static_assert(sizeof(LmCorrDirRecN) == 32, "one 32-byte scalar load");
+
+LM_NW_FN int lm_nw_seg_waves(int cnt) { return (cnt + LM_NW_NQ - 1) / LM_NW_NQ; }
+LM_NW_FN int lm_nw_listed_waves(const int32_t* cnt) {
+  int w = 0;
+  for (int c = 0; c < LM_TL_NC; ++c) w += lm_nw_seg_waves(cnt[c]);
+  return w;
+}
+LM_NW_FN LmCorrDirRecN lm_nw_record(const int32_t* waves, int n) {
+  LmCorrDirRecN r;
+  int e = 0;
+  for (int k = 0; k < LM_NDET; ++k) {
+    if (k < n) e += waves[k];
+    r.end[k] = e;
+  }
+  r.total = e;
+  r.pad = 0;
+  return r;
+}
+LM_NW_FN bool lm_nw_lookup(const LmCorrDirRecN& r, int n, int g, int* k, int* local) {
+  if (g >= r.total) return false;
+  int kk = 0, base = 0;
+  for (int j = 0; j < LM_NDET - 1; ++j)
+    if (j + 1 < n && g >= r.end[j]) {
+      kk = j + 1;
+      base = r.end[j];
+    }
+  *k = kk;
+  *local = g - base;
+  return true;
+}
+LM_NW_FN bool lm_nw_segment(const int32_t* cnt, int local, int* c, int* w, int* nv) {
+  int base = 0;
+  for (int s = 0; s < LM_TL_NC; ++s) {
+    const int wv = lm_nw_seg_waves(cnt[s]);
+    if (local < base + wv) {
+      *c = s;
+      *w = local - base;
+      const int left = cnt[s] - LM_NW_NQ * *w;
+      *nv = left < LM_NW_NQ ? left : LM_NW_NQ;
+      return true;
+    }
+    base += wv;
+  }
+  return false;
+}
+LM_NW_FN int lm_nw_grid_waves(int tiles, int nslots, int ndet) { return (tiles * nslots + 1) / 2 + LM_TL_NC * ndet; }
+
+#endif
diff --git a/locomouse_cpp_amd/csrc/lm_device.h b/locomouse_cpp_amd/csrc/lm_device.h
--- a/locomouse_cpp_amd/csrc/lm_device.h
+++ b/locomouse_cpp_amd/csrc/lm_device.h
@@ -87,6 +87,7 @@
   int32_t tbr_on[LM_NDET], tbr_ng[LM_NDET], tbr_off[LM_NDET];
   int32_t tbs_on[LM_NDET], tbs_off[LM_NDET];
   float tbs_bf[LM_NDET], tbs_e[LM_NDET];
+  int32_t nw_on[LM_NDET];
   int32_t fl_my[2], fl_mx[2], fl_oh[2], fl_ow[2];
   int32_t ing_b0[2], ing_nb[2], ing_threads;
   int32_t list_cap[LM_NLIST];
diff --git a/locomouse_cpp_amd/csrc/lm_kernels.hip b/locomouse_cpp_amd/csrc/lm_kernels.hip
--- a/locomouse_cpp_amd/csrc/lm_kernels.hip
+++ b/locomouse_cpp_amd/csrc/lm_kernels.hip
@@ -8,6 +8,7 @@
 #include "lm_introsort.h"
 
 #include "lm_dev_common.h"
+#include "lm_corr_narrow.h"
 #include "lm_tail_bound.h"
 #include "lm_tile_plan.h"
 
@@ -659,15 +660,21 @@
 #define LM_TBW_WPE 8
 #endif
 #define TBW_SEL(a) (k == 0 ? a[0] : k == 1 ? a[1] : a[2])
-template <bool ROWS>
+template <bool ROWS, bool NARROW>
 __global__ __launch_bounds__(LM_TB_THREADS) __attribute__((amdgpu_waves_per_eu(LM_TBW_WPE, 8))) void k_tile_bound(
     const LmConst* __restrict__ Kp, const uint32_t* __restrict__ rng, int64_t rng_slot, int s0, int nslot,
     const double* __restrict__ tbc, const uint8_t* __restrict__ bright, uint8_t* __restrict__ tail_flags,
     int32_t* __restrict__ tt_cnt, uint32_t* __restrict__ tt_list, uint8_t* __restrict__ pt_flags,
-    int32_t* __restrict__ pt_cnt, uint32_t* __restrict__ pt_list, unsigned long long* __restrict__ tbs_fallback) {
+    int32_t* __restrict__ pt_cnt, uint32_t* __restrict__ pt_list, unsigned long long* __restrict__ tbs_fallback,
+    const LmNarrowOut nwo) {
   const LmConst& K = *Kp;
   extern __shared__ __attribute__((aligned(16))) uint8_t tbw_lds[];
   __shared__ int s_n[3], s_b[3], s_m[3], s_base[3], s_nw;
+  __shared__ int s_c[3][2], s_g[3][2], s_p[3][2];
+  if (NARROW && threadIdx.x < 6) {
+    s_c[threadIdx.x >> 1][threadIdx.x & 1] = 0;
+    s_p[threadIdx.x >> 1][threadIdx.x & 1] = 0;
+  }
   const int v = (int)blockIdx.y < K.tbw_nband[0] ? 0 : 1;
   const int band = (int)blockIdx.y - (v ? K.tbw_nband[0] : 0);
   const int slot = s0 + (int)blockIdx.x;
@@ -1012,12 +1019,16 @@
           for (int r = 0; r < nr && proven; ++r) proven = level_b(r, 1);
         }
       }
-      if (!proven) mark[mb + t] = 1u;
+      if constexpr (NARROW) {
+        if (!proven) atomicOr(&mark[mb + t], 1u << (e - t * LM_TB_NBX) | (nr != LM_TB_H ? LM_NW_UNTRIED : 0u));
+      } else {
+        if (!proven) mark[mb + t] = 1u;
+      }
     }
     __syncthreads();
     constexpr int CR = LM_TBW_CR;
     for (int g0 = 0; g0 < nref; g0 += CR * T) {
-      uint32_t en[CR];
+      uint32_t en[CR], mk[CR];
       int kk[CR];
 #pragma unroll
       for (int u = 0; u < CR; ++u) {
@@ -1026,7 +1037,9 @@
         const int k = i < nr3[0] ? 0 : i < nr3[0] + nr3[1] ? 1 : 2;
         const int t = i - (k == 0 ? 0 : k == 1 ? nr3[0] : nr3[0] + nr3[1]);
         en[u] = act ? reinterpret_cast<const uint32_t*>(tbw_lds + TBW_SEL(ent3))[t] : 0u;
-        const bool kp = act && mark[i] != 0u;
+        mk[u] = act ? mark[i] : 0u;
+        const bool kp = mk[u] != 0u;
+
         kk[u] = kp ? k : -1;
         if (act) TBW_SEL(fl)[en[u] & 0xFFFFu] = kp ? 1 : 0;
       }
@@ -1038,6 +1051,7 @@
           const bool mine = kk[u] == k;
           const int pos = wave_append(mine, &s_m[k]);
           if (mine) reinterpret_cast<uint32_t*>(tbw_lds + ent3[k])[pos] = en[u];
+          if (NARROW && mine) mark[(k == 0 ? 0 : k == 1 ? nr3[0] : nr3[0] + nr3[1]) + pos] = mk[u];
         }
     }
     __syncthreads();
@@ -1066,6 +1080,61 @@
         (tail[k] ? tt_list + (int64_t)v * K.tt_stride : pt_list + (int64_t)D.list * K.tl_stride) +
         (int64_t)lm_tl_y0(c, G) * LM_INGEST_FB * ntile + s_base[k];
     for (int p = tid; p < s_n[k]; p += T) out[p] = ent[p];
+  }
+  if constexpr (NARROW) {
+    if (nwo.cnt == nullptr) return;
+    bool split[3];
+    int mbk[3];
+#pragma unroll
+    for (int k = 0; k < 3; ++k) {
+      split[k] = refine[k] && K.nw_on[3 * v + k] != 0;
+      mbk[k] = k == 0 ? 0 : k == 1 ? nr3[0] : nr3[0] + nr3[1];
+    }
+#pragma unroll
+    for (int k = 0; k < 3; ++k) {
+      if (!on[k]) continue;
+      const int n = s_n[k];
+      for (int p0 = 0; p0 < n; p0 += T) {
+        const int p = p0 + tid;
+        const bool act = p < n, nar = act && split[k] && lm_nw_classify(mark[mbk[k] + p]).narrow != 0;
+        const unsigned long long mn = __ballot(nar), mw = __ballot(act && !nar);
+        if ((tid & 63) == 0) {
+          if (mn != 0ull) atomicAdd(&s_c[k][1], (int)__popcll(mn));
+          if (mw != 0ull) atomicAdd(&s_c[k][0], (int)__popcll(mw));
+        }
+      }
+    }
+    __syncthreads();
+    if (tid < 6 && on[tid >> 1]) {
+      const int k = tid >> 1, cls = tid & 1, d = 3 * v + k;
+      const LmDet& D = K.det[d];
+      int32_t* __restrict__ cnt = nwo.cnt + (cls ? LM_NW_CNT_N + d * LM_TL_NC
+                                                 : D.kind != 0 ? LM_NW_CNT_TTW + v * LM_TL_NC : LM_NW_CNT_PTW + D.list * LM_TL_NC);
+      s_g[k][cls] = s_c[k][cls] ? atomicAdd(&cnt[c], s_c[k][cls]) : 0;
+    }
+    __syncthreads();
+#pragma unroll
+    for (int k = 0; k < 3; ++k) {
+      if (!on[k]) continue;
+      const int n = s_n[k];
+      const LmDet& D = K.det[3 * v + k];
+      const int ntile = tail[k] ? K.tt_tx[v] * K.tt_ty[v] : K.fl_tx[v] * K.fl_ty[v];
+      const uint32_t* ent = reinterpret_cast<const uint32_t*>(tbw_lds + K.tbw_ent[3 * v + k]);
+      const int64_t lo = tail[k] ? (int64_t)v * K.tt_stride : (int64_t)D.list * K.tl_stride;
+      const int64_t so = (int64_t)lm_tl_y0(c, G) * LM_INGEST_FB * ntile;
+      uint32_t* __restrict__ wout = (tail[k] ? nwo.ttw_list : nwo.ptw_list) + lo + so + s_g[k][0];
+      unsigned long long* __restrict__ nout = nwo.n_list + (tail[k] ? (int64_t)LM_NLIST * K.tl_stride : 0) + lo + so + s_g[k][1];
+      for (int p0 = 0; p0 < n; p0 += T) {
+        const int p = p0 + tid;
+        const bool act = p < n;
+        const LmNwClass cl = act && split[k] ? lm_nw_classify(mark[mbk[k] + p]) : LmNwClass{0, 0, 0};
+        const bool nar = cl.narrow != 0;
+        const int pn = wave_append(nar, &s_p[k][1]);
+        if (nar) nout[pn] = lm_nw_entry(ent[p], cl.first, cl.count);
+        const int pw = wave_append(act && !nar, &s_p[k][0]);
+        if (act && !nar) wout[pw] = ent[p];
+      }
+    }
   }
 }
 #undef TBW_SEL
@@ -2647,7 +2716,8 @@
                                               const LmConst* __restrict__ Kp, unsigned long long* __restrict__ keys,
                                               const LmSlotOut* __restrict__ prev_hdr, int prev_slot,
                                               LmSlotOut* __restrict__ hdr, int32_t* __restrict__ dark_cnt,
-                                              int32_t* __restrict__ tail_cnt, int32_t* __restrict__ pt_cnt) {
+                                              int32_t* __restrict__ tail_cnt, int32_t* __restrict__ pt_cnt,
+                                              int32_t* __restrict__ nw_cnt) {
   if (blockIdx.x == 1) {
     carry_block(*Kp, keys, prev_hdr, prev_slot, hdr);
     return;
@@ -2657,6 +2727,10 @@
   if (pt_cnt) {
     pt_cnt[threadIdx.x] = 0;
     pt_cnt[256 + threadIdx.x] = 0;
+  }
+  if (nw_cnt) {
+    static_assert(LM_NW_CNT_WORDS == 3 * 256, "k_prep zeroes the narrow / wide counters with its 256 threads");
+    for (int i = 0; i < 3; ++i) nw_cnt[256 * i + threadIdx.x] = 0;
   }
   for (int i = threadIdx.x; i < ns; i += blockDim.x) {
     slots[i] = h_slots[i];
diff --git a/locomouse_cpp_amd/csrc/lm_runtime.hip b/locomouse_cpp_amd/csrc/lm_runtime.hip
--- a/locomouse_cpp_amd/csrc/lm_runtime.hip
+++ b/locomouse_cpp_amd/csrc/lm_runtime.hip
@@ -99,6 +99,10 @@
   DevBuf<int32_t> pt_cnt;
   DevBuf<uint32_t> rng;
   DevBuf<LmCorrDirRec> corr_dir;
+  DevBuf<int32_t> nw_cnt;
+  DevBuf<uint32_t> ptw_list, ttw_list;
+  DevBuf<unsigned long long> nw_list;
+  DevBuf<LmCorrDirRecN> corr_dirn;
   HostBuf<int32_t> h_cnt;
   bool h_cnt_valid = false;
   DevBuf<long long> kprof;
@@ -176,6 +180,8 @@
     std::vector<size_t> lds;
     std::vector<int> threads;
     std::vector<char> ring;
+    std::vector<std::pair<const void*, LmDetGroup>> ngroups;
+    std::vector<size_t> nlds;
   } corr_plan[2];
   DevBuf<uint8_t> bkg, adj;
   DevBuf<int32_t> cal;
@@ -193,6 +199,7 @@
   bool tb_refine = true;
   bool tb_screen = true;
   bool corr_dir_on = true;
+  bool narrow_req = true, narrow_on = false;
   size_t tb_lds = 0;
   size_t tbw_lds = 0;
   bool tbw_row_loop = false;
@@ -332,6 +339,7 @@
   c->tb_screen = flag("LM_TILE_SCREEN", true);
   c->tb_ref = flag("LM_TILE_BOUND_REF", false);
   c->corr_dir_on = flag("LM_CORR_DIR", true);
+  c->narrow_req = flag("LM_CORR_NARROW", true);
   LmTileSwitches sw;
   sw.tailskip = flag("LM_CORR_TAILSKIP", true);
   sw.pointskip = flag("LM_CORR_POINTSKIP", true);
@@ -620,6 +628,48 @@
   c->gscratch_slot = std::max(3 * (int64_t)np, (5 * (int64_t)np + K.ong_nx * K.ong_ny + 2) / 2 + 1);
 }
 
+void build_narrow_plans(lm_ctx* c, const lm_setup* su) {
+  LmConst& K = c->K;
+  const bool f16 = su->corr_precision == LM_CORR_F16;
+  c->narrow_on = false;
+  for (int d = 0; d < LM_NDET; ++d) {
+    const LmDet& D = K.det[d];
+    const bool ring = !f16 && corr_ring(D.kw_ring) && D.kh >= 2;
+    K.nw_on[d] = c->narrow_req && !c->tb_ref && c->tb_refine && c->dark_on && ring && corr_narrow_width(D.kw_ring) &&
+                 K.tbr_on[d] != 0 && K.tbw_use[d] != 0 && (D.kind != 0 ? c->tailskip_on : c->pointskip_on);
+    c->narrow_on = c->narrow_on || K.nw_on[d] != 0;
+  }
+  for (int m = 0; m < 2; ++m) {
+    lm_ctx::CorrPlan& P = c->corr_plan[m];
+    P.ngroups.clear();
+    P.nlds.clear();
+    for (size_t gi = 0; gi < P.groups.size(); ++gi) {
+      if (!P.ring[gi]) continue;
+      const LmDetGroup& G = P.groups[gi].second;
+      const bool all = P.groups[gi].first == corr_kernel_rw_all(c->unfused);
+      LmDetGroup N;
+      std::memset(&N, 0, sizeof(N));
+      size_t lds = 0;
+      const void* fn = nullptr;
+      for (int k = 0; k < G.n; ++k) {
+        const int d = G.ids[k];
+        if (!K.nw_on[d]) continue;
+        const LmDet& D = K.det[d];
+        const int prev = N.n ? N.tile_end[N.n - 1] : 0;
+        N.ids[N.n] = d;
+        N.tile_end[N.n] = prev + D.tiles_x * D.tiles_y;
+        ++N.n;
+        N.ring_floats = std::max(N.ring_floats, rw_ring_floats(D.kw_ring, LM_NW_FW));
+        lds = std::max(lds, corr_rwn_lds(D.kw_ring));
+        fn = all ? corr_kernel_n_all(c->unfused) : corr_kernel_n(D.kw_ring, c->unfused);
+      }
+      if (N.n == 0) continue;
+      P.ngroups.push_back({fn, N});
+      P.nlds.push_back(lds);
+    }
+  }
+}
+
 void build_corr_plans(lm_ctx* c, const lm_setup* su) {
   LmConst& K = c->K;
   c->unfused = su->filter_arith == LM_FILTER_UNFUSED;
@@ -751,11 +801,18 @@
   c->fstride = (nv + 255) / 256 * 256;
   HIPCHK(hipFuncSetAttribute((const void*)k_tail<false>, hipFuncAttributeMaxDynamicSharedMemorySize, (int)c->tail_lds));
   HIPCHK(hipFuncSetAttribute((const void*)k_tile_bound_ref, hipFuncAttributeMaxDynamicSharedMemorySize, (int)c->tb_lds));
-  HIPCHK(hipFuncSetAttribute((const void*)k_tile_bound<false>, hipFuncAttributeMaxDynamicSharedMemorySize, (int)c->tbw_lds));
-  HIPCHK(hipFuncSetAttribute((const void*)k_tile_bound<true>, hipFuncAttributeMaxDynamicSharedMemorySize, (int)c->tbw_lds));
-  for (const auto& P : c->corr_plan)
+  HIPCHK(hipFuncSetAttribute((const void*)k_tile_bound<false, false>, hipFuncAttributeMaxDynamicSharedMemorySize, (int)c->tbw_lds));
+  HIPCHK(hipFuncSetAttribute((const void*)k_tile_bound<true, false>, hipFuncAttributeMaxDynamicSharedMemorySize, (int)c->tbw_lds));
+  if (c->narrow_on) {
+    HIPCHK(hipFuncSetAttribute((const void*)k_tile_bound<false, true>, hipFuncAttributeMaxDynamicSharedMemorySize, (int)c->tbw_lds));
+    HIPCHK(hipFuncSetAttribute((const void*)k_tile_bound<true, true>, hipFuncAttributeMaxDynamicSharedMemorySize, (int)c->tbw_lds));
+  }
+  for (const auto& P : c->corr_plan) {
     for (size_t g = 0; g < P.groups.size(); ++g)
       HIPCHK(hipFuncSetAttribute(P.groups[g].first, hipFuncAttributeMaxDynamicSharedMemorySize, (int)P.lds[g]));
+    for (size_t g = 0; g < P.ngroups.size(); ++g)
+      HIPCHK(hipFuncSetAttribute(P.ngroups[g].first, hipFuncAttributeMaxDynamicSharedMemorySize, (int)P.nlds[g]));
+  }
 }
 
 void validate_and_build(lm_ctx* c, const lm_setup* su, const lm_params* P, const lm_model* M) {
@@ -787,6 +844,7 @@
   c->tb_lds = plan.tb_lds;
   c->tbw_lds = plan.tbw_lds;
   c->tbw_row_loop = plan.row_loop;
+  build_narrow_plans(c, su);
   const std::vector<_Float16> w16 = f16_fragments(K, su, M);
   uint8_t adj[256];
   imadjust_table(adj);
@@ -845,6 +903,15 @@
     L.rng.alloc((size_t)(c->ext_slot_bytes / LM_INGEST_VEC) * ns);
     SET_SYNC(L.rng.p, 0, (size_t)(c->ext_slot_bytes / LM_INGEST_VEC) * ns * sizeof(uint32_t), st);
   }
+  if (c->narrow_on) {
+    L.nw_cnt.alloc(LM_NW_CNT_WORDS);
+    SET_SYNC(L.nw_cnt.p, 0, LM_NW_CNT_WORDS * sizeof(int32_t), st);
+    L.ptw_list.alloc(c->pointskip_on ? (size_t)LM_NLIST * K.tl_stride : 1);
+    L.ttw_list.alloc(c->tailskip_on ? (size_t)2 * K.tt_stride : 1);
+    L.nw_list.alloc((size_t)LM_NLIST * K.tl_stride + (size_t)2 * K.tt_stride);
+    L.corr_dirn.alloc(LM_NDET);
+    SET_SYNC(L.corr_dirn.p, 0, LM_NDET * sizeof(LmCorrDirRecN), st);
+  }
   L.err.alloc(16);
   if (c->corr_dir_on) {
     L.corr_dir.alloc(LM_NDET);
@@ -1140,6 +1207,21 @@
   return d;
 }
 
+CorrDark lane_dark_ring(const lm_ctx* c, Lane& L) {
+  CorrDark d = lane_dark(c, L);
+  if (c->narrow_on) {
+    if (d.tail_cnt) {
+      d.tail_cnt = L.nw_cnt.p + LM_NW_CNT_TTW;
+      d.tail_list = L.ttw_list.p;
+    }
+    if (d.pt_cnt) {
+      d.pt_cnt = L.nw_cnt.p + LM_NW_CNT_PTW;
+      d.pt_list = L.ptw_list.p;
+    }
+  }
+  return d;
+}
+
 void enqueue_chain(lm_ctx* c, Lane& L, Arena& A, const Lane::Pending& P, Timer& T, bool do_carry, int part) {
   const LmConst& K = c->K;
   const LmConst* dK = c->dK.p;
@@ -1149,7 +1231,7 @@
   if (part <= 0) {
     k_prep<<<do_carry ? 2 : 1, 256, 0, st>>>(L.h_slots.d, L.h_frame_ptr.d, L.h_ctl.d, n + 1, L.slots.p, L.frame_ptr.p,
                                              A.ctl.p, L.npos.p, L.err.p, dK, L.keys.p, L.arena[P.prv].hdr.p, P.last_n,
-                                             A.hdr.p, L.dark_cnt.p, L.tail_cnt.p, L.pt_cnt.p);
+                                             A.hdr.p, L.dark_cnt.p, L.tail_cnt.p, L.pt_cnt.p, L.nw_cnt.p);
     T.begin("k_minmax");
     k_minmax<<<dim3(LM_MM_SPLIT, n + 1 - s_lut0), LM_MM_THREADS, 0, st>>>(L.frame_ptr.p, c->bkg.p, c->npix, s_lut0,
                                                                         L.mm.p);
@@ -1175,19 +1257,28 @@
         k_tile_bound_ref<<<dim3((unsigned)nproc, 2), LM_TB_THREADS, c->tb_lds, st>>>(
             dK, L.ext.p, c->ext_slot_bytes, s_proc0, c->tb_const.p, dk.flags, dk.tail_flags, dk.tail_cnt, dk.tail_list,
             dk.pt_flags, dk.pt_cnt, dk.pt_list);
-      else
-        (c->tbw_row_loop ? k_tile_bound<true> : k_tile_bound<false>)
+      else {
+        const LmNarrowOut nwo = c->narrow_on ? LmNarrowOut{L.nw_cnt.p, L.ptw_list.p, L.ttw_list.p, L.nw_list.p}
+                                             : LmNarrowOut{nullptr, nullptr, nullptr, nullptr};
+        (c->narrow_on ? (c->tbw_row_loop ? k_tile_bound<true, true> : k_tile_bound<false, true>)
+                      : (c->tbw_row_loop ? k_tile_bound<true, false> : k_tile_bound<false, false>))
             <<<dim3((unsigned)nproc, (unsigned)(K.tbw_nband[0] + K.tbw_nband[1])), LM_TB_THREADS, c->tbw_lds, st>>>(
                 dK, L.rng.p, c->ext_slot_bytes / LM_INGEST_VEC, s_proc0, nproc, c->tb_const.p, dk.flags, dk.tail_flags,
-                dk.tail_cnt, dk.tail_list, dk.pt_flags, dk.pt_cnt, dk.pt_list, c->tbs_fallback.p);
+                dk.tail_cnt, dk.tail_list, dk.pt_flags, dk.pt_cnt, dk.pt_list, c->tbs_fallback.p, nwo);
+      }
       T.end();
     }
     const lm_ctx::CorrPlan& CP = c->corr_plan[P.plan];
     if (c->corr_dir_on && std::find(CP.ring.begin(), CP.ring.end(), (char)1) != CP.ring.end()) {
       std::vector<LmDetGroup> groups;
       for (const auto& grp : CP.groups) groups.push_back(grp.second);
-      HIPCHK(launch_corr_dir(st, dK, groups.data(), CP.ring.data(), (int)groups.size(), nproc, dk, L.corr_dir.p,
-                             L.err.p));
+      HIPCHK(launch_corr_dir(st, dK, groups.data(), CP.ring.data(), (int)groups.size(), nproc, lane_dark_ring(c, L),
+                             L.corr_dir.p, L.err.p));
+      if (c->narrow_on && !CP.ngroups.empty()) {
+        std::vector<LmDetGroup> ng;
+        for (const auto& grp : CP.ngroups) ng.push_back(grp.second);
+        HIPCHK(launch_corr_dir_n(st, ng.data(), (int)ng.size(), nproc, L.nw_cnt.p, L.corr_dirn.p, L.err.p));
+      }
     }
   }
   if (part == 1 || part < 0) {
@@ -1199,9 +1290,14 @@
       const void* w = c->setup.corr_precision == LM_CORR_F16 ? (const void*)c->weights16.p : (const void*)c->weights.p;
       HIPCHK(launch_corr(grp.first, CP.ring[gi], dim3(G.tile_end[G.n - 1], nproc), CP.threads[gi], CP.lds[gi], st, dK,
                          G, L.ext.p, c->ext_slot_bytes, w, s_proc0, L.keys.p, L.npos.p, L.tailbin.p,
-                         c->tailbin_slot_bytes, lane_dark(c, L),
+                         c->tailbin_slot_bytes, CP.ring[gi] ? lane_dark_ring(c, L) : lane_dark(c, L),
                          c->corr_dir_on && CP.ring[gi] ? L.corr_dir.p + gi : nullptr));
     }
+    if (c->narrow_on)
+      for (size_t gi = 0; gi < CP.ngroups.size(); ++gi)
+        HIPCHK(launch_corr_n(CP.ngroups[gi].first, nproc, CP.nlds[gi], st, dK, CP.ngroups[gi].second, L.ext.p,
+                             c->ext_slot_bytes, c->weights.p, L.keys.p, L.npos.p, L.tailbin.p, c->tailbin_slot_bytes,
+                             L.nw_cnt.p, L.nw_list.p, c->corr_dir_on ? L.corr_dirn.p + gi : nullptr));
     T.end();
   }
   if (part == 2 || part < 0) {
@@ -1880,6 +1976,58 @@
   });
 }
 
+LM_API lm_status lm_debug_narrow_work(lm_ctx* ctx, int32_t* out) {
+  if (!ctx || !out) return fail(LM_ERR_INVALID_ARGUMENT, "null argument");
+  for (int k = 0; k < 2 * LM_NDET; ++k) out[k] = -1;
+  if (!ctx->narrow_on) return LM_OK;
+  return read_delivered(ctx, no_check, [&](const Lane& L, auto fetch) {
+    int32_t h[LM_NW_CNT_WORDS];
+    fetch(h, L.nw_cnt.p, sizeof(h));
+    for (int d = 0; d < LM_NDET; ++d) {
+      const LmDet& D = ctx->K.det[d];
+      if (!(D.kind != 0 ? ctx->tailskip_on : ctx->pointskip_on)) continue;
+      const int32_t* w = h + (D.kind != 0 ? LM_NW_CNT_TTW + D.view * LM_TL_NC : LM_NW_CNT_PTW + D.list * LM_TL_NC);
+      out[2 * d] = std::accumulate(h + LM_NW_CNT_N + d * LM_TL_NC, h + LM_NW_CNT_N + (d + 1) * LM_TL_NC, 0);
+      out[2 * d + 1] = std::accumulate(w, w + LM_TL_NC, 0);
+    }
+  });
+}
+
+LM_API lm_status lm_debug_narrow_entries(lm_ctx* ctx, int32_t det, int32_t narrow, uint64_t* out, int32_t cap, int32_t* n) {
+  if (!ctx || !out || !n) return fail(LM_ERR_INVALID_ARGUMENT, "null argument");
+  *n = 0;
+  if (!ctx->narrow_on) return fail(LM_ERR_INVALID_ARGUMENT, "the narrow class is off");
+  if (det < 0 || det >= LM_NDET) return fail(LM_ERR_INVALID_ARGUMENT, "index out of range");
+  const LmConst& K = ctx->K;
+  const LmDet& D = K.det[det];
+  if (!(D.kind != 0 ? ctx->tailskip_on : ctx->pointskip_on)) return LM_OK;
+  return read_delivered(ctx, no_check, [&](const Lane& L, auto fetch) {
+    int32_t h[LM_NW_CNT_WORDS];
+    fetch(h, L.nw_cnt.p, sizeof(h));
+    const bool tail = D.kind != 0;
+    const int v = D.view, ntile = tail ? K.tt_tx[v] * K.tt_ty[v] : K.fl_tx[v] * K.fl_ty[v];
+    const int G = (ctx->delivered.slots + LM_INGEST_FB - 1) / LM_INGEST_FB;
+    const int32_t* cnt = h + (narrow ? LM_NW_CNT_N + det * LM_TL_NC
+                                     : tail ? LM_NW_CNT_TTW + v * LM_TL_NC : LM_NW_CNT_PTW + D.list * LM_TL_NC);
+    const int64_t lo = tail ? (int64_t)v * K.tt_stride : (int64_t)D.list * K.tl_stride;
+    int32_t got = 0;
+    for (int c = 0; c < LM_TL_NC; ++c) {
+      const int64_t so = (int64_t)lm_tl_y0(c, G) * LM_INGEST_FB * ntile;
+      const int m = std::min(cnt[c], cap - got);
+      if (m <= 0) continue;
+      if (narrow) {
+        fetch(out + got, L.nw_list.p + (tail ? (int64_t)LM_NLIST * K.tl_stride : 0) + lo + so, sizeof(uint64_t) * m);
+      } else {
+        std::vector<uint32_t> w((size_t)m);
+        fetch(w.data(), (tail ? L.ttw_list.p : L.ptw_list.p) + lo + so, sizeof(uint32_t) * m);
+        for (int i = 0; i < m; ++i) out[got + i] = w[i];
+      }
+      got += m;
+    }
+    *n = got;
+  });
+}
+
 LM_API lm_status lm_debug_tail_tiles(lm_ctx* ctx, int32_t f, int32_t view, uint8_t* out, int32_t rows, int32_t cols) {
   if (!ctx || !out) return fail(LM_ERR_INVALID_ARGUMENT, "null argument");
   if (!ctx->tailskip_on) return fail(LM_ERR_INVALID_ARGUMENT, "tail-tile skipping is off");
diff --git a/locomouse_cpp_amd/runtime.py b/locomouse_cpp_amd/runtime.py
--- a/locomouse_cpp_amd/runtime.py
+++ b/locomouse_cpp_amd/runtime.py
@@ -23,7 +23,7 @@
     "lm_detect_submit", "lm_detect_submit_device", "lm_detect_collect", "lm_ctx_lanes", "lm_ctx_pending",
     "lm_debug_corr_work", "lm_debug_batch_slots", "lm_debug_dark_tile_width",
     "lm_debug_dark_tile_height", "lm_debug_tail_work", "lm_debug_tail_tiles", "lm_debug_point_work",
-    "lm_debug_point_tiles", "lm_debug_screen_fallback",
+    "lm_debug_point_tiles", "lm_debug_screen_fallback", "lm_debug_narrow_work", "lm_debug_narrow_entries",
 )
 
 HIPCC_FLAGS = ["--offload-arch=gfx950", "-O3", "-std=c++17", "-fPIC", "-shared", "-ffp-contract=off", "-fno-slp-vectorize",
@@ -189,6 +189,9 @@
         L.lm_debug_point_work.argtypes = [C.c_void_p, C.POINTER(C.c_int32)]
         L.lm_debug_point_tiles.argtypes = [C.c_void_p, C.c_int32, C.c_int32, C.c_void_p, C.c_int32, C.c_int32]
         L.lm_debug_screen_fallback.argtypes = [C.c_void_p, C.POINTER(C.c_int64)]
+        L.lm_debug_narrow_work.argtypes = [C.c_void_p, C.POINTER(C.c_int32)]
+        L.lm_debug_narrow_entries.argtypes = [C.c_void_p, C.c_int32, C.c_int32, C.c_void_p, C.c_int32,
+                                              C.POINTER(C.c_int32)]
         L.lm_debug_batch_slots.argtypes = [C.c_void_p]
         L.lm_debug_batch_slots.restype = C.c_int32
         L.lm_synth_frames_device.argtypes = [C.c_int32, C.c_void_p, C.c_int32, C.c_int32, C.c_int64, C.c_int32,
@@ -423,6 +426,21 @@
         _check(lib().lm_debug_screen_fallback(self._h, C.byref(out)))
         return int(out.value)
 
+    def narrow_work(self):
+        out = (C.c_int32 * 12)()
+        _check(lib().lm_debug_narrow_work(self._h, out))
+        if all(out[k] < 0 for k in range(12)):
+            return None
+        return {d: (out[2 * d], out[2 * d + 1]) for d in range(6) if out[2 * d] >= 0}
+
+    def narrow_entries(self, det, narrow, cap=None):
+        if cap is None:
+            cap = max(1, (self.narrow_work() or {}).get(det, (0, 0))[0 if narrow else 1])
+        out = np.zeros(cap, np.uint64)
+        n = C.c_int32(0)
+        _check(lib().lm_debug_narrow_entries(self._h, det, 1 if narrow else 0, out.ctypes.data, cap, C.byref(n)))
+        return out[:n.value].copy()
+
     def tail_tiles(self, f, view):
         g = self.geometry()
         tw, th = self.dark_tile_shape()
```

After: 988,900, median of 6. 1.03x the previous value.
